# musket-ml/segmentation_training_pipeline

Hardware: AMD Instinct MI355X
Metric: images/sec U-Net/ResNet34 512x512 bs16 training step (higher is better)
Workload: dtype bf16; 1 GPU; U-Net/ResNet34 512x512x3 1-class, batch 16 per GPU, BCE+Dice, Adam, on-device augment S1 (BASELINE.json configs[1]); global_batch=16, parallelism=dp1, hipgraph=True

## Files before the change

segmentation_training_pipeline_amd/csrc/augment.hip:

```cpp
#include "common.h"
#include <cstdlib>

struct AugSample {
  float m[6];
  float add[3], mul[3];
  float flags, gray_q, noise_k, drop_t;
  float adde_lo, adde_hi, mule_lo, mule_hi;
  float seed, r0, r1, r2;
};

__device__ __forceinline__ uint32_t aug_hash(uint32_t seed, uint32_t pix, uint32_t ch, uint32_t op) {
  uint32_t h = seed ^ (pix * 0x9E3779B1u) ^ (ch * 0x85EBCA77u) ^ (op * 0xC2B2AE3Du);
  h ^= h >> 16; h *= 0x7feb352du; h ^= h >> 15; h *= 0x846ca68bu; h ^= h >> 16;
  return h;
}
__device__ __forceinline__ int clip255(int v) { return min(max(v, 0), 255); }

__device__ __forceinline__ int64_t fix10(double v) { return (int64_t)__double2ll_rn(v); }

__global__ __launch_bounds__(256) void augment_kernel(const uint8_t* __restrict__ img, const uint8_t* __restrict__ mask,
                                                      uint8_t* __restrict__ img_out, uint8_t* __restrict__ mask_out,
                                                      const AugSample* __restrict__ prm, int N, int Hin, int Win, int Hout,
                                                      int Wout, int C, const int32_t* __restrict__ field) {
  const int64_t total = (int64_t)N * Hout * Wout;
  for (int64_t i = (int64_t)blockIdx.x * 256 + threadIdx.x; i < total; i += (int64_t)gridDim.x * 256) {
    const int xo = (int)(i % Wout);
    const int yo = (int)((i / Wout) % Hout);
    const int n = (int)(i / ((int64_t)Wout * Hout));
    const AugSample s = prm[n];
    double xd = (double)xo, yd = (double)yo;
    if (field) {
      const int32_t f = field[i];
      xd = __dadd_rn(xd, __dmul_rn((double)(int16_t)(f & 0xffff), 0.015625));
      yd = __dadd_rn(yd, __dmul_rn((double)(int16_t)(f >> 16), 0.015625));
    }
    const int64_t X0 = fix10(__dmul_rn(__dmul_rn((double)s.m[0], xd), 1024.0)) +
                       fix10(__dmul_rn(__dadd_rn(__dmul_rn((double)s.m[1], yd), (double)s.m[2]), 1024.0));
    const int64_t Y0 = fix10(__dmul_rn(__dmul_rn((double)s.m[3], xd), 1024.0)) +
                       fix10(__dmul_rn(__dadd_rn(__dmul_rn((double)s.m[4], yd), (double)s.m[5]), 1024.0));
    const int64_t X = (X0 + 16) >> 5, Y = (Y0 + 16) >> 5;
    const int64_t ix = X >> 5, iy = Y >> 5;
    const int fx = (int)(X & 31), fy = (int)(Y & 31);
    const int w00 = (32 - fx) * (32 - fy), w01 = fx * (32 - fy), w10 = (32 - fx) * fy, w11 = fx * fy;
    const bool x0ok = ix >= 0 && ix < Win, x1ok = ix + 1 >= 0 && ix + 1 < Win;
    const bool y0ok = iy >= 0 && iy < Hin, y1ok = iy + 1 >= 0 && iy + 1 < Hin;
    const uint8_t* b = img + (int64_t)n * Hin * Win * C;
    const uint32_t flags = (uint32_t)s.flags, seed = (uint32_t)s.seed, pix = (uint32_t)(yo * Wout + xo);
    const int noise_k = (int)s.noise_k;
    const uint32_t drop_t = (uint32_t)s.drop_t;
    const int ae_lo = (int)s.adde_lo, ae_n = (int)s.adde_hi - ae_lo + 1;
    int px[4] = {0, 0, 0, 0};
    for (int c = 0; c < C; ++c) {
      const int v00 = (x0ok && y0ok) ? b[(iy * Win + ix) * C + c] : 0;
      const int v01 = (x1ok && y0ok) ? b[(iy * Win + ix + 1) * C + c] : 0;
      const int v10 = (x0ok && y1ok) ? b[((iy + 1) * Win + ix) * C + c] : 0;
      const int v11 = (x1ok && y1ok) ? b[((iy + 1) * Win + ix + 1) * C + c] : 0;
      int v = (w00 * v00 + w01 * v01 + w10 * v10 + w11 * v11 + 512) >> 10;
      const int cc = c < 3 ? c : 2;
      v = clip255(v + (int)s.add[cc]);
      if (s.mul[cc] != 1.f) v = clip255((int)rintf(__fmul_rn((float)v, s.mul[cc])));
      if (flags & 64u) {
        const float u = __fmul_rn((float)(aug_hash(seed, pix, (flags & 16u) ? c : 0, 1u) >> 8), 5.9604644775390625e-8f);
        const float m = __fadd_rn(s.mule_lo, __fmul_rn(__fsub_rn(s.mule_hi, s.mule_lo), u));
        v = clip255((int)rintf(__fmul_rn((float)v, m)));
      }
      if (flags & 32u) v = clip255(v + ae_lo + (int)(aug_hash(seed, pix, (flags & 8u) ? c : 0, 2u) % (uint32_t)ae_n));
      if (noise_k) {
        const uint32_t h = aug_hash(seed, pix, (flags & 2u) ? c : 0, 3u);
        const int sum = (int)(h & 255u) + (int)((h >> 8) & 255u) + (int)((h >> 16) & 255u) + (int)(h >> 24);
        v = clip255(v + (((sum - 510) * noise_k + 32768) >> 16));
      }
      if (drop_t && (aug_hash(seed, pix, (flags & 4u) ? c : 0, 4u) >> 8) < drop_t) v = 0;
      if (c < 4) px[c] = v;
      if (C != 3) img_out[i * C + c] = (uint8_t)((flags & 1u) ? 255 - v : v);
    }
    if (C == 3) {
      const int gq = (int)s.gray_q;
      if (gq) {
        const int gray = (px[0] * 4899 + px[1] * 9617 + px[2] * 1868 + 8192) >> 14;
#pragma unroll
        for (int c = 0; c < 3; ++c) px[c] = (gq * gray + (256 - gq) * px[c] + 128) >> 8;
      }
#pragma unroll
      for (int c = 0; c < 3; ++c) img_out[i * 3 + c] = (uint8_t)((flags & 1u) ? 255 - px[c] : px[c]);
    }
    if (mask) {
      const int64_t mx = (X0 + 512) >> 10, my = (Y0 + 512) >> 10;
      uint8_t mv = 0;
      if (mx >= 0 && mx < Win && my >= 0 && my < Hin) mv = mask[((int64_t)n * Hin + my) * Win + mx];
      mask_out[i] = mv;
    }
  }
}

static int launch_augment(const uint8_t* img, const uint8_t* mask, uint8_t* img_out, uint8_t* mask_out, const float* params,
                          const int32_t* field, int32_t N, int32_t Hin, int32_t Win, int32_t Hout, int32_t Wout, int32_t C, void* stream) {
  if (!img || !img_out || !params || N <= 0 || C <= 0 || (mask && !mask_out)) return STP_E_BADARG;
  int64_t g = ((int64_t)N * Hout * Wout + 255) / 256;
  if (g > 8192) g = 8192;
  hipLaunchKernelGGL(augment_kernel, dim3((int)g), dim3(256), 0, (hipStream_t)stream, img, mask, img_out, mask_out,
                     (const AugSample*)params, N, Hin, Win, Hout, Wout, C, field);
  STP_LAUNCH_CHECK();
  return STP_OK;
}

extern "C" int stp_augment_u8(const uint8_t* img, const uint8_t* mask, uint8_t* img_out, uint8_t* mask_out, const float* params,
                              int32_t N, int32_t Hin, int32_t Win, int32_t Hout, int32_t Wout, int32_t C, void* stream) {
  return launch_augment(img, mask, img_out, mask_out, params, nullptr, N, Hin, Win, Hout, Wout, C, stream);
}

extern "C" int stp_augment_field_u8(const uint8_t* img, const uint8_t* mask, uint8_t* img_out, uint8_t* mask_out, const float* params,
                                    const int32_t* field, int32_t N, int32_t Hin, int32_t Win, int32_t Hout, int32_t Wout, int32_t C,
                                    void* stream) {
  return launch_augment(img, mask, img_out, mask_out, params, field, N, Hin, Win, Hout, Wout, C, stream);
}

__device__ __forceinline__ int32_t pack_disp(int dx, int dy) {
  dx = min(max(dx, -32768), 32767);
  dy = min(max(dy, -32768), 32767);
  return (int32_t)(((uint32_t)dx & 0xffffu) | ((uint32_t)dy << 16));
}

__global__ __launch_bounds__(256) void field_piecewise_kernel(int32_t* __restrict__ field, const int32_t* __restrict__ grid, int N, int H, int W,
                                                              int R, int Cg) {
  const int64_t total = (int64_t)N * H * W;
  for (int64_t i = (int64_t)blockIdx.x * 256 + threadIdx.x; i < total; i += (int64_t)gridDim.x * 256) {
    const int x = (int)(i % W), y = (int)((i / W) % H), n = (int)(i / ((int64_t)W * H));
    const int64_t u = (int64_t)x * (Cg - 1) * 1024 / W, v = (int64_t)y * (R - 1) * 1024 / H;
    const int cx = min((int)(u >> 10), Cg - 2), cy = min((int)(v >> 10), R - 2);
    const int64_t fu = u - ((int64_t)cx << 10), fv = v - ((int64_t)cy << 10);
    const int32_t* g = grid + (((int64_t)n * R + cy) * Cg + cx) * 2;
    int d[2];
#pragma unroll
    for (int a = 0; a < 2; ++a) {
      const int64_t d00 = g[a], d10 = g[2 + a], d01 = g[2 * Cg + a], d11 = g[2 * Cg + 2 + a];
      const int64_t t = fu >= fv ? d00 * 1024 + fu * (d10 - d00) + fv * (d11 - d10) : d00 * 1024 + fv * (d01 - d00) + fu * (d11 - d01);
      d[a] = (int)((t + 512) >> 10);
    }
    field[i] = pack_disp(d[0], d[1]);
  }
}

extern "C" int stp_field_piecewise(int32_t* field, const int32_t* grid, int32_t N, int32_t H, int32_t W, int32_t rows, int32_t cols,
                                   void* stream) {
  if (!field || !grid || N <= 0 || H <= 0 || W <= 0 || rows < 2 || cols < 2) return STP_E_BADARG;
  int64_t g = ((int64_t)N * H * W + 255) / 256;
  if (g > 8192) g = 8192;
  hipLaunchKernelGGL(field_piecewise_kernel, dim3((int)g), dim3(256), 0, (hipStream_t)stream, field, grid, N, H, W, rows, cols);
  STP_LAUNCH_CHECK();
  return STP_OK;
}

#define STP_ELASTIC_RECORD 69
__global__ __launch_bounds__(256) void field_elastic_h_kernel(int32_t* __restrict__ tmp, const int32_t* __restrict__ prm, int N, int H, int W) {
  const int64_t total = (int64_t)N * H * W;
  for (int64_t i = (int64_t)blockIdx.x * 256 + threadIdx.x; i < total; i += (int64_t)gridDim.x * 256) {
    const int x = (int)(i % W), y = (int)((i / W) % H), n = (int)(i / ((int64_t)W * H));
    const int32_t* p = prm + (int64_t)n * STP_ELASTIC_RECORD;
    const uint32_t seed = (uint32_t)p[0];
    const int r = p[2];
    int t[2];
#pragma unroll
    for (int a = 0; a < 2; ++a) {
      int sum = 0;
      for (int k = -r; k <= r; ++k) {
        const int xx = x + k;
        if (xx < 0 || xx >= W) continue;
        const int nz = (int)(aug_hash(seed, (uint32_t)(y * W + xx), (uint32_t)a, 7u) >> 16) - 32768;
        sum += p[4 + (k < 0 ? -k : k)] * nz;
      }
      t[a] = (sum + 16384) >> 15;
    }
    tmp[i] = pack_disp(t[0], t[1]);
  }
}
__global__ __launch_bounds__(256) void field_elastic_v_kernel(int32_t* __restrict__ field, const int32_t* __restrict__ tmp,
                                                              const int32_t* __restrict__ prm, int N, int H, int W) {
  const int64_t total = (int64_t)N * H * W;
  for (int64_t i = (int64_t)blockIdx.x * 256 + threadIdx.x; i < total; i += (int64_t)gridDim.x * 256) {
    const int x = (int)(i % W), y = (int)((i / W) % H), n = (int)(i / ((int64_t)W * H));
    const int32_t* p = prm + (int64_t)n * STP_ELASTIC_RECORD;
    const int alpha = p[1], r = p[2];
    int s0 = 0, s1 = 0;
    for (int k = -r; k <= r; ++k) {
// ... 190 lines not shown
```

segmentation_training_pipeline_amd/csrc/bn_pool.hip:

```cpp
#include "common.h"
#include <algorithm>
#include <cstdlib>

#define BN_MAX_BLOCKS 1024
#ifndef POOL_ROWS
#define POOL_ROWS 4
#endif


template <typename T> __device__ __forceinline__ f32x4 ld4(const T* p);
template <> __device__ __forceinline__ f32x4 ld4<float>(const float* p) { return load4(p); }
template <> __device__ __forceinline__ f32x4 ld4<bf16_t>(const bf16_t* p) { return load4(p); }

template <typename T, int V> __device__ __forceinline__ void ldv(const T* p, float (&o)[V]) {
  if constexpr (V == 4) {
    const f32x4 v = ld4<T>(p);
    o[0] = v.x; o[1] = v.y; o[2] = v.z; o[3] = v.w;
  } else {
    const u32x4 r = *reinterpret_cast<const u32x4*>(p);
#pragma unroll
    for (int e = 0; e < 4; ++e) { o[2 * e] = h16lo_to_f32(r[e]); o[2 * e + 1] = h16hi_to_f32(r[e]); }
  }
}
template <typename T, int V> __device__ __forceinline__ void stv(T* p, const float (&o)[V]) {
// ... 1118 lines not shown
                       (bf16_t*)dx, rows, C, mean, rstd, gamma, (const float*)nullptr, sums, inv_rows, 0, accumulate_dx, (const long long*)nullptr, 0, (float*)nullptr, (float*)nullptr,
                       (const bf16_t*)dadd);
  else if (dtype == STP_F32)
    hipLaunchKernelGGL((bn_bwd_apply_kernel<float, 4>), dim3(gr), dim3(256), lds2, s, (const float*)x, (const float*)g, (float*)dx,
                       rows, C, mean, rstd, gamma, (const float*)nullptr, sums, inv_rows, 0, accumulate_dx, (const long long*)nullptr, 0, (float*)nullptr, (float*)nullptr,
                       (const float*)dadd);
  else
    return STP_E_BADARG;
  STP_LAUNCH_CHECK();
  return STP_OK;
}

extern "C" int stp_bn_backward_fused(const void* x, const void* g, void* dx, int32_t dtype, int64_t rows, int32_t C,
                                     const float* mean, const float* rstd, const float* gamma, const float* partial,
                                     int32_t tiles, float* dgamma, float* dbeta, int32_t accumulate_dx, void* workspace,
                                     size_t workspace_bytes, void* stream) {
  return stp_bn_backward_fused_add(x, g, dx, dx, dtype, rows, C, mean, rstd, gamma, partial, tiles, dgamma, dbeta, accumulate_dx, workspace,
                                   workspace_bytes, stream);
}

template <typename T, int V>
__global__ __launch_bounds__(256) void maxpool_fwd_kernel(const T* __restrict__ x, T* __restrict__ y, uint8_t* __restrict__ idx,
                                                          int N, int H, int W, int C, int Ho, int Wo) {
  const int cg = C / V;
  const int t = blockIdx.x * 256 + threadIdx.x;
  if (t >= Wo * cg) return;
  const int wo = t / cg, c = (t - wo * cg) * V;
  for (int rr = 0; rr < POOL_ROWS; ++rr) {
  const int orow = blockIdx.y * POOL_ROWS + rr;
  if (orow >= N * Ho) break;
  const int n = orow / Ho, ho = orow - n * Ho;
  float best[V];
  uint8_t bi[V];
  float v[9][V];
#pragma unroll
  for (int kh = 0; kh < 3; ++kh)
#pragma unroll
    for (int kw = 0; kw < 3; ++kw) {
      const int h = min(max(2 * ho - 1 + kh, 0), H - 1), w = min(max(2 * wo - 1 + kw, 0), W - 1);
      ldv<T, V>(x + (((size_t)n * H + h) * W + w) * C + c, v[kh * 3 + kw]);
    }
#pragma unroll
  for (int kh = 0; kh < 3; ++kh)
#pragma unroll
    for (int kw = 0; kw < 3; ++kw) {
      const int h = 2 * ho - 1 + kh, w = 2 * wo - 1 + kw;
      const bool in = (unsigned)h < (unsigned)H && (unsigned)w < (unsigned)W;
#pragma unroll
      for (int e = 0; e < V; ++e) {
        const float tv = in ? v[kh * 3 + kw][e] : 0.f;
        if ((kh | kw) == 0 || tv > best[e]) { best[e] = tv; bi[e] = (uint8_t)(kh * 3 + kw); }
      }
    }
  const size_t o = (((size_t)n * Ho + ho) * Wo + wo) * C + c;
  stv<T, V>(y + o, best);
  if (idx) {
    if constexpr (V == 8) *reinterpret_cast<uint2*>(idx + o) = *reinterpret_cast<const uint2*>(bi);
    else *reinterpret_cast<uint32_t*>(idx + o) = *reinterpret_cast<const uint32_t*>(bi);
  }
  }
}

__global__ __launch_bounds__(256) void bn_apply_maxpool_kernel(const bf16_t* __restrict__ x, bf16_t* __restrict__ yb, bf16_t* __restrict__ y,
                                                               uint8_t* __restrict__ idx, int N, int H, int W, int C, int Ho, int Wo,
                                                               const float* mean, const float* rstd, const float* gamma, const float* beta, int relu) {
  const int cg = C >> 3;
  const int t = blockIdx.x * 256 + threadIdx.x;
  if (t >= Wo * cg) return;
  const int wo = t / cg, c = (t - wo * cg) * 8;
  float sc[8], sh[8];
  {
    const f32x4 m0 = *reinterpret_cast<const f32x4*>(mean + c), m1 = *reinterpret_cast<const f32x4*>(mean + c + 4);
    const f32x4 r0 = *reinterpret_cast<const f32x4*>(rstd + c), r1 = *reinterpret_cast<const f32x4*>(rstd + c + 4);
    f32x4 g0 = {1.f, 1.f, 1.f, 1.f}, g1 = g0, b0 = {0.f, 0.f, 0.f, 0.f}, b1 = b0;
    if (gamma) { g0 = *reinterpret_cast<const f32x4*>(gamma + c); g1 = *reinterpret_cast<const f32x4*>(gamma + c + 4); }
    if (beta) { b0 = *reinterpret_cast<const f32x4*>(beta + c); b1 = *reinterpret_cast<const f32x4*>(beta + c + 4); }
#pragma unroll
    for (int e = 0; e < 8; ++e) {
      const float r = e < 4 ? r0[e & 3] : r1[e & 3], k = gamma ? r * (e < 4 ? g0[e & 3] : g1[e & 3]) : r;
      sc[e] = k;
      sh[e] = (e < 4 ? b0[e & 3] : b1[e & 3]) - (e < 4 ? m0[e & 3] : m1[e & 3]) * k;
    }
  }
  for (int rr = 0; rr < POOL_ROWS; ++rr) {
    const int orow = blockIdx.y * POOL_ROWS + rr;
    if (orow >= N * Ho) break;
    const int n = orow / Ho, ho = orow - n * Ho;
    u32x4 v[9];
#pragma unroll
    for (int kh = 0; kh < 3; ++kh)
#pragma unroll
      for (int kw = 0; kw < 3; ++kw) {
        const int h = min(max(2 * ho - 1 + kh, 0), H - 1), w = min(max(2 * wo - 1 + kw, 0), W - 1);
        v[kh * 3 + kw] = *reinterpret_cast<const u32x4*>(x + (((size_t)n * H + h) * W + w) * C + c);
      }
    float best[8];
    uint8_t bi[8];
#pragma unroll
    for (int kh = 0; kh < 3; ++kh)
#pragma unroll
      for (int kw = 0; kw < 3; ++kw) {
        const int h = 2 * ho - 1 + kh, w = 2 * wo - 1 + kw;
        const bool in = (unsigned)h < (unsigned)H && (unsigned)w < (unsigned)W;
        u32x4 o;
#pragma unroll
        for (int e = 0; e < 4; ++e) {
          const float lo = bn_act(bn_affine(h16lo_to_f32(v[kh * 3 + kw][e]), sc[2 * e], sh[2 * e]), relu);
          const float hi = bn_act(bn_affine(h16hi_to_f32(v[kh * 3 + kw][e]), sc[2 * e + 1], sh[2 * e + 1]), relu);
          o[e] = pack_bf16x2(lo, hi);
          const float tl = in ? h16lo_to_f32(o[e]) : 0.f, th = in ? h16hi_to_f32(o[e]) : 0.f;
          if ((kh | kw) == 0 || tl > best[2 * e]) { best[2 * e] = tl; bi[2 * e] = (uint8_t)(kh * 3 + kw); }
          if ((kh | kw) == 0 || th > best[2 * e + 1]) { best[2 * e + 1] = th; bi[2 * e + 1] = (uint8_t)(kh * 3 + kw); }
        }
        if (kh >= 1 && kw >= 1 && in) *reinterpret_cast<u32x4*>(yb + (((size_t)n * H + h) * W + w) * C + c) = o;
      }
    const size_t oo = (((size_t)n * Ho + ho) * Wo + wo) * C + c;
    *reinterpret_cast<u32x4*>(y + oo) = u32x4{pack_bf16x2(best[0], best[1]), pack_bf16x2(best[2], best[3]), pack_bf16x2(best[4], best[5]),
                                             pack_bf16x2(best[6], best[7])};
    if (idx) *reinterpret_cast<uint2*>(idx + oo) = *reinterpret_cast<const uint2*>(bi);
  }
}
extern "C" int stp_bn_apply_maxpool3x3s2(const void* x, void* yb, void* y, uint8_t* idx, int32_t N, int32_t H, int32_t W, int32_t C, int32_t dtype,
                                         const float* mean, const float* rstd, const float* gamma, const float* beta, int32_t relu, void* stream) {
  if (!stp_dtype_ok(dtype)) return STP_E_BADARG;
  if (dtype != STP_H16 || !x || !yb || !y || !mean || !rstd || N <= 0 || (C & 7) || (H & 1) || (W & 1)) return STP_E_BADARG;
  const int Ho = H / 2, Wo = W / 2;
  if ((int64_t)N * Ho > 65535 * POOL_ROWS) return STP_E_BADARG;
  const dim3 grid(ceil_div(Wo * (C / 8), 256), ceil_div(N * Ho, POOL_ROWS));
  hipLaunchKernelGGL(bn_apply_maxpool_kernel, grid, dim3(256), 0, (hipStream_t)stream, (const bf16_t*)x, (bf16_t*)yb, (bf16_t*)y, idx, N, H, W, C, Ho, Wo,
                     mean, rstd, gamma, beta, relu);
  STP_LAUNCH_CHECK();
  return STP_OK;
}

__device__ __forceinline__ f32x4 stored4(f32x4 v, const float*) { return v; }
__device__ __forceinline__ f32x4 stored4(f32x4 v, const bf16_t*) {
  const uint32_t a = pack_bf16x2(v.x, v.y), b = pack_bf16x2(v.z, v.w);
  return f32x4{h16lo_to_f32(a), h16hi_to_f32(a), h16lo_to_f32(b), h16hi_to_f32(b)};
}

#define BNB_ROWS 8


template <typename T, int V>
__device__ __forceinline__ void bnb_mask_store(float (&g)[V], size_t o, int c, const BnBack& bnb, T* __restrict__ dx, float (&sg)[V],
                                               float (&sq)[V]) {
  float xv[V];
  ldv<T, V>(reinterpret_cast<const T*>(bnb.x) + o, xv);
#pragma unroll
  for (int q = 0; q < V / 4; ++q) {
    const BnBackCh k = bnback_load(bnb, c + 4 * q);
    const f32x4 st = stored4(f32x4{g[4 * q], g[4 * q + 1], g[4 * q + 2], g[4 * q + 3]}, (const T*)nullptr);
    f32x4 s4 = {0.f, 0.f, 0.f, 0.f}, q4 = {0.f, 0.f, 0.f, 0.f};
    const f32x4 m = bnback_apply(k, bnb.relu, f32x4{xv[4 * q], xv[4 * q + 1], xv[4 * q + 2], xv[4 * q + 3]}, st, s4, q4);
#pragma unroll
    for (int e = 0; e < 4; ++e) { g[4 * q + e] = m[e]; sg[4 * q + e] += s4[e]; sq[4 * q + e] += q4[e]; }
  }
  stv<T, V>(dx + o, g);
}

template <int V>
__device__ __forceinline__ void bnb_reduce(const float (&sg)[V], const float (&sq)[V], int cg, int C, float* __restrict__ partial) {
  extern __shared__ float red[];
#pragma unroll
  for (int e = 0; e < V; ++e) { red[threadIdx.x * 2 * V + e] = sg[e]; red[threadIdx.x * 2 * V + V + e] = sq[e]; }
  __syncthreads();
  const int cl = cg < 256 ? cg : 256;
  for (int idx = threadIdx.x; idx < cl * V; idx += 256) {
    const int gq = idx / V, e = idx - gq * V;
    const int cg0 = (blockIdx.x * 256 + gq) % cg;
    float s = 0.f, q2 = 0.f;
    for (int l = gq; l < 256; l += cl) { s += red[l * 2 * V + e]; q2 += red[l * 2 * V + V + e]; }
    const size_t nblk = (size_t)gridDim.x * gridDim.y, blk = (size_t)blockIdx.y * gridDim.x + blockIdx.x;
    const int ch = cg0 * V + e;
    partial[(size_t)ch * nblk + blk] = s;
    partial[((size_t)C + ch) * nblk + blk] = q2;
  }
}

template <typename T, int V, bool BNB>
__global__ __launch_bounds__(256) void maxpool_bwd_kernel(const uint8_t* __restrict__ idx, const T* __restrict__ dy,
                                                          T* __restrict__ dx, int N, int H, int W, int C, int Ho, int Wo,
                                                          int accumulate, BnBack bnb, float* __restrict__ partial) {
  const int cg = C / V;
  const int t = blockIdx.x * 256 + threadIdx.x;
  const bool on = t < W * cg;
  if (!BNB && !on) return;
  const int w = on ? t / cg : 0, c = on ? (t - w * cg) * V : 0;
  constexpr int ROWS = BNB ? BNB_ROWS : POOL_ROWS;
  float sg[V], sq[V];
#pragma unroll
  for (int e = 0; e < V; ++e) { sg[e] = 0.f; sq[e] = 0.f; }
  for (int rr = 0; rr < ROWS; ++rr) {
    const int row = blockIdx.y * ROWS + rr;
    if (row >= N * H || !on) break;
    const int n = row / H, h = row - n * H;
    float g[V];
// ... 1568 lines not shown
}
extern "C" int stp_maxpool_k(const void* x, void* y, int32_t* idx, int32_t N, int32_t H, int32_t W, int32_t C, int32_t k, int32_t dtype,
                             void* stream) {
  if (!stp_dtype_ok(dtype)) return STP_E_BADARG;
  if (!x || !y || N <= 0 || H <= 0 || W <= 0 || C <= 0 || k < 1 || H % k || W % k) return STP_E_BADARG;
  const int g = grid_for((int64_t)N * (H / k) * (W / k) * C);
  if (dtype == STP_H16) hipLaunchKernelGGL(maxpool_k_kernel<bf16_t>, dim3(g), dim3(256), 0, (hipStream_t)stream, (const bf16_t*)x, (bf16_t*)y, idx, N, H, W, C, k);
  else if (dtype == STP_F32) hipLaunchKernelGGL(maxpool_k_kernel<float>, dim3(g), dim3(256), 0, (hipStream_t)stream, (const float*)x, (float*)y, idx, N, H, W, C, k);
  else return STP_E_BADARG;
  STP_LAUNCH_CHECK();
  return STP_OK;
}
extern "C" int stp_maxpool_k_bwd(const int32_t* idx, const void* dy, void* dx, int32_t N, int32_t H, int32_t W, int32_t C, int32_t k,
                                 int32_t dtype, int32_t accumulate, void* stream) {
  if (!stp_dtype_ok(dtype)) return STP_E_BADARG;
  if (!idx || !dy || !dx || N <= 0 || H <= 0 || W <= 0 || C <= 0 || k < 1 || H % k || W % k) return STP_E_BADARG;
  const int g = grid_for((int64_t)N * H * W * C);
  if (dtype == STP_H16) hipLaunchKernelGGL(maxpool_k_bwd_kernel<bf16_t>, dim3(g), dim3(256), 0, (hipStream_t)stream, idx, (const bf16_t*)dy, (bf16_t*)dx, N, H, W, C, k, accumulate);
  else if (dtype == STP_F32) hipLaunchKernelGGL(maxpool_k_bwd_kernel<float>, dim3(g), dim3(256), 0, (hipStream_t)stream, idx, (const float*)dy, (float*)dx, N, H, W, C, k, accumulate);
  else return STP_E_BADARG;
  STP_LAUNCH_CHECK();
  return STP_OK;
}

template <typename T>
__global__ __launch_bounds__(256) void resize_nearest_kernel(const T* __restrict__ x, T* __restrict__ y, int N, int H, int W, int C, int f,
                                                             int ldo, int coff) {
  const int Ho = H * f, Wo = W * f;
  const int64_t total = (int64_t)N * Ho * Wo * C;
  for (int64_t i = (int64_t)blockIdx.x * 256 + threadIdx.x; i < total; i += (int64_t)gridDim.x * 256) {
    const int c = (int)(i % C);
    const int64_t p = i / C;
    const int xo = (int)(p % Wo), yo = (int)((p / Wo) % Ho), n = (int)(p / ((int64_t)Wo * Ho));
    y[p * ldo + coff + c] = x[(((int64_t)n * H + yo / f) * W + xo / f) * C + c];
  }
}
template <typename T>
__global__ __launch_bounds__(256) void resize_nearest_bwd_kernel(const T* __restrict__ dy, T* __restrict__ dx, int N, int H, int W, int C,
                                                                 int f, int ldo, int coff, int accumulate) {
  const int Wo = W * f, Ho = H * f;
  const int64_t total = (int64_t)N * H * W * C;
  for (int64_t i = (int64_t)blockIdx.x * 256 + threadIdx.x; i < total; i += (int64_t)gridDim.x * 256) {
    const int c = (int)(i % C);
    const int64_t p = i / C;
    const int xi = (int)(p % W), yi = (int)((p / W) % H), n = (int)(p / ((int64_t)W * H));
    float s = 0.f;
    for (int a = 0; a < f; ++a)
      for (int b = 0; b < f; ++b) s += Elem<T>::load(dy + (((int64_t)n * Ho + yi * f + a) * Wo + xi * f + b) * ldo + coff + c);
    if (accumulate) s += Elem<T>::load(dx + i);
    Elem<T>::store(dx + i, s);
  }
}
extern "C" int stp_resize_nearest(const void* x, void* y, int32_t N, int32_t H, int32_t W, int32_t C, int32_t factor, int32_t ldo, int32_t coff,
                                  int32_t dtype, void* stream) {
  if (!stp_dtype_ok(dtype)) return STP_E_BADARG;
  if (!x || !y || N <= 0 || H <= 0 || W <= 0 || C <= 0 || factor < 1 || ldo < coff + C || coff < 0) return STP_E_BADARG;
  const int g = grid_for((int64_t)N * H * factor * W * factor * C);
  if (dtype == STP_H16) hipLaunchKernelGGL(resize_nearest_kernel<bf16_t>, dim3(g), dim3(256), 0, (hipStream_t)stream, (const bf16_t*)x, (bf16_t*)y, N, H, W, C, factor, ldo, coff);
  else if (dtype == STP_F32) hipLaunchKernelGGL(resize_nearest_kernel<float>, dim3(g), dim3(256), 0, (hipStream_t)stream, (const float*)x, (float*)y, N, H, W, C, factor, ldo, coff);
  else return STP_E_BADARG;
  STP_LAUNCH_CHECK();
  return STP_OK;
}
extern "C" int stp_resize_nearest_bwd(const void* dy, void* dx, int32_t N, int32_t H, int32_t W, int32_t C, int32_t factor, int32_t ldo,
                                      int32_t coff, int32_t dtype, int32_t accumulate, void* stream) {
  if (!stp_dtype_ok(dtype)) return STP_E_BADARG;
  if (!dy || !dx || N <= 0 || H <= 0 || W <= 0 || C <= 0 || factor < 1 || ldo < coff + C || coff < 0) return STP_E_BADARG;
  const int g = grid_for((int64_t)N * H * W * C);
  if (dtype == STP_H16) hipLaunchKernelGGL(resize_nearest_bwd_kernel<bf16_t>, dim3(g), dim3(256), 0, (hipStream_t)stream, (const bf16_t*)dy, (bf16_t*)dx, N, H, W, C, factor, ldo, coff, accumulate);
  else if (dtype == STP_F32) hipLaunchKernelGGL(resize_nearest_bwd_kernel<float>, dim3(g), dim3(256), 0, (hipStream_t)stream, (const float*)dy, (float*)dx, N, H, W, C, factor, ldo, coff, accumulate);
  else return STP_E_BADARG;
  STP_LAUNCH_CHECK();
  return STP_OK;
}

__global__ __launch_bounds__(256) void colsum_finalize_kernel(const float* partial, int blocks, int C, float* out,
                                                              int accumulate) {
  const int c = blockIdx.x * 4 + (threadIdx.x & 3);
  const Sum2 t = reduce_partials(partial, blocks, C, c, false);
  if ((threadIdx.x >> 2) != 0 || c >= C) return;
  out[c] = accumulate ? out[c] + (float)t.s : (float)t.s;
}

extern "C" int stp_channel_sum(const void* x, int32_t dtype, int64_t rows, int32_t C, float* out, int32_t accumulate,
                               void* workspace, size_t workspace_bytes, void* stream) {
  if (!stp_dtype_ok(dtype)) return STP_E_BADARG;
  if (!x || !out || !workspace || rows <= 0 || C <= 0 || (C & 3)) return STP_E_BADARG;
  if (workspace_bytes < stp_bn_workspace_bytes(C)) return STP_E_WORKSPACE;
  hipStream_t s = (hipStream_t)stream;
  const int blocks = bn_blocks(rows);
  float* partial = (float*)workspace;
  if (dtype == STP_H16 && (C & 7) == 0)
    hipLaunchKernelGGL((bn_partial_kernel<bf16_t, 8>), dim3(blocks), dim3(256), 256 * 16 * sizeof(float), s, (const bf16_t*)x, rows, C, partial);
  else if (dtype == STP_H16)
    hipLaunchKernelGGL((bn_partial_kernel<bf16_t, 4>), dim3(blocks), dim3(256), 256 * 8 * sizeof(float), s, (const bf16_t*)x, rows, C, partial);
  else if (dtype == STP_F32)
    hipLaunchKernelGGL((bn_partial_kernel<float, 4>), dim3(blocks), dim3(256), 256 * 8 * sizeof(float), s, (const float*)x, rows, C, partial);
  else
    return STP_E_BADARG;
  STP_LAUNCH_CHECK();
  hipLaunchKernelGGL(colsum_finalize_kernel, dim3(ceil_div(C, 4)), dim3(256), 0, s, partial, blocks, C, out, accumulate);
  STP_LAUNCH_CHECK();
  return STP_OK;
}

template <typename T>
__global__ __launch_bounds__(256) void add_inplace_kernel(T* __restrict__ dst, const T* __restrict__ src, int64_t n4) {
  for (int64_t i = (int64_t)blockIdx.x * 256 + threadIdx.x; i < n4; i += (int64_t)gridDim.x * 256)
    store4(dst + i * 4, ld4<T>(dst + i * 4) + ld4<T>(src + i * 4));
}

extern "C" int stp_add_inplace(void* dst, const void* src, int64_t count, int32_t dtype, void* stream) {
  if (!stp_dtype_ok(dtype)) return STP_E_BADARG;
  if (!dst || !src || count <= 0 || (count & 3)) return STP_E_BADARG;
  const int g = grid_for(count >> 2);
  hipStream_t s = (hipStream_t)stream;
  if (dtype == STP_H16)
    hipLaunchKernelGGL(add_inplace_kernel<bf16_t>, dim3(g), dim3(256), 0, s, (bf16_t*)dst, (const bf16_t*)src, count >> 2);
  else if (dtype == STP_F32)
    hipLaunchKernelGGL(add_inplace_kernel<float>, dim3(g), dim3(256), 0, s, (float*)dst, (const float*)src, count >> 2);
  else
    return STP_E_BADARG;
  STP_LAUNCH_CHECK();
  return STP_OK;
}
```

segmentation_training_pipeline_amd/csrc/conv_sc.h:

```cpp
#pragma once
#include "common.h"
#include <cstdlib>
#include <type_traits>
#include <utility>

struct ScArgs {
  const char* src;
  const char* weight;
  const float* bias;
  char* dst;
  int N, H, W, Hs, Ws, Cout, up, accumulate, relu;
  int tiles_x, tiles_y;
  FastDiv divTx, divTy;
  float* stats;
  int stat_slots;
  BnBack bnb;
  int sum2;
  uint32_t src_bytes;
  BnBack pbn;
};

template <typename T> struct ScStageBn;
template <> struct ScStageBn<float> {
  f32x4 sc, sh;
  __device__ __forceinline__ void load(const BnBack& b, int c) { const BnBackCh k = bnback_load(b, c); sc = k.sc; sh = k.sh; }
  __device__ __forceinline__ void load_tab(const float* tsc, const float* tsh, int c) {
    sc = *reinterpret_cast<const f32x4*>(tsc + c); sh = *reinterpret_cast<const f32x4*>(tsh + c);
  }
  __device__ __forceinline__ u32x4 apply(const u32x4& r, int relu) const {
    u32x4 o;
#pragma unroll
    for (int e = 0; e < 4; ++e) o[e] = __float_as_uint(bn_act(bn_affine(__uint_as_float(r[e]), sc[e], sh[e]), relu));
    return o;
  }
};
template <> struct ScStageBn<bf16_t> {
  f32x2 sc[4], sh[4];
  __device__ __forceinline__ void load(const BnBack& b, int c) {
    const BnBackCh k0 = bnback_load(b, c), k1 = bnback_load(b, c + 4);
    sc[0] = f32x2{k0.sc[0], k0.sc[1]}; sc[1] = f32x2{k0.sc[2], k0.sc[3]}; sc[2] = f32x2{k1.sc[0], k1.sc[1]}; sc[3] = f32x2{k1.sc[2], k1.sc[3]};
    sh[0] = f32x2{k0.sh[0], k0.sh[1]}; sh[1] = f32x2{k0.sh[2], k0.sh[3]}; sh[2] = f32x2{k1.sh[0], k1.sh[1]}; sh[3] = f32x2{k1.sh[2], k1.sh[3]};
  }
  __device__ __forceinline__ void load_tab(const float* tsc, const float* tsh, int c) {
#pragma unroll
    for (int e = 0; e < 4; ++e) { sc[e] = *reinterpret_cast<const f32x2*>(tsc + c + 2 * e); sh[e] = *reinterpret_cast<const f32x2*>(tsh + c + 2 * e); }
  }
  __device__ __forceinline__ u32x4 apply(const u32x4& r, int relu) const {
    u32x4 o;
#pragma unroll
    for (int e = 0; e < 4; ++e) {
      f32x2 v = {h16lo_to_f32(r[e]), h16hi_to_f32(r[e])};
      v = __builtin_elementwise_fma(v, sc[e], sh[e]);
      o[e] = pack_bf16x2(bn_act(v.x, relu), bn_act(v.y, relu));
    }
    return o;
  }
};


constexpr int SC_TH = 8, SC_TW = 32, SC_HW = SC_TW + 2, SC_HH = SC_TH + 2;

template <int... Ks, typename F>
__device__ __forceinline__ void sc_unroll_seq(std::integer_sequence<int, Ks...>, F&& f) { (f(std::integral_constant<int, Ks>{}), ...); }
template <int N, typename F>
__device__ __forceinline__ void sc_unroll(F&& f) { sc_unroll_seq(std::make_integer_sequence<int, N>{}, f); }
#ifndef SC_RING
#define SC_RING 8
#endif

#ifndef SC_WPE_SMALL
#define SC_WPE_SMALL 4
#endif

static inline bool sc_stream_on() {
  static const bool on = !(getenv("STP_SC_STREAM") && atoi(getenv("STP_SC_STREAM")) == 0);
  return on;
}
static inline int sc_cu_count() {
  static const int cus = [] {
    int d = 0, n = 0;
    if (hipGetDevice(&d) != hipSuccess || hipDeviceGetAttribute(&n, hipDeviceAttributeMultiprocessorCount, d) != hipSuccess || n <= 0) n = 256;
    return n;
  }();
  return cus;
}
static inline int sc_stream_blocks(int dtype, int cin, int cout, int ntiles) {
  const int per_cu = cout <= 16 ? (dtype == STP_H16 && cin <= 16 ? SC_WPE_SMALL : 3) : 2;
  const int64_t b = (int64_t)sc_cu_count() * per_cu;
  return (int)(b < ntiles ? b : ntiles);
}


struct ScWgArgs {
  const char* src;
  const char* dy;
  float* slabs;
  int N, H, W, Hs, Ws, Cout, up;
  int tiles_x, tiles_y, ntiles;
  int ctot, coff;
  uint32_t src_bytes, dy_bytes;
  BnBack pbn;
};

constexpr int ST_HH = (SC_TH - 1) * 2 + 7, ST_HW = 70, ST_WROW = 464, ST_HALO = ST_HH * ST_HW * 8, ST_WBYTES = 64 * ST_WROW;

struct StemArgs {
  const char* src;
  const char* weight;
  char* dst;
  int N, H, W, Ho, Wo, tiles_x, tiles_y;
  FastDiv divTx, divTy;
  float* stats;
  uint32_t src_bytes;
};

bool stem_lean_serves(int N, int H, int W);
int stem_lean_blocks(int ntiles);
int stem_lean_launch(const StemArgs& a, hipStream_t s);
bool stem_wg_lean_serves(int N, int H, int W, int Ho, int Wo);
int stem_wg_lean_blocks(int N, int Ho, int Wo);
int stem_wg_lean_launch(const void* src, const void* dy, float* slabs, int N, int H, int W, int Ho, int Wo, hipStream_t s);

int sc_lean_launch(const ScArgs& a, int cin, int dtype, hipStream_t s);
int sc_wg_lean_launch(const ScWgArgs& a, int cin, int cout, int dtype, int blocks, hipStream_t s);
```

segmentation_training_pipeline_amd/csrc/conv_sc.hip:

```cpp
#include "conv_sc.h"

__device__ __forceinline__ f32x4 sc_stored(f32x4 v, const float*) { return v; }
__device__ __forceinline__ f32x4 sc_stored(f32x4 v, const bf16_t*) {
  const uint32_t a = pack_bf16x2(v.x, v.y), b = pack_bf16x2(v.z, v.w);
  return f32x4{h16lo_to_f32(a), h16hi_to_f32(a), h16lo_to_f32(b), h16hi_to_f32(b)};
}

template <typename T> struct ScMma;
template <> struct ScMma<bf16_t> {
  __device__ static __forceinline__ void run(const u32x4& a, const u32x4& b, f32x4& c) {
    c = mfma16_16x16x32(a, b, c);
  }
};
template <> struct ScMma<float> {
  __device__ static __forceinline__ void run(const u32x4& a, const u32x4& b, f32x4& c) {
    c = __builtin_amdgcn_mfma_f32_16x16x4f32(__uint_as_float(a.x), __uint_as_float(b.x), c, 0, 0, 0);
    c = __builtin_amdgcn_mfma_f32_16x16x4f32(__uint_as_float(a.y), __uint_as_float(b.y), c, 0, 0, 0);
    c = __builtin_amdgcn_mfma_f32_16x16x4f32(__uint_as_float(a.z), __uint_as_float(b.z), c, 0, 0, 0);
    c = __builtin_amdgcn_mfma_f32_16x16x4f32(__uint_as_float(a.w), __uint_as_float(b.w), c, 0, 0, 0);
  }
};

template <typename T> struct ScRaw4;
template <> struct ScRaw4<float> {
// ... 455 lines not shown
        if (PART && c == NCH - 1 && !last_ok) v = u32x4{0u, 0u, 0u, 0u};
#pragma unroll
        for (int i = 0; i < TM; ++i) ScMma<T>::run(fa[i][c], v, acc[i][F]);
        if constexpr (k + D < R) issue(std::integral_constant<int, k + D>{});
      });
    } else
#endif
    {
#pragma unroll
    for (int f = 0; f < 4; ++f) {
#pragma unroll
      for (int c = 0; c < NCH; ++c) {
        u32x4 fb = {0u, 0u, 0u, 0u};
#if !defined(STP_EXP) || STP_EXP != 13
        if (bl[c] != 0xffffffffu) fb = *reinterpret_cast<const u32x4*>(smem + bl[c] + (CUR * BUF + ((f >> 1) * SC_HW + (f & 1) * 16) * PIXB));
#pragma unroll
        for (int i = 0; i < TM; ++i) ScMma<T>::run(fa[i][c], fb, acc[i][f]);
#else
        if (a.N < 0) acc[0][f][0] += __uint_as_float(fa[0][c][0] + bl[c]);
#endif
      }
    }
    }
    ep.finish(a, acc, red, n, y0, x0, tile, ntiles, tid, wave, lr, lg);
  };

  ep.reset_stats();
  for (int tile = t_first; tile < t_end; tile += 2 * t_step) {
    body(tile, std::integral_constant<int, 0>{});
    if (tile + t_step < t_end) body(tile + t_step, std::integral_constant<int, 1>{});
  }
  ep.flush_stats(a, red, (int)blockIdx.x, (int)gridDim.x, tid, wave, lr, lg);
}

template <typename T, int CIN, int TM>
static int launch_sc(const ScArgs& a, hipStream_t s) {
  const int ntiles = a.N * a.tiles_x * a.tiles_y;
  if (sc_stream_on()) {
    constexpr int NV = SC_HH * SC_HW * (CIN / Elem<T>::VEC), NPASS = (NV + 255) / 256;
    const size_t lds = (size_t)2 * NPASS * 4096 + (4 * TM * 16 * 2 + 128 + 64) * sizeof(float);
    const int blocks = sc_stream_blocks(Elem<T>::DTYPE, CIN, TM * 16, ntiles);
    static bool attr_set = false;
    if (lds > 64 * 1024 && !attr_set) {
      if (hipFuncSetAttribute(reinterpret_cast<const void*>(conv_sc_stream_kernel<T, CIN, TM>), hipFuncAttributeMaxDynamicSharedMemorySize, (int)lds) != hipSuccess)
        return STP_E_LAUNCH;
      attr_set = true;
    }
    hipLaunchKernelGGL((conv_sc_stream_kernel<T, CIN, TM>), dim3(blocks), dim3(256), lds, s, a);
    STP_LAUNCH_CHECK();
    return STP_OK;
  }
  const size_t lds = (size_t)SC_HH * SC_HW * CIN * sizeof(T) + 4 * TM * 16 * 2 * sizeof(float);
  hipLaunchKernelGGL((conv_sc_kernel<T, CIN, TM>), dim3(ntiles), dim3(256), lds, s, a);
  STP_LAUNCH_CHECK();
  return STP_OK;
}

extern "C" int stp_conv2d_sc_stats_tiles(const stp_conv_params* p) {
  const int ntiles = p->N * ceil_div(p->Hv, SC_TH) * ceil_div(p->Wv, SC_TW);
  if (!sc_stream_on() || p->stats_slots) return ntiles;
  return sc_stream_blocks(p->dtype, p->C0, p->Cout <= 16 ? 16 : 32, ntiles);
}

template <typename T>
static int dispatch_sc(const ScArgs& a, int cin, hipStream_t s) {
  const int tm = a.Cout <= 16 ? 1 : 2;
  switch (cin * 4 + tm) {
    case 4 * 4 + 1: if constexpr (sizeof(T) == 4) return launch_sc<T, 4, 1>(a, s); else return STP_E_BADARG;
    case 4 * 4 + 2: if constexpr (sizeof(T) == 4) return launch_sc<T, 4, 2>(a, s); else return STP_E_BADARG;
    case 8 * 4 + 1: return launch_sc<T, 8, 1>(a, s);
    case 8 * 4 + 2: return launch_sc<T, 8, 2>(a, s);
    case 16 * 4 + 1: return launch_sc<T, 16, 1>(a, s);
    case 16 * 4 + 2: return launch_sc<T, 16, 2>(a, s);
    case 32 * 4 + 1: return launch_sc<T, 32, 1>(a, s);
    case 32 * 4 + 2: return launch_sc<T, 32, 2>(a, s);
    default: return STP_E_BADARG;
  }
}

extern "C" int stp_conv2d_sc_eligible(const stp_conv_params* p) {
  if (!p || !stp_dtype_ok(p->dtype)) return 0;
  const int vec = p->dtype == STP_H16 ? 8 : 4;
  const int cin = p->C0;
  const bool cin_ok = p->dtype == STP_F32 ? (cin == 4 || cin == 8 || cin == 16) : (cin == 8 || cin == 16 || cin == 32);
  return p->KH == 3 && p->KW == 3 && p->stride == 1 && p->pad == 1 && p->C1 == 0 && cin_ok && (cin % vec) == 0 && p->Cout <= 32 &&
         p->Cd0 == p->Cout && !p->residual && p->Ho == p->Hv && p->Wo == p->Wv &&
         (p->src0_mode == STP_SRC_DIRECT || (p->src0_mode == STP_SRC_NEAREST2X && p->Hv == 2 * p->Hs0 && p->Wv == 2 * p->Ws0));
}

extern "C" int stp_conv2d_sc(const stp_conv_params* p, void* stream) {
  if (!stp_conv2d_sc_eligible(p) || !p->src0 || !p->weight || !p->dst0) return STP_E_BADARG;
  ScArgs a;
  a.src = (const char*)p->src0; a.weight = (const char*)p->weight; a.bias = p->bias; a.dst = (char*)p->dst0;
  a.N = p->N; a.H = p->Hv; a.W = p->Wv; a.Hs = p->Hs0; a.Ws = p->Ws0; a.Cout = p->Cout;
  a.up = p->src0_mode == STP_SRC_NEAREST2X; a.accumulate = p->accumulate0; a.relu = p->relu;
  {
    const uint64_t sb = (uint64_t)p->N * p->Hs0 * p->Ws0 * p->C0 * (p->dtype == STP_H16 ? 2 : 4);
    if (sb >= 0x80000000ull) return STP_E_BADARG;
    a.src_bytes = (uint32_t)sb;
  }
  a.tiles_x = ceil_div(a.W, SC_TW); a.tiles_y = ceil_div(a.H, SC_TH);
  a.divTx = make_fastdiv((uint32_t)a.tiles_x); a.divTy = make_fastdiv((uint32_t)a.tiles_y);
  a.stats = p->stats_partial;
  a.stat_slots = p->stats_slots;
  if (a.stats && (p->Cout & 3)) return STP_E_BADARG;
  if (a.stat_slots && (!a.stats || (a.stat_slots & (a.stat_slots - 1)) || a.stat_slots > 64)) return STP_E_BADARG;
  a.bnb.x = (const char*)p->bnb_x; a.bnb.mean = p->bnb_mean; a.bnb.rstd = p->bnb_rstd; a.bnb.gamma = p->bnb_gamma;
  a.bnb.beta = p->bnb_beta; a.bnb.relu = p->bnb_relu;
  a.sum2 = p->dst_sum2x2;
  a.pbn.x = nullptr; a.pbn.mean = p->src_bn_mean; a.pbn.rstd = p->src_bn_rstd; a.pbn.gamma = p->src_bn_gamma; a.pbn.beta = p->src_bn_beta;
  a.pbn.relu = p->src_bn_relu;
  if (a.pbn.mean && !a.pbn.rstd) return STP_E_BADARG;
  if (a.bnb.x && (!a.stats || !a.bnb.mean || !a.bnb.rstd || p->relu)) return STP_E_BADARG;
  if (a.sum2 && ((p->Cout & 3) || (a.H & 1) || (a.W & 1) || p->bias || p->relu || (a.stats && !a.bnb.x))) return STP_E_BADARG;
  const_cast<stp_conv_params*>(p)->stats_tiles = stp_conv2d_sc_stats_tiles(p);
  hipStream_t s = (hipStream_t)stream;
  {
    const int r = sc_lean_launch(a, p->C0, p->dtype, s);
    if (r != 1) return r;
  }
  return p->dtype == STP_H16 ? dispatch_sc<bf16_t>(a, p->C0, s) : dispatch_sc<float>(a, p->C0, s);
}

struct ScwArgs {
  const char* src;
  const char* weight;
  char* dst_up;
  char* dst_sk;
  int N, H, W, C0, C1, acc_up, acc_sk;
  int tiles_x, tiles_y;
  FastDiv divTx, divTy;
  float* stats;
  BnBack bnb;
  uint32_t src_bytes, x_bytes;
  uint32_t up_bytes, sk_bytes;
};

template <typename T>
__global__ __launch_bounds__(256, 2) void conv_scw_stream_kernel(const ScwArgs a) {
  constexpr int CIN = 32, SZ = (int)sizeof(T), K = 9 * CIN, NCH = 9, VPP = 4, PIXB = CIN * SZ;
  constexpr int NV = SC_HH * SC_HW * VPP, NPASS = (NV + 255) / 256, BUF = NPASS * 4096;
  static_assert(SZ == 2, "16-bit storage");
  extern __shared__ __attribute__((aligned(16))) char smem[];
  float* ktab = reinterpret_cast<float*>(smem + 2 * BUF);
  constexpr int XBUF = 3 * 4096;
  char* const xlds = smem + 2 * BUF + 2048;
  const int tid = threadIdx.x, lane = tid & 63;
  const int wave = __builtin_amdgcn_readfirstlane(tid >> 6);
  const int lr = lane & 15, lg = lane >> 4;
  const int cbi[2] = {a.C0 == 64 ? wave * 16 : wave * 32, a.C0 == 64 ? 64 + wave * 16 : wave * 32 + 16};
  const bool upi[2] = {cbi[0] < a.C0, cbi[1] < a.C0};

  const int ntiles = a.N * a.tiles_x * a.tiles_y;
  int t_first, t_step, t_end;
  if ((gridDim.x & 7) == 0) {
    const int q = ntiles >> 3, r = ntiles & 7, x = blockIdx.x & 7;
    const int start = x < r ? x * (q + 1) : r * (q + 1) + (x - r) * q;
    t_first = start + (int)(blockIdx.x >> 3); t_step = (int)(gridDim.x >> 3); t_end = start + q + (x < r ? 1 : 0);
  } else {
    t_first = (int)blockIdx.x; t_step = (int)gridDim.x; t_end = ntiles;
  }
  if (t_first >= t_end) {
    if (a.stats && tid < a.C0) {
      a.stats[(size_t)tid * gridDim.x + blockIdx.x] = 0.f;
      a.stats[((size_t)a.C0 + tid) * gridDim.x + blockIdx.x] = 0.f;
    }
    return;
  }

  const __amdgpu_buffer_rsrc_t rs = __builtin_amdgcn_make_buffer_rsrc((void*)a.src, 0, a.src_bytes, 0x00020000);
  const int H2 = a.H >> 1, W2 = a.W >> 1;
  const bool bnb = a.bnb.x != nullptr;
  const bool xrs_on = bnb;
  const __amdgpu_buffer_rsrc_t xrs = __builtin_amdgcn_make_buffer_rsrc((void*)(bnb ? a.bnb.x : a.src), 0, bnb ? a.x_bytes : 0u, 0x00020000);
  int hyx[NPASS];
  const int cvb = (tid % VPP) * 16;
#pragma unroll
  for (int p = 0; p < NPASS; ++p) {
    const int v = p * 256 + tid, pix = v / VPP;
    const int hy = pix / SC_HW, hx = pix - hy * SC_HW;
    hyx[p] = v < NV ? (hy << 16 | hx) : -1;
  }
  int xq[3];
  {
    const int vpp = a.C0 >> 3;
#pragma unroll
    for (int p = 0; p < 3; ++p) {
      const int v = p * 256 + tid, px = v / vpp;
      xq[p] = (xrs_on && px < 64) ? ((px >> 4) << 16 | (px & 15) << 8 | (v - px * vpp)) : -1;
    }
  }
  auto decode = [&](int tile, int& n, int& y0, int& x0) {
    const int bq = (int)fdiv((uint32_t)tile, a.divTx);
    const int tx = tile - bq * a.tiles_x;
    n = (int)fdiv((uint32_t)bq, a.divTy);
    const int ty = bq - n * a.tiles_y;
    y0 = ty * SC_TH; x0 = tx * SC_TW;
  };
  uint32_t hrel[NPASS];
#pragma unroll
  for (int p = 0; p < NPASS; ++p) hrel[p] = hyx[p] >= 0 ? (uint32_t)(((hyx[p] >> 16) * a.W + (hyx[p] & 0xffff)) * PIXB + cvb) : 0x80000000u;
  auto issue_tile = [&](int tile, int b) {
    int n, y0, x0;
// ... 1153 lines not shown
        u32x4 fa[TMo];
#pragma unroll
        for (int i = 0; i < TMo; ++i) {
          const char* p = dyt + ((row * SC_TW + xl) * COUT + i * 16) * SZ + qb;
          const s16x4_t lo = __builtin_amdgcn_ds_read_tr16_b64_v4i16((__attribute__((address_space(3))) s16x4_t*)p);
          const s16x4_t hi = __builtin_amdgcn_ds_read_tr16_b64_v4i16((__attribute__((address_space(3))) s16x4_t*)(p + 16 * DYB));
          const u32x2 l2 = __builtin_bit_cast(u32x2, lo), h2 = __builtin_bit_cast(u32x2, hi);
          fa[i] = u32x4{l2.x, l2.y, h2.x, h2.y};
        }
#pragma unroll
        for (int t = 0; t < 3; ++t) {
          const int tap = wave + 4 * t;
          if (tap < 9) {
            const int kh = tap / 3, kw = tap - kh * 3;
#pragma unroll
            for (int j = 0; j < TNi; ++j) {
              const char* p = halo + (((row + kh) * SC_HW + xl + kw) * CIN + j * 16) * SZ + qb;
              const s16x4_t lo = __builtin_amdgcn_ds_read_tr16_b64_v4i16((__attribute__((address_space(3))) s16x4_t*)p);
              const s16x4_t hi = __builtin_amdgcn_ds_read_tr16_b64_v4i16((__attribute__((address_space(3))) s16x4_t*)(p + 16 * PIXB));
              const u32x2 l2 = __builtin_bit_cast(u32x2, lo), h2 = __builtin_bit_cast(u32x2, hi);
              const u32x4 fb = u32x4{l2.x, l2.y, h2.x, h2.y};
#pragma unroll
              for (int i = 0; i < TMo; ++i)
                acc[t][i][j] = mfma16_16x16x32(fa[i], fb, acc[t][i][j]);
            }
          }
        }
      } else {
#pragma unroll
        for (int s = 0; s < 8; ++s) {
          const int x = s * 4 + lg;
          float fa[TMo];
#pragma unroll
          for (int i = 0; i < TMo; ++i) fa[i] = *reinterpret_cast<const float*>(dyt + ((row * SC_TW + x) * COUT + i * 16 + lr) * SZ);
#pragma unroll
          for (int t = 0; t < 3; ++t) {
            const int tap = wave + 4 * t;
            if (tap < 9) {
              const int kh = tap / 3, kw = tap - kh * 3;
#pragma unroll
              for (int j = 0; j < TNi; ++j) {
                const float fb = *reinterpret_cast<const float*>(halo + (((row + kh) * SC_HW + x + kw) * CIN + j * 16 + lr) * SZ);
#pragma unroll
                for (int i = 0; i < TMo; ++i) acc[t][i][j] = __builtin_amdgcn_mfma_f32_16x16x4f32(fa[i], fb, acc[t][i][j], 0, 0, 0);
              }
            }
          }
        }
      }
    }
  }

  float* out = a.slabs + (size_t)blockIdx.x * a.Cout * (9 * a.ctot);
#pragma unroll
  for (int t = 0; t < 3; ++t) {
    const int tap = wave + 4 * t;
    if (tap >= 9) continue;
#pragma unroll
    for (int i = 0; i < TMo; ++i)
#pragma unroll
      for (int j = 0; j < TNi; ++j)
#pragma unroll
        for (int r = 0; r < 4; ++r) {
          const int co = i * 16 + lg * 4 + r;
          if (co < a.Cout) out[(size_t)co * (9 * a.ctot) + tap * a.ctot + a.coff + j * 16 + lr] = acc[t][i][j][r];
        }
  }
}

#define SC_WG_MAX_BLOCKS 1024

static bool wgrad_stem_shape(const stp_wgrad_params* p) {
  return p->dtype == STP_H16 && p->C0 == 4 && p->C1 == 0 && p->KH == 7 && p->KW == 8 && p->stride == 2 && p->pad == 3 && p->Cout == 64 &&
         p->src0_mode == STP_SRC_DIRECT && p->Hs0 == p->Hv && p->Ws0 == p->Wv && p->Ho == (p->Hv - 1) / 2 + 1 && p->Wo == (p->Wv - 1) / 2 + 1 &&
         !p->src_bn_mean && stem_wg_lean_serves(p->N, p->Hv, p->Wv, p->Ho, p->Wo);
}

extern "C" int stp_wgrad_sc_eligible(const stp_wgrad_params* p) {
  if (!p || !stp_dtype_ok(p->dtype)) return 0;
  if (wgrad_stem_shape(p)) return 1;
  const int vec = p->dtype == STP_H16 ? 8 : 4;
  const bool c0ok = p->C0 == 16 || p->C0 == 32 || (p->C0 == 64 && vec == 8);
  const bool c1ok = p->C1 == 0 || p->C1 == 16 || p->C1 == 32 || (p->C1 == 64 && vec == 8);
  return p->KH == 3 && p->KW == 3 && p->stride == 1 && p->pad == 1 && c0ok && c1ok &&
         (p->Cout == 8 || p->Cout == 16 || p->Cout == 32 || (p->Cout == 4 && vec == 4)) && (p->Cout % vec) == 0 &&
         p->Ho == p->Hv && p->Wo == p->Wv &&
         (p->src0_mode == STP_SRC_DIRECT || (p->src0_mode == STP_SRC_NEAREST2X && p->Hv == 2 * p->Hs0 && p->Wv == 2 * p->Ws0));
}

extern "C" int stp_wgrad_sc_slabs(const stp_wgrad_params* p) {
  if (wgrad_stem_shape(p)) return stem_wg_lean_blocks(p->N, p->Ho, p->Wo);
  const int64_t tiles = (int64_t)p->N * ceil_div(p->Hv, SC_TH) * ceil_div(p->Wv, SC_TW);
  static const int max_blocks = getenv("STP_SC_WG_BLOCKS") ? atoi(getenv("STP_SC_WG_BLOCKS")) : SC_WG_MAX_BLOCKS;
  const int vec = p->dtype == STP_H16 ? 8 : 4, cin = p->C0 > p->C1 ? p->C0 : p->C1;
  const int64_t npx = ((int64_t)SC_HH * SC_HW * (cin / vec) + 255) / 256, npd = ((int64_t)SC_TH * SC_TW * ((p->Cout + vec - 1) / vec) + 255) / 256;
  const int64_t lds = 2 * (npx + npd) * 4096;
  int per_cu = (int)((160 * 1024) / (lds > 0 ? lds : 1));
  per_cu = per_cu < 1 ? 1 : per_cu > 4 ? 4 : per_cu;
  int64_t blocks = (int64_t)sc_cu_count() * per_cu;
  if (blocks > max_blocks) blocks = max_blocks;
  return (int)(tiles < blocks ? tiles : blocks);
}

template <typename T, int CIN, int COUT>
static int launch_sc_wg(const ScWgArgs& a, int blocks, hipStream_t s) {
  if (sc_stream_on() && a.src_bytes && a.dy_bytes) {
    constexpr int VEC = Elem<T>::VEC;
    constexpr int NPX = (SC_HH * SC_HW * (CIN / VEC) + 255) / 256, NPD = (SC_TH * SC_TW * (COUT / VEC) + 255) / 256;
    const size_t lds = (size_t)2 * (NPX + NPD) * 4096;
    static bool attr_set = false;
    if (lds > 64 * 1024 && !attr_set) {
      if (hipFuncSetAttribute(reinterpret_cast<const void*>(conv_sc_wgrad_stream_kernel<T, CIN, COUT>), hipFuncAttributeMaxDynamicSharedMemorySize, (int)lds) != hipSuccess)
        return STP_E_LAUNCH;
      attr_set = true;
    }
    hipLaunchKernelGGL((conv_sc_wgrad_stream_kernel<T, CIN, COUT>), dim3(blocks), dim3(256), lds, s, a);
    STP_LAUNCH_CHECK();
    return STP_OK;
  }
  const size_t lds = (size_t)SC_HH * SC_HW * CIN * sizeof(T) + (size_t)SC_TH * SC_TW * COUT * sizeof(T) + 64;
  hipLaunchKernelGGL((conv_sc_wgrad_kernel<T, CIN, COUT>), dim3(blocks), dim3(256), lds, s, a);
  STP_LAUNCH_CHECK();
  return STP_OK;
}

template <typename T>
static int sc_wg_dispatch(const ScWgArgs& a, int cin, int cout, int blocks, hipStream_t s) {
  {
    const int r = sc_wg_lean_launch(a, cin, cout, Elem<T>::DTYPE, blocks, s);
    if (r != 1) return r;
  }
  const int key = cin * 64 + cout;
  if constexpr (sizeof(T) == 2) {
    switch (key) {
      case 16 * 64 + 8: return launch_sc_wg<T, 16, 8>(a, blocks, s);
      case 16 * 64 + 16: return launch_sc_wg<T, 16, 16>(a, blocks, s);
      case 16 * 64 + 32: return launch_sc_wg<T, 16, 32>(a, blocks, s);
      case 32 * 64 + 8: return launch_sc_wg<T, 32, 8>(a, blocks, s);
      case 32 * 64 + 16: return launch_sc_wg<T, 32, 16>(a, blocks, s);
      case 32 * 64 + 32: return launch_sc_wg<T, 32, 32>(a, blocks, s);
      case 64 * 64 + 8: return launch_sc_wg<T, 64, 8>(a, blocks, s);
      case 64 * 64 + 16: return launch_sc_wg<T, 64, 16>(a, blocks, s);
      case 64 * 64 + 32: return launch_sc_wg<T, 64, 32>(a, blocks, s);
      default: return STP_E_BADARG;
    }
  } else {
    switch (key) {
      case 16 * 64 + 4: return launch_sc_wg<T, 16, 4>(a, blocks, s);
      case 16 * 64 + 8: return launch_sc_wg<T, 16, 8>(a, blocks, s);
      case 16 * 64 + 16: return launch_sc_wg<T, 16, 16>(a, blocks, s);
      case 16 * 64 + 32: return launch_sc_wg<T, 16, 32>(a, blocks, s);
      case 32 * 64 + 4: return launch_sc_wg<T, 32, 4>(a, blocks, s);
      case 32 * 64 + 8: return launch_sc_wg<T, 32, 8>(a, blocks, s);
      case 32 * 64 + 16: return launch_sc_wg<T, 32, 16>(a, blocks, s);
      case 32 * 64 + 32: return launch_sc_wg<T, 32, 32>(a, blocks, s);
      default: return STP_E_BADARG;
    }
  }
}

extern "C" int stp_wgrad_sc_partial(const stp_wgrad_params* p, void* workspace, void* stream) {
  if (!stp_wgrad_sc_eligible(p) || !p->src0 || !p->dy || !workspace || (p->C1 > 0 && !p->src1)) return STP_E_BADARG;
  if (wgrad_stem_shape(p)) return stem_wg_lean_launch(p->src0, p->dy, (float*)workspace, p->N, p->Hv, p->Wv, p->Ho, p->Wo, (hipStream_t)stream);
  ScWgArgs a;
  a.dy = (const char*)p->dy; a.slabs = (float*)workspace;
  a.N = p->N; a.H = p->Hv; a.W = p->Wv; a.Cout = p->Cout;
  a.tiles_x = ceil_div(a.W, SC_TW); a.tiles_y = ceil_div(a.H, SC_TH); a.ntiles = a.N * a.tiles_x * a.tiles_y;
  a.ctot = p->C0 + p->C1;
  a.pbn.x = nullptr; a.pbn.mean = p->src_bn_mean; a.pbn.rstd = p->src_bn_rstd; a.pbn.gamma = p->src_bn_gamma; a.pbn.beta = p->src_bn_beta;
  a.pbn.relu = p->src_bn_relu;
  if (a.pbn.mean && (!a.pbn.rstd || p->C1 > 0)) return STP_E_BADARG;
  const int blocks = stp_wgrad_sc_slabs(p);
  hipStream_t s = (hipStream_t)stream;
  const uint64_t szb = p->dtype == STP_H16 ? 2 : 4, lim = 0x80000000ull;
  const uint64_t dyb = (uint64_t)p->N * p->Hv * p->Wv * p->Cout * szb, b0 = (uint64_t)p->N * p->Hs0 * p->Ws0 * p->C0 * szb;
  const uint64_t b1 = (uint64_t)p->N * p->Hv * p->Wv * p->C1 * szb;
  a.dy_bytes = dyb < lim ? (uint32_t)dyb : 0u;
  a.src_bytes = b0 < lim ? (uint32_t)b0 : 0u;
  a.src = (const char*)p->src0; a.Hs = p->Hs0; a.Ws = p->Ws0; a.up = p->src0_mode == STP_SRC_NEAREST2X; a.coff = 0;
  int rc = p->dtype == STP_H16 ? sc_wg_dispatch<bf16_t>(a, p->C0, p->Cout, blocks, s) : sc_wg_dispatch<float>(a, p->C0, p->Cout, blocks, s);
  if (rc != STP_OK || p->C1 == 0) return rc;
  a.pbn.mean = nullptr;
  a.src = (const char*)p->src1; a.Hs = p->Hv; a.Ws = p->Wv; a.up = 0; a.coff = p->C0;
  a.src_bytes = b1 < lim ? (uint32_t)b1 : 0u;
  return p->dtype == STP_H16 ? sc_wg_dispatch<bf16_t>(a, p->C1, p->Cout, blocks, s) : sc_wg_dispatch<float>(a, p->C1, p->Cout, blocks, s);
}
```

segmentation_training_pipeline_amd/csrc/conv_sc_lean.hip:

```cpp
#include "conv_sc.h"

enum { SCL_STATS = 0, SCL_BNB = 1, SCL_BNB_SUM2 = 2, SCL_HEAD = 3 };

struct TileC { int n, y0, x0; bool interior; };

__device__ __forceinline__ f32x2 scl_unpack(uint32_t w) { return f32x2{h16lo_to_f32(w), h16hi_to_f32(w)}; }

template <int TM>
__device__ __forceinline__ void scl_store(char* p, const u32x2 (&o)[TM]) {
  if constexpr (TM == 2) *reinterpret_cast<u32x4*>(p) = u32x4{o[0].x, o[0].y, o[1].x, o[1].y};
  else *reinterpret_cast<u32x2*>(p) = o[0];
}

template <int CIN, int TM, int EPI, bool PBN, bool UP>
__global__ __launch_bounds__(256, (TM == 1 ? (CIN <= 16 ? SC_WPE_SMALL : 3) : 2)) void conv_sc_lean_kernel(const ScArgs a) {
  typedef bf16_t T;
  constexpr int SZ = 2, VEC = 8, KC = 32, K = 9 * CIN, NCH = (K + KC - 1) / KC, VPP = CIN / VEC, PIXB = CIN * SZ;
  constexpr int HH = UP ? SC_TH / 2 + 2 : SC_HH, HW = UP ? SC_TW / 2 + 2 : SC_HW;
  constexpr int NV = HH * HW * VPP, NPASS = (NV + 255) / 256, BUF = NPASS * 4096;
  constexpr bool PART = (K % KC) != 0;
  constexpr int COUT = EPI == SCL_HEAD ? 1 : TM * 16;
  constexpr int CB = COUT * SZ;
  static_assert(EPI != SCL_HEAD || TM == 1, "head: one output channel");
  static_assert(!PBN || EPI == SCL_STATS || EPI == SCL_HEAD, "producer BatchNormalization: forward only");

  extern __shared__ __attribute__((aligned(16))) char smem[];
  float* red = reinterpret_cast<float*>(smem + 2 * BUF);
  float* ptab = red + 4 * TM * 16 * 2;
  const int tid = threadIdx.x, lane = tid & 63;
  const int wave = __builtin_amdgcn_readfirstlane(tid >> 6);
  const int lr = lane & 15, lg = lane >> 4;
  constexpr int sh = UP ? 1 : 0;

  const int ntiles = a.N * a.tiles_x * a.tiles_y;
  int t_first, t_step, t_end;
  if ((gridDim.x & 7) == 0) {
    const int q = ntiles >> 3, r = ntiles & 7, x = blockIdx.x & 7;
    const int start = x < r ? x * (q + 1) : r * (q + 1) + (x - r) * q;
    t_first = start + (int)(blockIdx.x >> 3); t_step = (int)(gridDim.x >> 3); t_end = start + q + (x < r ? 1 : 0);
  } else {
    t_first = (int)blockIdx.x; t_step = (int)gridDim.x; t_end = ntiles;
  }
  if (t_first >= t_end) return;

  const __amdgpu_buffer_rsrc_t rs = __builtin_amdgcn_make_buffer_rsrc((void*)a.src, 0, a.src_bytes, 0x00020000);
  int hyx[NPASS];
  uint32_t lo[NPASS];
  const int cvb = (tid % VPP) * 16;
#pragma unroll
  for (int p = 0; p < NPASS; ++p) {
    const int v = p * 256 + tid, pix = v / VPP;
    const int hy = pix / HW, hx = pix - hy * HW;
    hyx[p] = v < NV ? (hy << 16 | hx) : -1;
    lo[p] = v < NV ? (uint32_t)(((hy - 1) * a.Ws + (hx - 1)) * PIXB + cvb) : 0x80000000u;
  }

  auto decode = [&](int tile) -> TileC {
    const int bq = (int)fdiv((uint32_t)tile, a.divTx);
    const int tx = tile - bq * a.tiles_x;
    const int n = (int)fdiv((uint32_t)bq, a.divTy);
    const int ty = bq - n * a.tiles_y;
    TileC t;
    t.n = n; t.y0 = ty * SC_TH; t.x0 = tx * SC_TW;
    t.interior = ty > 0 && tx > 0 && t.y0 + SC_TH < a.H && t.x0 + SC_TW < a.W;
    return t;
  };
  auto issue_tile = [&](const TileC& t, int b, bool live) -> uint32_t {
    uint32_t inside = 0;
    if (live && t.interior) {
      const uint32_t tb = (uint32_t)((t.n * a.Hs + (t.y0 >> sh)) * a.Ws + (t.x0 >> sh)) * (uint32_t)PIXB;
#pragma unroll
      for (int p = 0; p < NPASS; ++p)
        __builtin_amdgcn_raw_ptr_buffer_load_lds(rs, (__attribute__((address_space(3))) void*)(smem + b * BUF + p * 4096 + wave * 1024), 16, (int)(tb + lo[p]), 0, 0, 0);
      inside = (1u << NPASS) - 1u;
    } else {
#pragma unroll
      for (int p = 0; p < NPASS; ++p) {
        const int gy = (t.y0 >> sh) - 1 + (hyx[p] >> 16), gx = (t.x0 >> sh) - 1 + (hyx[p] & 0xffff);
        const bool ok = live && hyx[p] >= 0 && (unsigned)gy < (unsigned)a.Hs && (unsigned)gx < (unsigned)a.Ws;
        const uint32_t off = ok ? (uint32_t)((t.n * a.Hs + gy) * a.Ws + gx) * (uint32_t)PIXB + (uint32_t)cvb : 0x80000000u;
        inside |= ok ? (1u << p) : 0u;
        __builtin_amdgcn_raw_ptr_buffer_load_lds(rs, (__attribute__((address_space(3))) void*)(smem + b * BUF + p * 4096 + wave * 1024), 16, (int)off, 0, 0, 0);
      }
    }
    return inside;
  };

  TileC tc = decode(t_first);
  uint32_t inside_cur = issue_tile(tc, 0, true);

  u32x4 fa[TM][NCH];
  constexpr int NA = UP ? 2 : 1;
  uint32_t bla[NA][NCH];
#pragma unroll
  for (int c = 0; c < NCH; ++c) {
    const int k0 = c * KC + lg * VEC;
    const int tap = k0 / CIN, ch = k0 - tap * CIN;
    const int kh = tap / 3, kw = tap - kh * 3;
#pragma unroll
    for (int ar = 0; ar < NA; ++ar) {
      const int prow = UP ? wave + ((ar + kh + 1) >> 1) : wave * 2 + kh, pcol = UP ? ((lr + kw + 1) >> 1) : kw + lr;
      bla[ar][c] = (uint32_t)(uintptr_t)smem + ((k0 < K) ? (uint32_t)(((prow * HW + pcol) * CIN + ch) * SZ) : 0u);
    }
#pragma unroll
    for (int i = 0; i < TM; ++i) {
      u32x4 w = {0u, 0u, 0u, 0u};
      const int wrow = TM == 2 ? (lr >> 2) * 8 + i * 4 + (lr & 3) : i * 16 + lr;
      if (k0 < K) w = *reinterpret_cast<const u32x4*>(a.weight + ((size_t)wrow * K + k0) * SZ);
      fa[i][c] = w;
    }
  }
  const bool last_ok = (NCH - 1) * KC + lg * VEC < K;
  if (PBN && tid < CIN) {
    const float r = a.pbn.rstd[tid], sc = a.pbn.gamma ? r * a.pbn.gamma[tid] : r;
    ptab[tid] = sc;
    ptab[32 + tid] = (a.pbn.beta ? a.pbn.beta[tid] : 0.f) - a.pbn.mean[tid] * sc;
  }
  f32x2 ksc[TM][2], ksh[TM][2];
  float alo = 0.f, ahi = 0.f;
  if constexpr (EPI == SCL_BNB || EPI == SCL_BNB_SUM2) {
#pragma unroll
    for (int i = 0; i < TM; ++i) {
      const BnBackCh k = bnback_load(a.bnb, TM == 2 ? lg * 8 + i * 4 : i * 16 + lg * 4);
      ksc[i][0] = f32x2{k.sc[0], k.sc[1]}; ksc[i][1] = f32x2{k.sc[2], k.sc[3]};
      ksh[i][0] = f32x2{k.sh[0], k.sh[1]}; ksh[i][1] = f32x2{k.sh[2], k.sh[3]};
    }
    alo = a.bnb.relu ? __uint_as_float(1u) : -__builtin_inff();
    ahi = a.bnb.relu == 2 ? __uint_as_float(0x40bfffffu) : __builtin_inff();
  }
  float bias0 = 0.f;
  if constexpr (EPI == SCL_HEAD) bias0 = a.bias ? a.bias[0] : 0.f;
  constexpr int LB = TM == 2 ? 16 : 8;
  const uint32_t so = EPI == SCL_BNB_SUM2 ? (uint32_t)((wave * (a.W >> 1) + (lr >> 1)) * CB + lg * LB)
                      : EPI == SCL_HEAD   ? (uint32_t)(((wave * 2) * a.W + lr) * CB)
                                          : (uint32_t)(((wave * 2) * a.W + lr) * CB + lg * LB);
  f32x4 ss[TM], qq[TM];
#pragma unroll
  for (int i = 0; i < TM; ++i) { ss[i] = f32x4{0.f, 0.f, 0.f, 0.f}; qq[i] = f32x4{0.f, 0.f, 0.f, 0.f}; }
  lds_barrier();

  const bool own = !(lr & 1);
  auto prefetch = [&](const TileC& pt, const bool EDGE, u32x2 (&xo)[TM][4]) __attribute__((always_inline)) {
    if constexpr (EPI == SCL_BNB) {
      const char* xb = a.bnb.x + (((size_t)pt.n * a.H + pt.y0) * a.W + pt.x0) * CB;
#pragma unroll
      for (int f = 0; f < 4; ++f) {
        const char* xf = xb + (size_t)(((f >> 1) * a.W + (f & 1) * 16) * CB);
        const bool ok = !EDGE || (pt.y0 + wave * 2 + (f >> 1) < a.H && pt.x0 + (f & 1) * 16 + lr < a.W);
        if constexpr (TM == 2) {
          const u32x4 w4 = *reinterpret_cast<const u32x4*>(ok ? xf + so : a.bnb.x);
          xo[0][f] = u32x2{w4.x, w4.y}; xo[TM - 1][f] = u32x2{w4.z, w4.w};
        } else {
          xo[0][f] = *reinterpret_cast<const u32x2*>(ok ? xf + so : a.bnb.x);
        }
      }
    }
    if constexpr (EPI == SCL_BNB_SUM2) {
      const char* xb = a.bnb.x + (((size_t)pt.n * (a.H >> 1) + (pt.y0 >> 1)) * (a.W >> 1) + (pt.x0 >> 1)) * CB;
#pragma unroll
      for (int h2 = 0; h2 < 2; ++h2) {
        const char* xf = xb + (size_t)(h2 * 8 * CB);
        const bool ok = own && (!EDGE || (pt.y0 + wave * 2 < a.H && pt.x0 + h2 * 16 + lr < a.W));
        if constexpr (TM == 2) {
          const u32x4 w4 = *reinterpret_cast<const u32x4*>(ok ? xf + so : a.bnb.x);
          xo[0][h2] = u32x2{w4.x, w4.y}; xo[TM - 1][h2] = u32x2{w4.z, w4.w};
        } else {
          xo[0][h2] = *reinterpret_cast<const u32x2*>(ok ? xf + so : a.bnb.x);
        }
      }
    }
  };
  u32x2 xp[TM][4];
  constexpr bool AHEAD = (EPI == SCL_BNB || EPI == SCL_BNB_SUM2) && !(CIN == 32 && TM == 2 && EPI == SCL_BNB);
  if constexpr (AHEAD) {
    if (tc.interior) prefetch(tc, false, xp); else prefetch(tc, true, xp);
  }

  int cur = 0;
  for (int tile = t_first; tile < t_end; tile += t_step, cur ^= 1) {
    const TileC t = tc;
    ScStageBn<T> sbn;
    if (PBN) sbn.load_tab(ptab, ptab + 32, (tid % VPP) * VEC);
    __builtin_amdgcn_s_waitcnt(0x0f70);
    asm volatile("" ::: "memory");
    if (PBN) {
#pragma unroll
      for (int p0 = 0; p0 < NPASS; p0 += 3) {
        u32x4 v[3];
#pragma unroll
        for (int q = 0; q < 3; ++q)
          if (p0 + q < NPASS) v[q] = *reinterpret_cast<const u32x4*>(smem + cur * BUF + ((p0 + q) * 256 + tid) * 16);
#pragma unroll
        for (int q = 0; q < 3; ++q)
          if (p0 + q < NPASS && (inside_cur & (1u << (p0 + q))))
            *reinterpret_cast<u32x4*>(smem + cur * BUF + ((p0 + q) * 256 + tid) * 16) = sbn.apply(v[q], a.pbn.relu);
      }
    }
    lds_barrier();

    const bool edge = !t.interior;
    if constexpr (!AHEAD) {
      if (edge) prefetch(t, true, xp); else prefetch(t, false, xp);
    }
    const int next = tile + t_step;
    const bool live = next < t_end;
    if (live) tc = decode(next);
    inside_cur = issue_tile(tc, cur ^ 1, live);
    u32x2 xn[TM][4];
    if (AHEAD && live) {
      if (tc.interior) prefetch(tc, false, xn); else prefetch(tc, true, xn);
    }

    f32x4 acc[TM][4];
#pragma unroll
    for (int i = 0; i < TM; ++i)
#pragma unroll
      for (int f = 0; f < 4; ++f) acc[i][f] = f32x4{0.f, 0.f, 0.f, 0.f};
    {
      constexpr int R = 4 * NCH;
      constexpr int RING = (CIN == 32 && TM == 2 && EPI == SCL_BNB_SUM2) ? 4 : SC_RING;
      constexpr int D = RING < R ? RING : R;
      u32x4 ring[D];
      auto issue = [&ring, &bla](auto kc) {
        constexpr int k = decltype(kc)::value, F = k / NCH, c = k % NCH;
        constexpr int OFF = UP ? (F & 1) * 8 * PIXB : ((F >> 1) * SC_HW + (F & 1) * 16) * PIXB;
        asm volatile("ds_read_b128 %0, %1 offset:%2" : "=v"(ring[k % D]) : "v"(bla[UP ? (F >> 1) : 0][c]), "n"(OFF));
      };
      sc_unroll<D>(issue);
      sc_unroll<R>([&ring, &fa, &acc, &issue, last_ok](auto kc) {
        constexpr int k = decltype(kc)::value, F = k / NCH, c = k % NCH;
        constexpr int young = (R - 1 - k) < (D - 1) ? (R - 1 - k) : (D - 1);
        asm volatile("s_waitcnt lgkmcnt(%1)" : "+v"(ring[k % D]) : "n"(young));
        u32x4 v = ring[k % D];
        if (PART && c == NCH - 1 && !last_ok) v = u32x4{0u, 0u, 0u, 0u};
#pragma unroll
        for (int i = 0; i < TM; ++i) acc[i][F] = mfma16_16x16x32(fa[i][c], v, acc[i][F]);
        if constexpr (k + D < R) issue(std::integral_constant<int, k + D>{});
      });
    }

    auto epilogue = [&](const bool EDGE) __attribute__((always_inline)) {
      bool okf[4];
#pragma unroll
      for (int f = 0; f < 4; ++f) okf[f] = !EDGE || (t.y0 + wave * 2 + (f >> 1) < a.H && t.x0 + (f & 1) * 16 + lr < a.W);
      if constexpr (EPI == SCL_STATS) {
        char* ob = a.dst + (((size_t)t.n * a.H + t.y0) * a.W + t.x0) * CB;
        const bool st = a.stats != nullptr;
#pragma unroll
        for (int f = 0; f < 4; ++f) {
          char* of = ob + (size_t)(((f >> 1) * a.W + (f & 1) * 16) * CB);
          u32x2 o[TM];
#pragma unroll
          for (int i = 0; i < TM; ++i) {
            const f32x4 v = acc[i][f];
            o[i] = u32x2{pack_bf16x2(v.x, v.y), pack_bf16x2(v.z, v.w)};
            if (st && okf[f]) {
              const f32x2 s0 = scl_unpack(o[i].x), s1 = scl_unpack(o[i].y);
              const f32x4 sv = {s0.x, s0.y, s1.x, s1.y};
              ss[i] += sv;
              qq[i] += sv * sv;
            }
          }
          if (okf[f]) scl_store<TM>(of + so, o);
        }
      }
      if constexpr (EPI == SCL_HEAD) {
        char* ob = a.dst + (((size_t)t.n * a.H + t.y0) * a.W + t.x0) * CB;
// ... 27 lines not shown
            }
          }
          if (okf[f]) scl_store<TM>(of + so, oo);
        }
      }
      if constexpr (EPI == SCL_BNB_SUM2) {
        char* ob = a.dst + (((size_t)t.n * (a.H >> 1) + (t.y0 >> 1)) * (a.W >> 1) + (t.x0 >> 1)) * CB;
#pragma unroll
        for (int h2 = 0; h2 < 2; ++h2) {
          char* of = ob + (size_t)(h2 * 8 * CB);
          const bool mine = own && okf[h2];
          u32x2 oo[TM];
#pragma unroll
          for (int i = 0; i < TM; ++i) {
            f32x4 v = acc[i][h2] + acc[i][h2 + 2];
#pragma unroll
            for (int e = 0; e < 4; ++e)
              v[e] += __int_as_float(__builtin_amdgcn_update_dpp(0, __float_as_int(v[e]), 0xB1, 0xf, 0xf, true));
            u32x2& o = oo[i];
#pragma unroll
            for (int e = 0; e < 2; ++e) {
              const uint32_t stw = pack_bf16x2(v[2 * e], v[2 * e + 1]);
              const f32x2 dy = scl_unpack(stw), xv = scl_unpack(xp[i][h2][e]);
              const f32x2 tt = __builtin_elementwise_fma(xv, ksc[i][e], ksh[i][e]);
              const f32x2 g = {mine && __builtin_amdgcn_fmed3f(tt.x, alo, ahi) == tt.x ? dy.x : 0.f,
                               mine && __builtin_amdgcn_fmed3f(tt.y, alo, ahi) == tt.y ? dy.y : 0.f};
              ss[i][2 * e] += g.x; ss[i][2 * e + 1] += g.y;
              qq[i][2 * e] = fmaf(g.x, xv.x, qq[i][2 * e]); qq[i][2 * e + 1] = fmaf(g.y, xv.y, qq[i][2 * e + 1]);
              o[e] = pack_bf16x2(g.x, g.y);
            }
          }
          if (mine) scl_store<TM>(of + so, oo);
        }
      }
    };
    if (edge) epilogue(true); else epilogue(false);
    {
      const uint32_t flip = cur ? (uint32_t)(-BUF) : (uint32_t)BUF;
#pragma unroll
      for (int ar = 0; ar < NA; ++ar)
#pragma unroll
        for (int c = 0; c < NCH; ++c) bla[ar][c] += flip;
    }
    if constexpr (AHEAD) {
#pragma unroll
      for (int i = 0; i < TM; ++i)
#pragma unroll
        for (int f = 0; f < 4; ++f) xp[i][f] = xn[i][f];
    }
  }

  if (EPI != SCL_HEAD && a.stats) {
    if constexpr (EPI == SCL_BNB || EPI == SCL_BNB_SUM2) {
#pragma unroll
      for (int i = 0; i < TM; ++i) {
        const int cb = TM == 2 ? lg * 8 + i * 4 : i * 16 + lg * 4;
        const f32x4 mu = *reinterpret_cast<const f32x4*>(a.bnb.mean + cb), rsd = *reinterpret_cast<const f32x4*>(a.bnb.rstd + cb);
#pragma unroll
        for (int e = 0; e < 4; ++e) qq[i][e] = rsd[e] * (qq[i][e] - mu[e] * ss[i][e]);
      }
    }
#pragma unroll
    for (int i = 0; i < TM; ++i)
#pragma unroll
      for (int e = 0; e < 4; ++e) {
        const float sv = row_sum16_to_lane15(ss[i][e]), qv = row_sum16_to_lane15(qq[i][e]);
        if (lr == 15) {
          const int cl = (TM == 2 ? lg * 8 + i * 4 : i * 16 + lg * 4) + e;
          red[(wave * TM * 16 + cl) * 2] = sv;
          red[(wave * TM * 16 + cl) * 2 + 1] = qv;
        }
      }
    lds_barrier();
    if (tid < TM * 16) {
      float sv = 0.f, qv = 0.f;
#pragma unroll
      for (int w = 0; w < 4; ++w) { sv += red[(w * TM * 16 + tid) * 2]; qv += red[(w * TM * 16 + tid) * 2 + 1]; }
      a.stats[(size_t)tid * gridDim.x + blockIdx.x] = sv;
      a.stats[((size_t)COUT + tid) * gridDim.x + blockIdx.x] = qv;
    }
  }
}

template <int CIN, int TM, int EPI, bool PBN, bool UP>
static int launch_scl(const ScArgs& a, hipStream_t s) {
  const int ntiles = a.N * a.tiles_x * a.tiles_y;
  constexpr int NV = (UP ? (SC_TH / 2 + 2) * (SC_TW / 2 + 2) : SC_HH * SC_HW) * (CIN / 8), NPASS = (NV + 255) / 256;
  const size_t lds = (size_t)2 * NPASS * 4096 + (4 * TM * 16 * 2 + 64) * sizeof(float);
  const int blocks = sc_stream_blocks(STP_H16, CIN, TM * 16, ntiles);
  static bool attr_set = false;
  if (lds > 64 * 1024 && !attr_set) {
    if (hipFuncSetAttribute(reinterpret_cast<const void*>(conv_sc_lean_kernel<CIN, TM, EPI, PBN, UP>), hipFuncAttributeMaxDynamicSharedMemorySize, (int)lds) != hipSuccess)
      return STP_E_LAUNCH;
    attr_set = true;
  }
  hipLaunchKernelGGL((conv_sc_lean_kernel<CIN, TM, EPI, PBN, UP>), dim3(blocks), dim3(256), lds, s, a);
  STP_LAUNCH_CHECK();
  return STP_OK;
}

template <int EPI, bool PBN, bool UP>
static int dispatch_scl2(const ScArgs& a, int cin, int tm, hipStream_t s) {
  switch (cin * 4 + tm) {
    case 8 * 4 + 1: return launch_scl<8, 1, EPI, PBN, UP>(a, s);
    case 16 * 4 + 1: return launch_scl<16, 1, EPI, PBN, UP>(a, s);
    case 32 * 4 + 1: return launch_scl<32, 1, EPI, PBN, UP>(a, s);
    case 8 * 4 + 2: if constexpr (EPI != SCL_HEAD) return launch_scl<8, 2, EPI, PBN, UP>(a, s); else return 1;
    case 16 * 4 + 2: if constexpr (EPI != SCL_HEAD) return launch_scl<16, 2, EPI, PBN, UP>(a, s); else return 1;
    case 32 * 4 + 2: if constexpr (EPI != SCL_HEAD) return launch_scl<32, 2, EPI, PBN, UP>(a, s); else return 1;
    default: return 1;
  }
}
template <int EPI, bool PBN>
static int dispatch_scl(const ScArgs& a, int cin, int tm, hipStream_t s) {
  if (a.up) {
    if constexpr (EPI == SCL_STATS) return dispatch_scl2<EPI, PBN, true>(a, cin, tm, s); else return 1;
  }
  return dispatch_scl2<EPI, PBN, false>(a, cin, tm, s);
}

static bool sc_lean_on() {
  static const bool on = !(getenv("STP_SC_LEAN") && atoi(getenv("STP_SC_LEAN")) == 0);
  return on;
}

int sc_lean_launch(const ScArgs& a, int cin, int dtype, hipStream_t s) {
  if (!sc_lean_on() || !sc_stream_on() || dtype != STP_H16 || a.stat_slots || a.accumulate || a.relu) return 1;
  const bool pbn = a.pbn.mean != nullptr;
  const int tm = a.Cout <= 16 ? 1 : 2;
  if (a.bnb.x) {
    if (pbn || a.bias || !a.stats || a.Cout != tm * 16) return 1;
    return a.sum2 ? dispatch_scl<SCL_BNB_SUM2, false>(a, cin, tm, s) : dispatch_scl<SCL_BNB, false>(a, cin, tm, s);
  }
  if (a.sum2) return 1;
  if (a.Cout == 1) {
    if (a.stats) return 1;
    return pbn ? dispatch_scl<SCL_HEAD, true>(a, cin, 1, s) : dispatch_scl<SCL_HEAD, false>(a, cin, 1, s);
  }
  if (a.bias || a.Cout != tm * 16) return 1;
  return pbn ? dispatch_scl<SCL_STATS, true>(a, cin, tm, s) : dispatch_scl<SCL_STATS, false>(a, cin, tm, s);
}

template <int CIN, int COUT, bool PBN, bool UP>
__global__ __launch_bounds__(256) void conv_sc_wgrad_lean_kernel(const ScWgArgs a) {
  typedef bf16_t T;
  constexpr int SZ = 2, VEC = 8, TMo = (COUT + 15) / 16, TNi = CIN / 16, PIXB = CIN * SZ, DYB = COUT * SZ;
  constexpr int VPPX = CIN / VEC, VPPD = COUT / VEC;
  constexpr int HH = UP ? SC_TH / 2 + 2 : SC_HH, HW = UP ? SC_TW / 2 + 2 : SC_HW;
  constexpr int NVX = HH * HW * VPPX, NPX = (NVX + 255) / 256;
  constexpr int NVD = SC_TH * SC_TW * VPPD, NPD = (NVD + 255) / 256;
  constexpr int XBUF = NPX * 4096, DBUF = NPD * 4096, BUF = XBUF + DBUF;
  constexpr int F3 = 3 * TMo * TNi;
  static_assert(4 * F3 * 1024 <= 2 * BUF, "the final reduction of a filter row fits the (dead) staging buffers");

  extern __shared__ __attribute__((aligned(16))) char smem[];
  const int tid = threadIdx.x, lane = tid & 63;
  const int wave = __builtin_amdgcn_readfirstlane(tid >> 6);
  const int lr = lane & 15, lg = lane >> 4;
  constexpr int sh = UP ? 1 : 0;

  int t_first, t_step, t_end;
  if ((gridDim.x & 7) == 0) {
    const int q = a.ntiles >> 3, r = a.ntiles & 7, x = blockIdx.x & 7;
    const int start = x < r ? x * (q + 1) : r * (q + 1) + (x - r) * q;
    t_first = start + (int)(blockIdx.x >> 3); t_step = (int)(gridDim.x >> 3); t_end = start + q + (x < r ? 1 : 0);
  } else {
    t_first = (int)blockIdx.x; t_step = (int)gridDim.x; t_end = a.ntiles;
  }

  f32x4 acc[9][TMo][TNi];
#pragma unroll
  for (int t = 0; t < 9; ++t)
#pragma unroll
    for (int i = 0; i < TMo; ++i)
#pragma unroll
      for (int j = 0; j < TNi; ++j) acc[t][i][j] = f32x4{0.f, 0.f, 0.f, 0.f};

  if (t_first < t_end) {
    const __amdgpu_buffer_rsrc_t rsx = __builtin_amdgcn_make_buffer_rsrc((void*)a.src, 0, a.src_bytes, 0x00020000);
    const __amdgpu_buffer_rsrc_t rsd = __builtin_amdgcn_make_buffer_rsrc((void*)a.dy, 0, a.dy_bytes, 0x00020000);
    int hyx[NPX], pyx[NPD];
    uint32_t lox[NPX], lod[NPD];
    const uint32_t cvx = (uint32_t)(tid % VPPX) * 16u, cvd = (uint32_t)(tid % VPPD) * 16u;
#pragma unroll
    for (int p = 0; p < NPX; ++p) {
      const int v = p * 256 + tid, pix = v / VPPX;
      const int hy = pix / HW, hx = pix - hy * HW;
      hyx[p] = v < NVX ? (hy << 16 | hx) : -1;
      lox[p] = v < NVX ? (uint32_t)(((hy - 1) * a.Ws + (hx - 1)) * PIXB) + cvx : 0x80000000u;
    }
#pragma unroll
    for (int p = 0; p < NPD; ++p) {
      const int v = p * 256 + tid, pix = v / VPPD;
      const int py = pix / SC_TW, px = pix % SC_TW;
      pyx[p] = v < NVD ? (py << 16 | px) : -1;
      lod[p] = v < NVD ? (uint32_t)((py * a.W + px) * DYB) + cvd : 0x80000000u;
    }
    auto decode = [&](int tile) -> TileC {
      int b = tile;
      const int tx = b % a.tiles_x; b /= a.tiles_x;
      const int ty = b % a.tiles_y;
      TileC t;
      t.n = b / a.tiles_y; t.y0 = ty * SC_TH; t.x0 = tx * SC_TW;
      t.interior = ty > 0 && tx > 0 && t.y0 + SC_TH < a.H && t.x0 + SC_TW < a.W;
      return t;
    };
    auto issue_tile = [&](const TileC& t, int bsel, bool live) -> uint32_t {
      uint32_t inside = 0;
      char* xb = smem + bsel * BUF;
      if (live && t.interior) {
        const uint32_t tbx = (uint32_t)((t.n * a.Hs + (t.y0 >> sh)) * a.Ws + (t.x0 >> sh)) * (uint32_t)PIXB;
        const uint32_t tbd = (uint32_t)((t.n * a.H + t.y0) * a.W + t.x0) * (uint32_t)DYB;
#pragma unroll
        for (int p = 0; p < NPX; ++p)
          __builtin_amdgcn_raw_ptr_buffer_load_lds(rsx, (__attribute__((address_space(3))) void*)(xb + p * 4096 + wave * 1024), 16, (int)(tbx + lox[p]), 0, 0, 0);
#pragma unroll
        for (int p = 0; p < NPD; ++p)
          __builtin_amdgcn_raw_ptr_buffer_load_lds(rsd, (__attribute__((address_space(3))) void*)(xb + XBUF + p * 4096 + wave * 1024), 16, (int)(tbd + lod[p]), 0, 0, 0);
        inside = (1u << NPX) - 1u;
      } else {
#pragma unroll
        for (int p = 0; p < NPX; ++p) {
          const int gy = (t.y0 >> sh) - 1 + (hyx[p] >> 16), gx = (t.x0 >> sh) - 1 + (hyx[p] & 0xffff);
          const bool ok = live && hyx[p] >= 0 && (unsigned)gy < (unsigned)a.Hs && (unsigned)gx < (unsigned)a.Ws;
          const uint32_t off = ok ? (uint32_t)((t.n * a.Hs + gy) * a.Ws + gx) * (uint32_t)PIXB + cvx : 0x80000000u;
          inside |= ok ? (1u << p) : 0u;
          __builtin_amdgcn_raw_ptr_buffer_load_lds(rsx, (__attribute__((address_space(3))) void*)(xb + p * 4096 + wave * 1024), 16, (int)off, 0, 0, 0);
        }
#pragma unroll
        for (int p = 0; p < NPD; ++p) {
          const int gy = t.y0 + (pyx[p] >> 16), gx = t.x0 + (pyx[p] & 0xffff);
          const bool ok = live && pyx[p] >= 0 && gy < a.H && gx < a.W;
          const uint32_t off = ok ? (uint32_t)((t.n * a.H + gy) * a.W + gx) * (uint32_t)DYB + cvd : 0x80000000u;
          __builtin_amdgcn_raw_ptr_buffer_load_lds(rsd, (__attribute__((address_space(3))) void*)(xb + XBUF + p * 4096 + wave * 1024), 16, (int)off, 0, 0, 0);
        }
      }
      return inside;
    };

    TileC tc = decode(t_first);
    uint32_t inside_cur = issue_tile(tc, 0, true);
    ScStageBn<T> sbn;
    if (PBN) sbn.load(a.pbn, (tid % VPPX) * VEC);
    const int xl = lg * 4 + (lr >> 2), qb = (lr & 3) * 8;
    const uint32_t aA0 = (uint32_t)(uintptr_t)smem + (uint32_t)(XBUF + ((2 * wave * SC_TW + xl) * COUT) * SZ + qb);
    uint32_t aB0[3];
#pragma unroll
    for (int kw = 0; kw < 3; ++kw)
      aB0[kw] = (uint32_t)(uintptr_t)smem + (uint32_t)((UP ? (wave * HW + ((xl + kw + 1) >> 1)) : ((2 * wave) * HW + xl + kw)) * CIN * SZ + qb);

    int cur = 0;
    for (int tile = t_first; tile < t_end; tile += t_step, cur ^= 1) {
      __builtin_amdgcn_s_waitcnt(0x0f70);
      asm volatile("" ::: "memory");
      if (PBN) {
#pragma unroll
        for (int p0 = 0; p0 < NPX; p0 += 3) {
          u32x4 v[3];
#pragma unroll
          for (int q = 0; q < 3; ++q)
            if (p0 + q < NPX) v[q] = *reinterpret_cast<const u32x4*>(smem + cur * BUF + ((p0 + q) * 256 + tid) * 16);
#pragma unroll
          for (int q = 0; q < 3; ++q)
            if (p0 + q < NPX && (inside_cur & (1u << (p0 + q))))
              *reinterpret_cast<u32x4*>(smem + cur * BUF + ((p0 + q) * 256 + tid) * 16) = sbn.apply(v[q], a.pbn.relu);
        }
      }
      lds_barrier();
      const int next = tile + t_step;
      const bool live = next < t_end;
      if (live) tc = decode(next);
      inside_cur = issue_tile(tc, cur ^ 1, live);

      const uint32_t aA = aA0 + (uint32_t)(cur * BUF);
      uint32_t aB[3];
#pragma unroll
      for (int kw = 0; kw < 3; ++kw) aB[kw] = aB0[kw] + (uint32_t)(cur * BUF);
      u32x2 fa[2][TMo][2];
      u32x2 fb[2][3][TNi][2];
      sc_unroll<2 * TMo * 2>([&fa, aA](auto kc) {
        constexpr int k = decltype(kc)::value, r = k / (TMo * 2), i = (k / 2) % TMo, hl = k & 1;
        asm volatile("ds_read_b64_tr_b16 %0, %1 offset:%2" : "=v"(fa[r][i][hl]) : "v"(aA), "n"((r * SC_TW * COUT + i * 16 + hl * 16 * COUT) * SZ));
      });
      auto issue_b = [&fb, &aB](auto hc) {
        constexpr int h = decltype(hc)::value;
        sc_unroll<3 * TNi * 2>([&fb, &aB](auto kc) {
          constexpr int k = decltype(kc)::value, kw = k / (TNi * 2), j = (k / 2) % TNi, hl = k & 1;
          constexpr int OFF = UP ? ((((h + 1) >> 1) * HW + hl * 8) * CIN + j * 16) * SZ : ((h * HW + hl * 16) * CIN + j * 16) * SZ;
          asm volatile("ds_read_b64_tr_b16 %0, %1 offset:%2" : "=v"(fb[h & 1][kw][j][hl]) : "v"(aB[kw]), "n"(OFF));
        });
      };
      issue_b(std::integral_constant<int, 0>{});
      sc_unroll<4>([&](auto hc) {
        constexpr int h = decltype(hc)::value;
        if constexpr (h < 3) issue_b(std::integral_constant<int, h + 1>{});
        asm volatile("s_waitcnt lgkmcnt(%0)" ::"n"(h < 3 ? 3 * TNi * 2 : 0) : "memory");
        if constexpr (h == 0) {
#pragma unroll
          for (int r = 0; r < 2; ++r)
#pragma unroll
            for (int i = 0; i < TMo; ++i) { asm volatile("" : "+v"(fa[r][i][0])); asm volatile("" : "+v"(fa[r][i][1])); }
        }
#pragma unroll
        for (int kw = 0; kw < 3; ++kw)
#pragma unroll
          for (int j = 0; j < TNi; ++j) { asm volatile("" : "+v"(fb[h & 1][kw][j][0])); asm volatile("" : "+v"(fb[h & 1][kw][j][1])); }
#pragma unroll
        for (int r = 0; r < 2; ++r) {
          const int kh = h - r;
          if (kh < 0 || kh > 2) continue;
#pragma unroll
          for (int kw = 0; kw < 3; ++kw)
#pragma unroll
            for (int j = 0; j < TNi; ++j) {
              const u32x4 vb = {fb[h & 1][kw][j][0].x, fb[h & 1][kw][j][0].y, fb[h & 1][kw][j][1].x, fb[h & 1][kw][j][1].y};
#pragma unroll
              for (int i = 0; i < TMo; ++i) {
                const u32x4 va = {fa[r][i][0].x, fa[r][i][0].y, fa[r][i][1].x, fa[r][i][1].y};
                acc[kh * 3 + kw][i][j] = mfma16_16x16x32(va, vb, acc[kh * 3 + kw][i][j]);
              }
            }
        }
      });
    }
  }

  float* out = a.slabs + (size_t)blockIdx.x * a.Cout * (9 * a.ctot);
  f32x4* rbuf = reinterpret_cast<f32x4*>(smem);
  __builtin_amdgcn_s_waitcnt(0x0f70);
#pragma unroll
  for (int kh = 0; kh < 3; ++kh) {
    lds_barrier();
#pragma unroll
    for (int kw = 0; kw < 3; ++kw)
#pragma unroll
      for (int i = 0; i < TMo; ++i)
#pragma unroll
        for (int j = 0; j < TNi; ++j) rbuf[(wave * F3 + (kw * TMo + i) * TNi + j) * 64 + lane] = acc[kh * 3 + kw][i][j];
    lds_barrier();
    for (int f = wave; f < F3; f += 4) {
      const f32x4 s01 = rbuf[(0 * F3 + f) * 64 + lane] + rbuf[(1 * F3 + f) * 64 + lane];
      const f32x4 s23 = rbuf[(2 * F3 + f) * 64 + lane] + rbuf[(3 * F3 + f) * 64 + lane];
      const f32x4 v = s01 + s23;
      const int kw = f / (TMo * TNi), i = (f / TNi) % TMo, j = f % TNi;
#pragma unroll
      for (int r = 0; r < 4; ++r) {
        const int co = i * 16 + lg * 4 + r;
        if (co < a.Cout) out[(size_t)co * (9 * a.ctot) + (kh * 3 + kw) * a.ctot + a.coff + j * 16 + lr] = v[r];
      }
    }
  }
}

template <int CIN, int COUT, bool PBN, bool UP>
static int launch_scwl(const ScWgArgs& a, int blocks, hipStream_t s) {
  constexpr int NPX = ((UP ? (SC_TH / 2 + 2) * (SC_TW / 2 + 2) : SC_HH * SC_HW) * (CIN / 8) + 255) / 256, NPD = (SC_TH * SC_TW * (COUT / 8) + 255) / 256;
  const size_t lds = (size_t)2 * (NPX + NPD) * 4096;
  static bool attr_set = false;
  if (lds > 64 * 1024 && !attr_set) {
    if (hipFuncSetAttribute(reinterpret_cast<const void*>(conv_sc_wgrad_lean_kernel<CIN, COUT, PBN, UP>), hipFuncAttributeMaxDynamicSharedMemorySize, (int)lds) != hipSuccess)
      return STP_E_LAUNCH;
    attr_set = true;
  }
  hipLaunchKernelGGL((conv_sc_wgrad_lean_kernel<CIN, COUT, PBN, UP>), dim3(blocks), dim3(256), lds, s, a);
  STP_LAUNCH_CHECK();
  return STP_OK;
}

static bool sc_wg_lean_3232() {
  static const bool on = getenv("STP_SC_WG_LEAN_3232") && atoi(getenv("STP_SC_WG_LEAN_3232")) != 0;
  return on;
}

template <bool PBN, bool UP>
static int dispatch_scwl(const ScWgArgs& a, int cin, int cout, int blocks, hipStream_t s) {
  switch (cin * 64 + cout) {
    case 16 * 64 + 8: return launch_scwl<16, 8, PBN, UP>(a, blocks, s);
    case 16 * 64 + 16: return launch_scwl<16, 16, PBN, UP>(a, blocks, s);
    case 16 * 64 + 32: return launch_scwl<16, 32, PBN, UP>(a, blocks, s);
    case 32 * 64 + 8: return launch_scwl<32, 8, PBN, UP>(a, blocks, s);
    case 32 * 64 + 16: return launch_scwl<32, 16, PBN, UP>(a, blocks, s);
    case 32 * 64 + 32: if (UP || sc_wg_lean_3232()) return launch_scwl<32, 32, PBN, UP>(a, blocks, s); else return 1;
    default: return 1;
  }
}

int sc_wg_lean_launch(const ScWgArgs& a, int cin, int cout, int dtype, int blocks, hipStream_t s) {
  if (!sc_lean_on() || !sc_stream_on() || dtype != STP_H16 || !a.src_bytes || !a.dy_bytes) return 1;
  if (a.up) return a.pbn.mean ? dispatch_scwl<true, true>(a, cin, cout, blocks, s) : dispatch_scwl<false, true>(a, cin, cout, blocks, s);
  return a.pbn.mean ? dispatch_scwl<true, false>(a, cin, cout, blocks, s) : dispatch_scwl<false, false>(a, cin, cout, blocks, s);
}

constexpr int STL_VPR = 35, STL_NV = ST_HH * STL_VPR, STL_NPASS = (STL_NV + 255) / 256, STL_BUF = STL_NPASS * 4096, STL_ROW = STL_VPR * 16;
constexpr int STL_LDS = ST_WBYTES + 2 * STL_BUF + 4 * 64 * 2 * 4;

__global__ __launch_bounds__(256, 2) void conv_stem_lean_kernel(const StemArgs a) {
  constexpr int TM = 4, NCH = 7, K = 224, COUT = 64;
  extern __shared__ __attribute__((aligned(16))) char smem[];
  char* const wl = smem;
  char* const hb = smem + ST_WBYTES;
  float* const red = reinterpret_cast<float*>(smem + ST_WBYTES + 2 * STL_BUF);
  const int tid = threadIdx.x, lane = tid & 63;
  const int wave = __builtin_amdgcn_readfirstlane(tid >> 6);
  const int lr = lane & 15, lg = lane >> 4;

  const int ntiles = a.N * a.tiles_x * a.tiles_y;
  int t_first, t_step, t_end;
  if ((gridDim.x & 7) == 0) {
    const int q = ntiles >> 3, r = ntiles & 7, x = blockIdx.x & 7;
    const int start = x < r ? x * (q + 1) : r * (q + 1) + (x - r) * q;
    t_first = start + (int)(blockIdx.x >> 3); t_step = (int)(gridDim.x >> 3); t_end = start + q + (x < r ? 1 : 0);
  } else {
    t_first = (int)blockIdx.x; t_step = (int)gridDim.x; t_end = ntiles;
  }
  f32x4 ss[TM], qq[TM];
#pragma unroll
  for (int i = 0; i < TM; ++i) { ss[i] = f32x4{0.f, 0.f, 0.f, 0.f}; qq[i] = f32x4{0.f, 0.f, 0.f, 0.f}; }

  if (t_first < t_end) {
    const __amdgpu_buffer_rsrc_t rs = __builtin_amdgcn_make_buffer_rsrc((void*)a.src, 0, a.src_bytes, 0x00020000);
    int hyx[STL_NPASS];
    uint32_t lo[STL_NPASS];
#pragma unroll
    for (int p = 0; p < STL_NPASS; ++p) {
      const int v = p * 256 + tid, hy = v / STL_VPR, vx = v - hy * STL_VPR;
      hyx[p] = v < STL_NV ? (hy << 16 | vx) : -1;
      lo[p] = v < STL_NV ? (uint32_t)((hy * a.W + 2 * vx) * 8) : 0x80000000u;
    }
    auto decode = [&](int tile) -> TileC {
      const int bq = (int)fdiv((uint32_t)tile, a.divTx);
      const int tx = tile - bq * a.tiles_x;
      const int n = (int)fdiv((uint32_t)bq, a.divTy);
      const int ty = bq - n * a.tiles_y;
      TileC t;
      t.n = n; t.y0 = ty * SC_TH; t.x0 = tx * SC_TW;
      t.interior = 2 * t.y0 >= 3 && 2 * t.x0 >= 4 && 2 * t.y0 + 17 < a.H && 2 * t.x0 + 65 < a.W && t.y0 + SC_TH <= a.Ho && t.x0 + SC_TW <= a.Wo;
      return t;
    };
    auto issue_tile = [&](const TileC& t, int b, bool live) {
      if (live && t.interior) {
        const uint32_t tb = (uint32_t)(((t.n * a.H + 2 * t.y0 - 3) * a.W + 2 * t.x0 - 4) * 8);
#pragma unroll
        for (int p = 0; p < STL_NPASS; ++p)
          __builtin_amdgcn_raw_ptr_buffer_load_lds(rs, (__attribute__((address_space(3))) void*)(hb + b * STL_BUF + p * 4096 + wave * 1024), 16, (int)(tb + lo[p]), 0, 0, 0);
      } else {
#pragma unroll
        for (int p = 0; p < STL_NPASS; ++p) {
          const int gy = 2 * t.y0 - 3 + (hyx[p] >> 16), gx = 2 * t.x0 - 4 + 2 * (hyx[p] & 0xffff);
          const bool ok = live && hyx[p] >= 0 && (unsigned)gy < (unsigned)a.H && (unsigned)gx < (unsigned)a.W;
          const uint32_t off = ok ? (uint32_t)(((t.n * a.H + gy) * a.W + gx) * 8) : 0x80000000u;
          __builtin_amdgcn_raw_ptr_buffer_load_lds(rs, (__attribute__((address_space(3))) void*)(hb + b * STL_BUF + p * 4096 + wave * 1024), 16, (int)off, 0, 0, 0);
        }
      }
    };
    TileC tc = decode(t_first);
    issue_tile(tc, 0, true);
    for (int v = tid; v < COUT * (K / 8); v += 256) {
      const int co = v / (K / 8), q = v - co * (K / 8);
      const int slot = ((co >> 5) * 2 + ((co >> 2) & 1)) * 16 + ((co >> 3) & 3) * 4 + (co & 3);
      *reinterpret_cast<u32x4*>(wl + (q * COUT + slot) * 16) = *reinterpret_cast<const u32x4*>(a.weight + ((size_t)co * K + q * 8) * 2);
    }
    const uint32_t wa = (uint32_t)(uintptr_t)wl + (uint32_t)((lg * COUT + lr) * 16);
    uint32_t ba = (uint32_t)(uintptr_t)hb + (uint32_t)((4 * wave) * STL_ROW + (2 * lr + 2 * lg + 1) * 8);
    const uint32_t so = (uint32_t)(((wave * 2) * a.Wo + lr) * (COUT * 2) + lg * 16);
#if defined(STP_STEM_WAIT_LATE)
    __builtin_amdgcn_s_waitcnt(0x0f70);
    asm volatile("" ::: "memory");
#endif

    int cur = 0;
    bool prev_full = false;
// ... 300 lines not shown
```

segmentation_training_pipeline_amd/graph.py:

```python
import os
import ctypes as C
from collections import OrderedDict

import numpy as np
import torch

from . import _lib, ops

_TD = {"bf16": torch.bfloat16, "fp16": torch.float16, "fp32": torch.float32}


class StpShapeError(ValueError):
    pass


def _rup(a, b):
    return (a + b - 1) // b * b


class DT(object):
    __slots__ = ("name", "N", "H", "W", "C", "buf", "grad", "_grad_ready", "grad_writes", "needs_grad", "gradC", "meta")

    def __init__(self, name, N, H, W, Cn, buf=None, needs_grad=False):
        self.name, self.N, self.H, self.W, self.C = name, N, H, W, Cn
# ... 257 lines not shown
    @staticmethod
    def _set_src_bn(p, bn):
        p.src_bn_mean, p.src_bn_rstd, p.src_bn_gamma, p.src_bn_beta, p.src_bn_relu = bn[1:]

    @staticmethod
    def _set_bnb(q, bn):
        q.bnb_x, q.bnb_mean, q.bnb_rstd, q.bnb_gamma, q.bnb_beta, q.bnb_relu = bn or (None, None, None, None, None, 0)

    def _fuse_bn_into_consumers(self):
        drop, kept = set(), set()
        for t in self.tensors.values():
            rec, sc, halo = t.meta.get("apply_rec"), t.meta.get("sc_consumers") or [], t.meta.get("halo_consumers") or []
            if rec is None or not (sc or halo) or len(sc) + len(halo) != t.meta.get("uses", 0):
                continue
            bn = t.meta["bn"]
            halo_full = bool(halo) and all(ok for _, _, ok in halo)
            for cp, wp in sc + [h[:2] for h in halo]:
                cp.src0 = bn[0]
                self._set_src_bn(cp, bn)
                if not halo or halo_full:
                    self._set_src_bn(wp, bn)
            if halo and not halo_full:
                kept.add(id(rec))
            else:
                t.meta["deferred"] = rec
                t.meta["src_override"] = bn[0]
                drop.add(id(rec))
        self.fwd = [r for r in self.fwd if id(r) not in drop]
        return kept

    def _fuse_bn_finalize(self, keep=()):
        if os.environ.get("STP_BN_FUSE_FINALIZE", "1") == "0":
            return
        out, i, fwd = [], 0, self.fwd
        while i < len(fwd):
            r = fwd[i]
            nxt = fwd[i + 1] if i + 1 < len(fwd) else None
            if (r[2] == "stp_bn_finalize" and nxt is not None and nxt[2] == "stp_bn_apply" and id(nxt) not in keep
                    and nxt[1][7] == r[1][6] and nxt[1][8] == r[1][7] and nxt[1][1] == nxt[1][3] == self.cdt and nxt[1][5] == nxt[1][6] == r[1][3]
                    and nxt[1][12] == 0.0):
                part, tiles, rows, Cn, eps, mom, mean, rstd, mm, mv = r[1]
                x, _, y, _, rows2, _, _, _, _, gp, beta, relu, _ = nxt[1]
                if rows2 == rows and int(self.lib.stp_bn_finalize_apply_ok(self.cdt, rows, Cn, tiles)):
                    out.append((self.lib.stp_bn_finalize_apply, (part, tiles, x, y, self.cdt, rows, Cn, eps, mom, mean, rstd, mm, mv, gp, beta, relu),
                                "stp_bn_finalize_apply", None))
                    i += 2
                    continue
            out.append(r)
            i += 1
        self.fwd = out

    def tensor(self, name):
        t = self.tensors[name]
        rec = t.meta.get("deferred")
        if rec is not None:
            fn, args = rec[0], rec[1]
            rc = fn(*args, torch.cuda.current_stream().cuda_stream)
            if rc != 0:
                raise _lib.StpError("%s failed with %d" % (rec[2], rc))
        return t

    def _scratch(self, nbytes):
        nbytes = int(nbytes)
        if nbytes <= 0:
            return None, 0
        buf = self._alloc((nbytes // 4,), torch.float32)
        return buf.data_ptr(), nbytes

    def _group_stats(self, p, st, Cs):
        cols = int(self.lib.stp_conv2d_stats_floats(C.byref(p))) // (2 * Cs)
        G = int(self.lib.stp_conv2d_stats_group_for(C.byref(p)))
        if G < 2:
            return st, cols
        ng = -(-cols // G)
        out = self._alloc((2 * Cs * ng,), torch.float32)
        cnt = torch.zeros((max(1, int(self.lib.stp_conv2d_stats_group_counters(C.byref(p), G))),), dtype=torch.int32, device=self.device)
        self._keep.append(cnt)
        p.stats_group_out, p.stats_group_counters, p.stats_group = out.data_ptr(), cnt.data_ptr(), G
        return out, ng

    def _emit_conv(self, lst, p, meta=None):
        self._keep.append(p)
        if meta is not None and meta.get("tile") == 512:
            meta = dict(meta, sc=(int(p.C0), 1 if p.Cout <= 16 else 2))
        if meta is not None and meta.get("tile") == 800:
            meta = dict(meta, pw=(int(p.C0), int(p.Cout)))
        lst.append((self.lib.stp_conv2d, (C.byref(p),), "stp_conv2d", meta))

    def _emit_wgrad(self, p, name, flops, defer_hi=0):
        lst = self.bwd
        self._keep.append(p)
        meta = {"layer": name, "pass": "wgrad", "flops": flops, "cout": p.Cout, "sc": bool(self.lib.stp_wgrad_sc_eligible(C.byref(p))),
                "kernel_id": int(self.lib.stp_conv2d_wgrad_kernel_id(C.byref(p)))}
        if defer_hi > 0 and self.reduce_batch > 0:
            db = int(self.lib.stp_wgrad_reduce_desc_bytes())
            wsb = int(self.lib.stp_conv2d_wgrad_workspace_bytes(C.byref(p)))
            ws = self._alloc((max(wsb // 4, 4) + 4,), torch.float32)
            desc = (C.c_char * db)()
            count = int(self.lib.stp_wgrad_reduce_desc_fill(C.addressof(desc), 0, C.byref(p), ws.data_ptr()))
            if count > 0:
                lst.append((self.lib.stp_conv2d_wgrad_partial, (C.byref(p), ws.data_ptr(), ws.numel() * 4, 0), "stp_conv2d_wgrad", meta))
                self._pending_reduces.append((bytes(desc), count))
                self._pending_reduce_hi = max(self._pending_reduce_hi, int(defer_hi))
                if len(self._pending_reduces) >= self.reduce_batch:
                    self._flush_reduces()
                return
            self._keep = [t for t in self._keep if t is not ws]
        lst.append((self.lib.stp_conv2d_wgrad_partial, (C.byref(p), self.ws_wgrad.data_ptr(), self.ws_wgrad.numel() * 4, 0),
                    "stp_conv2d_wgrad", meta))
        lst.append((self.lib.stp_conv2d_wgrad_reduce, (C.byref(p), self.ws_wgrad.data_ptr(), 0), "stp_conv2d_wgrad_reduce", None))

    def _flush_reduces(self):
        if not self._pending_reduces:
            return
        table = b"".join(d for d, _ in self._pending_reduces)
        dev = self._table(table)
        n, maxc = len(self._pending_reduces), max(c for _, c in self._pending_reduces)
        self.bwd.append((self.lib.stp_wgrad_reduce_batched, (dev.data_ptr(), n, maxc), "stp_wgrad_reduce_batched", {"layers": n}))
        self._pending_reduces, self._pending_reduce_hi = [], 0

    def _flush_wgroup(self):
        if not self._wgroup:
            return
        layers, cls = self._wgroup, self._wgroup_cls
        self._wgroup, self._wgroup_cls, self._wgroup_flops, self._wgroup_hi, self._wgroup_reads = [], 0, 0.0, 0, set()
        n = len(layers)
        lone_group = cls == 128 and 0 < self.wgrad_lone_group_gflop * 1e9 <= layers[0][2]
        if n == 1 and cls != 32 and not lone_group:
            self._emit_wgrad(*layers[0])
            return
        arr = (C.POINTER(_lib.WgradParams) * n)(*[C.pointer(wp) for wp, _, _ in layers])
        tb = int(self.lib.stp_wgrad_group_table_bytes(arr, n))
        wsb = int(self.lib.stp_wgrad_group_workspace_bytes(arr, n))
        if tb <= 0 or wsb <= 0:
            raise StpShapeError("grouped weight gradient: the layers %s do not form a group" % [nm for _, nm, _ in layers])
        host = (C.c_char * tb)()
        _lib.check(self.lib.stp_wgrad_group_build(arr, n, C.addressof(host), tb), "stp_wgrad_group_build")
        dev = self._table(bytes(host))
        ws = self._alloc((wsb // 4,), torch.float32)
        self._keep += [arr, host] + [wp for wp, _, _ in layers]
        names = [nm for _, nm, _ in layers]
        self.wgroups.append((names, cls))
        hdr = (C.c_int32 * 16).from_buffer_copy(bytes(host)[:64])
        meta = {"layer": "group[%d]:%s..%s" % (n, names[0], names[-1]), "pass": "wgrad", "flops": sum(f for _, _, f in layers), "cout": cls,
                "bm": cls, "layers": names, "taps9": int(hdr[15]), "pbn": int(hdr[14])}
        self.bwd.append((self.lib.stp_wgrad_group_partial, (C.addressof(host), dev.data_ptr(), ws.data_ptr(), wsb), "stp_wgrad_group_partial", meta))
        self.bwd.append((self.lib.stp_wgrad_group_reduce, (C.addressof(host), dev.data_ptr(), ws.data_ptr()), "stp_wgrad_group_reduce", None))

    def input_u8(self, name, H, W, Cn):
        t = DT(name, self.N, H, W, Cn, None if self.dry else self._alloc((self.N, H, W, Cn), torch.uint8))
        self.inputs[name] = t
        return t

    def input_bn(self, name, x, eps):
        if x.C > 7:
            raise StpShapeError("input_bn handles up to 7 image channels")
        Cp = 4 if x.C <= 3 else 8
        beta = self.param(name + "/beta", (x.C,), "beta")
        mm = self.state(name + "/moving_mean", x.C, 0.0)
        mv = self.state(name + "/moving_variance", x.C, 1.0)
        out = self._new(name, x.H, x.W, Cp, False)
        out.meta["real_c"] = x.C
        out.meta["input_bn_beta"] = beta
        if self.dry:
            return out
        if self.training:
            mean, rstd = self._alloc((x.C,), torch.float32), self._alloc((x.C,), torch.float32)
# ... 621 lines not shown
            self._emit(self.bwd, "stp_maxpool2x2_bwd", idx.data_ptr(), out.grad.data_ptr(), self._gradbuf(x).data_ptr(), self.N,
                       x.H, x.W, x.C, self.cdt, int(x.grad_ready))
            x.grad_ready = True

        if self.training:
            self._tape.append(back)
        return out

    def maxpool(self, name, x):
        Ho, Wo = (x.H + 2 - 3) // 2 + 1, (x.W + 2 - 3) // 2 + 1
        out = self._new(name, Ho, Wo, x.C, x.needs_grad)
        self._use(x)
        if self.dry:
            return out
        idx = self._alloc((self.N, Ho, Wo, x.C), torch.uint8) if self.training else None
        last = self.fwd[-1] if self.fwd else None
        if (self.training and self.dtype != "fp32" and last is not None and last[2] == "stp_bn_apply" and last[1][2] == x.buf.data_ptr()
                and last[1][1] == last[1][3] == self.cdt and last[1][5] == last[1][6] == x.C and last[1][12] == 0.0 and x.C % 8 == 0
                and x.H % 2 == 0 and x.W % 2 == 0 and x.meta.get("apply_rec") in (None, last) and not x.meta.get("sc_consumers")
                and not x.meta.get("halo_consumers") and os.environ.get("STP_FUSE_BN_POOL_FWD", "1") != "0"):
            xa = last[1]
            self.fwd.pop()
            x.meta.pop("apply_rec", None)
            self._emit(self.fwd, "stp_bn_apply_maxpool3x3s2", xa[0], x.buf.data_ptr(), out.buf.data_ptr(), idx.data_ptr() if idx is not None else None,
                       self.N, x.H, x.W, x.C, self.cdt, xa[7], xa[8], xa[9], xa[10], xa[11])
        else:
            self._emit(self.fwd, "stp_maxpool3x3s2", x.buf.data_ptr(), out.buf.data_ptr(), idx.data_ptr() if idx is not None else None,
                       self.N, x.H, x.W, x.C, self.cdt)

        def back():
            if not (x.needs_grad and out.grad_ready):
                return
            acc = int(x.grad_ready)
            self._emit_grad_pass("stp_maxpool3x3s2_bwd", x, acc, (self.N, x.H, x.W, x.C, self.cdt),
                                 (idx.data_ptr(), out.grad.data_ptr(), self._gradbuf(x).data_ptr(), self.N, x.H, x.W, x.C, self.cdt, acc),
                                 os.environ.get("STP_FUSE_POOL_BN", "0") == "1")
            x.grad_ready = True

        if self.training:
            self._tape.append(back)
        return out

    def _emit_loss(self, name, logits, target, dims, weights, tail=()):
        dl = self._gradbuf(logits) if self.training else None
        if len(weights) == 5:
            self._loss_weights = (C.c_float * 5)(*weights)
            weights = (C.addressof(self._loss_weights),)
        else:
            weights = tuple(float(w) for w in weights)
        self._emit(self.fwd, name, logits.buf.data_ptr(), target.buf.data_ptr(), *dims, self.cdt, *weights, self.loss_scalars.data_ptr(),
                   dl.data_ptr() if dl is not None else None, logits.gradC, float(self.loss_scale), self.ws_loss.data_ptr(),
                   self.ws_loss.numel() * 4, *tail)
        if self.training and self.dls is not None:
            self._emit(self.fwd, "stp_scale_by_device", dl.data_ptr(), logits.rows * logits.gradC, self.cdt, self.dls.data_ptr(), self.dls.data_ptr() + 16)
        return dl

    def _emit_confusion(self, rows, target, factor=0, ignore_label=None):
        if not self.class_metrics:
            return
        classes = rows.C
        nb = int(self.lib.stp_class_confusion_workspace_bytes(classes))
        if nb <= 0:
            raise StpShapeError("class metrics need a head of 2..32 classes")
        self.class_counts = self._alloc((classes * classes,), torch.int32)
        ws = self._alloc((nb // 4,), torch.int32)
        if factor:
            self._emit(self.fwd, "stp_class_confusion_up", rows.buf.data_ptr(), target.buf.data_ptr(), self.N, rows.H, rows.W, factor, classes,
                       rows.C, self.cdt, self.class_counts.data_ptr(), ws.data_ptr(), nb)
        elif ignore_label is not None:
            self._emit(self.fwd, "stp_class_confusion_ignore", rows.buf.data_ptr(), target.buf.data_ptr(), rows.rows, classes, rows.C, self.cdt,
                       self.class_counts.data_ptr(), ws.data_ptr(), nb, int(ignore_label))
        else:
            self._emit(self.fwd, "stp_class_confusion", rows.buf.data_ptr(), target.buf.data_ptr(), rows.rows, classes, rows.C, self.cdt,
                       self.class_counts.data_ptr(), ws.data_ptr(), nb)

    def sigmoid_loss(self, logits, target, w_bce, w_dice, w_iou=0.0, w_jaccard=0.0, w_focal=0.0, w_lovasz=0.0):
        if logits.C != 1:
            raise StpShapeError("binary loss expects one class")
        if self.dry:
            return
        self.loss_scalars = self._alloc((16,), torch.float32)
        self.loss_scalars.zero_()
        count = logits.rows
        if w_iou or w_jaccard or w_focal:
            dl = self._emit_loss("stp_sigmoid_loss_ex", logits, target, (count,), (w_bce, w_dice, w_iou, w_jaccard, w_focal))
        else:
            dl = self._emit_loss("stp_sigmoid_bce_dice", logits, target, (count,), (w_bce, w_dice))
        logits.meta["loss_bias_grad"] = bool(self.training and not w_lovasz and self.dls is None)
        if w_lovasz:
            if self.training and self.loss_scale != 1.0:
                raise StpShapeError("lovasz_loss has no loss-scaling form: use loss_scale=1 (or bf16) with it")
            nbytes = int(self.lib.stp_lovasz_workspace_bytes(count, self.N))
            if nbytes <= 0:
                raise StpShapeError("lovasz_loss: the sort workspace cannot be sized (no device)")
            self.ws_lovasz = torch.empty(nbytes, dtype=torch.uint8, device=self.device)
            self._emit(self.fwd, "stp_lovasz_hinge", logits.buf.data_ptr(), target.buf.data_ptr(), self.N, count // self.N, self.cdt,
                       float(w_lovasz), self.loss_scalars.data_ptr(), dl.data_ptr() if dl is not None else None, logits.gradC,
                       self.ws_lovasz.data_ptr(), nbytes)
        logits.grad_ready = self.training

    def sigmoid_multilabel_loss(self, logits, target, w_bce, w_dice, w_iou=0.0, w_jaccard=0.0, w_focal=0.0):
        if not 2 <= logits.C <= 8:
            raise StpShapeError("multi-label loss expects 2..8 classes")
        if self.dry:
            return
        self.loss_scalars = self._alloc((16,), torch.float32)
        self.loss_scalars.zero_()
        self._emit_loss("stp_sigmoid_multilabel_loss", logits, target, (logits.rows, logits.C, logits.C), (w_bce, w_dice, w_iou, w_jaccard, w_focal))
        logits.meta["loss_bias_grad"] = "multilabel" if (self.training and self.dls is None) else False
        logits.grad_ready = self.training

    def softmax_loss(self, logits, target, w_cce, w_dice, w_iou=0.0, w_jaccard=0.0, w_focal=0.0):
        if logits.C < 2:
            raise StpShapeError("categorical loss expects at least two classes")
        if self.dry:
            return
        opts = self.masked_loss or {}
        ignore_label, class_weights = opts.get("ignore_label"), opts.get("class_weights")
        masked = ignore_label is not None or class_weights is not None
        if masked or w_iou or w_jaccard or w_focal:
            name, tail, ign = "stp_softmax_loss_ex", (), None
            if masked:
                if logits.C > 32:
                    raise StpShapeError("ignore_label / class_weights need a head of 2..32 classes")
                ign = -1 if ignore_label is None else int(ignore_label)
                cw = None
                if class_weights is not None:
                    if len(class_weights) != logits.C:
                        raise StpShapeError("class_weights: %d weights for %d classes" % (len(class_weights), logits.C))
                    cw = self._alloc((logits.C,), torch.float32)
                    cw.copy_(torch.tensor([float(w) for w in class_weights], dtype=torch.float32))
                self.class_weights = cw
                name, tail = "stp_softmax_loss_masked", (ign, cw.data_ptr() if cw is not None else None)
            self.loss_scalars = self._alloc((16,), torch.float32)
            self.loss_scalars.zero_()
            self._emit_loss(name, logits, target, (logits.rows, logits.C, logits.C), (w_cce, w_dice, w_iou, w_jaccard, w_focal), tail=tail)
            self._emit_confusion(logits, target, ignore_label=ign)
            logits.grad_ready = self.training
            return
        self.loss_scalars = self._alloc((12,), torch.float32)
        rec = logits.meta.get("resize_rec")
        if (self.training and rec is not None and self.fwd[rec[0]][2] == "stp_resize_bilinear" and rec[1].needs_grad
                and not rec[1].grad_ready and target.buf.data_ptr() % 4 == 0
                and self.lib.stp_softmax_cce_dice_up_ok(rec[2], logits.C, self.cdt)
                and (not self.class_metrics or self.lib.stp_class_confusion_up_ok(rec[2], logits.C, self.cdt))):
            idx, lo, f = rec
            logits.meta["deferred"] = (self.fwd[idx][0], self.fwd[idx][1], self.fwd[idx][2])
            self.fwd[idx] = (None, (), "fused:resize->loss", None)
            nb = int(self.lib.stp_softmax_cce_dice_up_corner_bytes(self.N, lo.H, lo.W, logits.C))
            corners = self._alloc((nb // 4,), torch.float32)
            dlow = self._gradbuf(lo)
            dls = self.dls.data_ptr() if self.dls is not None else None
            self._emit(self.fwd, "stp_softmax_cce_dice_up", lo.buf.data_ptr(), target.buf.data_ptr(), self.N, lo.H, lo.W, f, logits.C, lo.C,
                       self.cdt, float(w_cce), float(w_dice), self.loss_scalars.data_ptr(), dlow.data_ptr(), lo.gradC, float(self.loss_scale),
                       dls, (dls + 16) if dls is not None else None, self.ws_loss.data_ptr(), self.ws_loss.numel() * 4, corners.data_ptr(), nb)
            self._emit_confusion(lo, target, f)
            lo.grad_ready = True
            logits.grad_ready = False
            logits.meta["fused_into_loss"] = True
            return
        self._emit_loss("stp_softmax_cce_dice", logits, target, (logits.rows, logits.C, logits.C), (w_cce, w_dice))
        self._emit_confusion(logits, target)
        logits.grad_ready = self.training

    def softmax_out(self, logits):
        if self.dry:
# ... 40 lines not shown
            elif name == "stp_lovasz_hinge" and done:
                a = list(args)
                a[2] = n_valid
                _lib.check(fn(*a, st), name)
        if not done:
            raise _lib.StpError("the plan has no loss launch")
        self.rerun_confusion(n_valid)

    def rerun_confusion(self, n_valid):
        n_valid = int(n_valid)
        if not 0 < n_valid <= self.N:
            raise ValueError("n_valid out of range")
        st = torch.cuda.current_stream().cuda_stream
        for fn, args, name, _meta in self.fwd:
            if name in ("stp_class_confusion", "stp_class_confusion_up", "stp_class_confusion_ignore"):
                a = list(args)
                a[2] = n_valid if name.endswith("_up") else args[2] // self.N * n_valid
                _lib.check(fn(*a, st), name)

    def init_states(self):
        for name, (off, numel, init) in self.states.items():
            self.S[off:off + numel] = init

    def set_trainable_mask(self):
        self.mask.fill_(1)
        for info in self.params.values():
            if not info.trainable:
                self.mask[info.offset:info.offset + info.numel] = 0


class Dgrad(object):

    def __init__(self, q, layer, s2d=False, fold1=False, folded_up=False, two_dest=False, collapsed=False):
        self.q, self.s2d, self.fold1, self.folded_up, self.two_dest = q, s2d, fold1, folded_up, two_dest
        self.C1 = 0 if collapsed else layer.C1
        self.flops = layer.flops * (layer.C0 - 0.0) / (layer.C0 + layer.C1) if collapsed else layer.flops


class ConvLayer(object):

    def __init__(self, plan, name, x, Cout, k, stride, pad, src1, upsample, residual, transpose, relu, same_tf, fold_shortcut, param_cols):
        if transpose:
            if stride != 1 or upsample or src1 is not None or residual is not None or k % 2:
                raise StpShapeError("transpose=True is the plain stride-2 'same' Conv2DTranspose with an even kernel")
            pad = k - 1 - (k // 2 - 1)
        real_c0 = x.meta.get("real_c", x.C)
        stem = real_c0 != x.C
        if stem and (src1 is not None or upsample):
            raise StpShapeError("padded-channel input supports a plain conv only")
        C0, C1 = x.C, (src1.C if src1 is not None else 0)
        if not stem and (C0 % plan.vec or C1 % plan.vec):
            raise StpShapeError("%s: input channels (%d,%d) must be multiples of %d for dtype %s" % (name, C0, C1, plan.vec, plan.dtype))
        Hv, Wv = (2 * x.H, 2 * x.W) if upsample else ((2 * x.H - 1, 2 * x.W - 1) if transpose else (x.H, x.W))
        if src1 is not None and (src1.H, src1.W) != (Hv, Wv):
            raise StpShapeError("%s: skip tensor is %dx%d, expected %dx%d" % (name, src1.H, src1.W, Hv, Wv))
        Ho, Wo = (Hv + 2 * pad - k) // stride + 1, (Wv + 2 * pad - k) // stride + 1
        if same_tf:
            Ho, Wo = -(-Hv // stride), -(-Wv // stride)
            pad = max((Ho - 1) * stride + k - Hv, 0) // 2
            if max((Wo - 1) * stride + k - Wv, 0) // 2 != pad:
                raise StpShapeError("%s: 'same' padding differs between height and width" % name)
        self.KWp = k + (k & 1) if (stem and x.C == 4) else k
        self.plan, self.name, self.x, self.src1, self.residual, self.fs, self.param_cols = plan, name, x, src1, residual, fold_shortcut, param_cols
        self.Cout, self.k, self.stride, self.pad, self.upsample, self.transpose, self.relu = Cout, k, stride, pad, upsample, transpose, relu
        self.real_c0, self.stem, self.C0, self.C1, self.Hv, self.Wv, self.Ho, self.Wo = real_c0, stem, C0, C1, Hv, Wv, Ho, Wo
        self.Cin_master, self.Cinp = real_c0 + C1, C0 + C1
        self.src_mode = ops.SRC_NEAREST2X if upsample else (ops.SRC_ZEROINS2X if transpose else ops.SRC_DIRECT)

    def declare(self, param_name, param_shape, cout_pad, bias):
        pl, name, x, src1, residual, Cout, k, Cin_master, param_cols = self.plan, self.name, self.x, self.src1, self.residual, self.Cout, self.k, self.Cin_master, self.param_cols
        if param_cols is not None:
            if k != 1 or self.stem or self.transpose or self.C1 or Cout % pl.vec or Cin_master % 4 or param_cols[0] % 4 or param_cols[1] % 4 \
                    or param_cols[0] + Cin_master > param_cols[1]:
                raise StpShapeError("%s: a column range of a shared kernel serves a plain 1x1 convolution with aligned channel counts" % name)
            param_shape = None
        w = pl.param((param_name or name) + "/kernel", (Cout, 1, 1, param_cols[1]) if param_cols is not None else (param_shape or (Cout, k, k, Cin_master)),
                     "tkernel" if self.transpose else "kernel")
        if param_shape is not None and int(np.prod(param_shape)) != Cout * k * k * Cin_master:
            raise StpShapeError("%s: parameter view of %s does not match %d x %d x %d x %d" % (name, param_shape, Cout, k, k, Cin_master))
        self.w, self.b = w, (pl.param(name + "/bias", (Cout,), "bias") if bias else None)
        CoutB = self.CoutB = _rup(Cout, cout_pad or pl.vec)
        self.x_ng, self.s_ng = x.needs_grad, (src1.needs_grad if src1 is not None else False)
        self.out = pl._new(name, self.Ho, self.Wo, Cout, self.x_ng or self.s_ng or w.trainable or (residual is not None and residual.needs_grad))
        self.out.gradC = CoutB
        if bias:
            pl._bn_ws_c = max(pl._bn_ws_c, CoutB)
        pl._use(x, src1, residual)
        wp = self.wp = _lib.WgradParams()
        wp.N, wp.Hs0, wp.Ws0, wp.Hv, wp.Wv, wp.C0, wp.C1, wp.src0_mode = pl.N, x.H, x.W, self.Hv, self.Wv, self.C0, self.C1, self.src_mode
        wp.KH, wp.KW, wp.stride, wp.pad, wp.Ho, wp.Wo, wp.Cout = k, self.KWp, self.stride, self.pad, self.Ho, self.Wo, CoutB
        wp.accumulate, wp.dtype, wp.splits = 0, pl.cdt, 0
        if pl.training and w.trainable:
            pl._wg_ws_bytes = max(pl._wg_ws_bytes, int(pl.lib.stp_conv2d_wgrad_workspace_bytes(C.byref(wp))))

    def forward(self, bn_stats, flops_as):
        pl, x, src1, residual, out, k, Cout = self.plan, self.x, self.src1, self.residual, self.out, self.k, self.Cout
        self._weight_copies()
        p = self.p = ops.conv_params(x.buf, self.wf, out.buf, N=pl.N, Hs0=x.H, Ws0=x.W, Hv=self.Hv, Wv=self.Wv, C0=self.C0, C1=self.C1,
                                     src1=src1.buf if src1 is not None else None,
                                     mode=self.src_mode, KH=k, KW=self.KWp, stride=self.stride, pad=self.pad,
                                     Ho=self.Ho, Wo=self.Wo, Cout=Cout, dtype=pl.cdt, residual=residual.buf if residual is not None else None)
        self._collapsed_copies()
        self._register_bn_consumer()
        if self.b is not None:
            p.bias = pl._pptr(self.b)
        if self.relu:
            if self.CoutB != Cout:
                raise StpShapeError("%s: a fused ReLU needs Cout to be a multiple of %d" % (self.name, pl.vec))
            p.relu = 1
        if bn_stats and pl.training and pl.slot_arena is not None and pl.N * self.Ho * self.Wo <= pl.bn_slots_max_rows:
            p.stats_partial, p.stats_slots = out.meta["stats_slots"] = pl._slots(Cout)
        elif bn_stats and pl.training:
            nfl = int(pl.lib.stp_conv2d_stats_floats(C.byref(p)))
            st = pl._alloc((max(nfl, 4),), torch.float32)
            p.stats_partial = st.data_ptr()
            out.meta["stats_table"] = pl._group_stats(p, st, Cout)
        self.flops = 2.0 * pl.N * self.Ho * self.Wo * Cout * k * k * self.Cin_master / (4.0 if self.transpose else 1.0)
        if flops_as is not None:
            self.flops = float(flops_as)
        pl._emit_conv(pl.fwd, p, {"layer": self.name, "pass": "fwd", "flops": self.flops, "tile": int(pl.lib.stp_conv2d_tile_for(C.byref(p))),
                                  "src2": bool(self.C1 or self.upsample)})

    def _weight_copies(self):
        pl, w, Cout, k, KWp, Cinp, Cin_master, param_cols = self.plan, self.w, self.Cout, self.k, self.KWp, self.Cinp, self.Cin_master, self.param_cols
        wf = self.wf = pl._alloc((_rup(Cout, 16) * k * KWp * Cinp,))
        self.need_dgrad = pl.training and (self.x_ng or self.s_ng) and not self.stem
        wb = self.wb = pl._alloc((_rup(Cinp, 16) * k * k * self.CoutB,)) if self.need_dgrad else None
        self.out.meta["wb"] = wb
        wsrc = pl._pptr(w)
        if param_cols is not None:
            w.pending_slices += 1
            wm = pl._alloc((Cout * Cin_master,), torch.float32)
            pl._emit(pl.prep, "stp_copy_cols_f32", wm.data_ptr(), Cin_master, wsrc + 4 * int(param_cols[0]), int(param_cols[1]), Cout, Cin_master, 0)
            wsrc = wm.data_ptr()
        self.out.meta["w_master"] = (wsrc, Cout, Cin_master, k)
        pl._prep_layers.append((wsrc, wf.data_ptr(), wb.data_ptr() if wb is not None else None, Cout, k, k, Cin_master, KWp, Cinp, self.CoutB))

    def _collapsed_copies(self):
        pl, p, C0, C1, rows_f = self.plan, self.p, self.C0, self.C1, _rup(self.Cout, 16)
        self.w4 = None
        if not (self.upsample and self.src1 is not None and self.k == 3 and self.KWp == 3 and self.stride == 1 and self.pad == 1
                and self.Cinp == self.Cin_master == C0 + C1
                and os.environ.get("STP_UPCOLLAPSE", "1") != "0" and not pl.lib.stp_conv2d_scn_eligible(C.byref(p))
                and int(pl.lib.stp_conv2d_halo_variant(C.byref(p))) < 0):
            return
        wup = pl._alloc((rows_f * 16 * C0,))
        pl._upc_layers.append((pl._pptr(self.w), wup.data_ptr(), self.Cout, rows_f, C0, C0 + C1))
        p.weight_up = wup.data_ptr()
        if self.need_dgrad and self.x_ng and C0 % 16 == 0 and os.environ.get("STP_UPCOLLAPSE_BWD", "0") == "1":
            self.w4 = pl._alloc((C0 * 16 * self.CoutB,))
            pl._upc4_layers.append((pl._pptr(self.w), self.w4.data_ptr(), self.Cout, self.CoutB, C0, C0 + C1))

    def _register_bn_consumer(self):
        pl, x, p, wp, w = self.plan, self.x, self.p, self.wp, self.w
        if not pl.training or x.meta.get("apply_rec") is None or self.src1 is not None or self.transpose or self.stem:
            return
        if self.residual is None and pl.lib.stp_conv2d_sc_eligible(C.byref(p)) and (not w.trainable or pl.lib.stp_wgrad_sc_eligible(C.byref(wp))):
            x.meta["sc_consumers"].append((p, wp))
        elif pl.fuse_bn_halo and not self.upsample and pl.lib.stp_conv2d_halo_variant(C.byref(p)) >= 0:
            x.meta["halo_consumers"].append((p, wp, (not w.trainable) or int(pl.lib.stp_conv2d_wgrad_kernel_id(C.byref(wp))) in (2, 3)))

    def backward(self):
        pl, out, residual, b = self.plan, self.out, self.residual, self.b
        if not out.needs_grad or not out.grad_ready:
            return
        dy = self.dy = out.grad
        if self.relu:
            pl._guard_write(dy)
            pl._emit(pl.bwd, "stp_relu_bwd", out.buf.data_ptr(), dy.data_ptr(), out.rows * out.gradC, pl.cdt)
        if residual is not None and residual.needs_grad:
            if not residual.grad_ready and residual.gradC == out.gradC:
                residual.grad = dy
                residual.grad_ready = True
            else:
                pl._emit(pl.bwd, "stp_add_inplace", pl._gradbuf(residual).data_ptr(), dy.data_ptr(), out.rows * out.gradC, pl.cdt)
        if self.w.trainable:
            self._weight_grad()
        if b is not None and b.trainable and out.meta.get("loss_bias_grad") and self.Cout == 1:
            pl._emit(pl.bwd, "stp_sigmoid_loss_bias_grad", pl.ws_loss.data_ptr(), out.rows, pl._gptr(b), 0)
        elif b is not None and b.trainable and out.meta.get("loss_bias_grad") == "multilabel":
            pl._emit(pl.bwd, "stp_sigmoid_multilabel_bias_grad", pl.ws_loss.data_ptr(), out.rows, self.Cout, pl._gptr(b), 0)
        elif b is not None and b.trainable:
            pl._emit_bias_grad(dy, out.rows, self.CoutB, self.Cout, b)
        if self.need_dgrad and not out.meta.get("dgrad_folded"):
            self._data_grad()

    def _weight_grad(self):
        pl, x, src1, w, wp, k, Cout, Cin_master, param_cols = self.plan, self.x, self.src1, self.w, self.wp, self.k, self.Cout, self.Cin_master, self.param_cols
        padded, gcols = self.stem or self.CoutB != Cout, None
        if padded:
            dwp = pl._alloc((self.CoutB * k * self.KWp * self.Cinp,), torch.float32)
            wp.dw = dwp.data_ptr()
        elif param_cols is not None:
            gcols = pl._alloc((Cout * Cin_master,), torch.float32)
            wp.dw = gcols.data_ptr()
        else:
            wp.dw = pl._gptr(w)
        wp.src0, wp.src1, wp.dy = x.meta.get("src_override") or x.buf.data_ptr(), (src1.buf.data_ptr() if src1 is not None else None), self.dy.data_ptr()
        cls = int(pl.lib.stp_wgrad_group_class(C.byref(wp))) if (pl.wgrad_group_gflop > 0 and not padded and gcols is None) else 0
        if cls:
            self._wgrad_join_group(cls)
        else:
            pl._flush_wgroup()
            pl._emit_wgrad(wp, self.name, self.flops, defer_hi=0 if (padded or gcols is not None) else w.end)
        if gcols is not None:
            w.pending_slices -= 1
            gbase = pl._gptr(w) if w.pending_slices == 0 else pl.G.data_ptr() + 4 * w.offset
            pl._emit(pl.bwd, "stp_copy_cols_f32", gbase + 4 * int(param_cols[0]), int(param_cols[1]), gcols.data_ptr(), Cin_master, Cout, Cin_master, 0)
        if padded:
            pl._emit(pl.bwd, "stp_weight_grad_unpad", dwp.data_ptr(), pl._gptr(w), Cout, k, k, Cin_master, self.KWp, self.Cinp, 0)
        beta = x.meta.get("input_bn_beta")
        if self.stem and beta is not None and beta.trainable:
            pl._emit(pl.bwd, "stp_stem_beta_grad", dwp.data_ptr(), pl._pptr(w), pl._gptr(beta), Cout, k, k, self.real_c0, self.KWp, self.Cinp, self.real_c0)

    def _wgrad_join_group(self, cls):
        pl = self.plan
        if pl._wgroup and pl._wgroup_cls != cls:
            pl._flush_wgroup()
        pl._wgroup.append((self.wp, self.name, self.flops))
        pl._wgroup_cls = cls
        pl._wgroup_flops += self.flops
        pl._wgroup_hi = max(pl._wgroup_hi, self.w.end)
        pl._wgroup_reads.add(self.dy.data_ptr())
        if pl._wgroup_flops >= pl.wgrad_group_gflop * 1e9:
            pl._flush_wgroup()

    def _data_grad(self):
        pl, x = self.plan, self.x
        self._dgrad_dests()
        q = self._dgrad_plain()
        if self.stride not in (1, 2):
            raise StpShapeError("data gradient supports stride 1 and 2")
        if self._form_scatter():
            return
        form = (self._form_s2d() or self._form_parity_fold(q) or self._form_fold1(q) or self._form_collapsed()
                or self._form_sum2x2_stream(q) or self._form_sum2x2_halo(q) or Dgrad(q, self))
        if form.folded_up and self.d0_hires is not None:
            pl._keep = [t for t in pl._keep if t is not self.d0_hires]
            self.d0 = self.d0_hires = None
        self._attach_bn_sums(form)
        pl._emit_conv(pl.bwd, form.q, {"layer": self.name, "pass": "dgrad", "flops": form.flops,
                                       "tile": int(pl.lib.stp_conv2d_tile_for(C.byref(form.q))), "s2d": form.s2d, "fold1": form.fold1})
        if self.upsample and self.x_ng and not form.folded_up:
            acc = int(x.grad_ready)
            pl._emit_grad_pass("stp_upsample2x_bwd", x, acc, (pl.N, x.H, x.W, self.C0, self.C0, pl.cdt),
                               (self.d0.data_ptr(), pl._gradbuf(x).data_ptr(), pl.N, x.H, x.W, self.C0, self.C0, pl.cdt, acc),
                               os.environ.get("STP_FUSE_UP_BN", "1") != "0")
        if self.x_ng:
            x.grad_ready = True
        if self.s_ng:
            self.src1.grad_ready = True

    def _dgrad_dests(self):
        pl, x, src1, shape = self.plan, self.x, self.src1, (self.plan.N, self.Hv, self.Wv)
        self.d0_hires = None
        if self.upsample:
            d0 = self.d0_hires = pl._alloc(shape + (self.C0,)) if self.x_ng else None
            self.acc0 = 0
        else:
            d0 = pl._gradbuf(x) if self.x_ng else None
            self.acc0 = int(x.grad_ready)
        d1 = pl._gradbuf(src1) if self.s_ng else None
        self.acc1 = int(src1.grad_ready) if self.s_ng else 0
        if d0 is None:
            d0 = pl._alloc(shape + (self.C0,))
        if self.C1 and d1 is None:
            d1 = pl._alloc(shape + (self.C1,))
        self.d0, self.d1 = d0, d1

    def _dgrad_plain(self):
        pl, x, k, stride, Ho, Wo, C0 = self.plan, self.x, self.k, self.stride, self.Ho, self.Wo, self.C0
        if self.transpose:
            return ops.conv_params(self.dy, self.wb, self.d0, N=pl.N, Hs0=Ho, Ws0=Wo, Hv=Ho, Wv=Wo, C0=self.CoutB, mode=ops.SRC_DIRECT, KH=k, KW=k,
                                   stride=2, pad=k - 1 - self.pad, Ho=x.H, Wo=x.W, Cout=C0, dtype=pl.cdt, accumulate0=self.acc0)
        return ops.conv_params(self.dy, self.wb, self.d0, N=pl.N, Hs0=Ho, Ws0=Wo,
                               Hv=(2 * Ho - 1 if stride == 2 else Ho), Wv=(2 * Wo - 1 if stride == 2 else Wo),
                               C0=self.CoutB, mode=(ops.SRC_ZEROINS2X if stride == 2 else ops.SRC_DIRECT), KH=k, KW=k, stride=1,
                               pad=k - 1 - self.pad, Ho=self.Hv, Wo=self.Wv, Cout=C0 + self.C1, dtype=pl.cdt, dst1=self.d1, Cd0=C0,
                               accumulate0=self.acc0, accumulate1=self.acc1)

    def _form_scatter(self):
        pl, x, N, Ho, Wo, C0 = self.plan, self.x, self.plan.N, self.Ho, self.Wo, self.C0
        if not (self.stride == 2 and self.k == 1 and self.pad == 0 and not self.transpose and not self.upsample and self.src1 is None and self.x_ng
                and self.fs is None and C0 % 4 == 0 and os.environ.get("STP_SCATTER_1X1S2", "1") != "0"):
            return False
        t_low = pl._alloc((N, Ho, Wo, C0))
        qg = ops.conv_params(self.dy, self.wb, t_low, N=N, Hs0=Ho, Ws0=Wo, Hv=Ho, Wv=Wo, C0=self.CoutB, mode=ops.SRC_DIRECT, KH=1, KW=1,
                             stride=1, pad=0, Ho=Ho, Wo=Wo, Cout=C0, dtype=pl.cdt)
        pl._emit_conv(pl.bwd, qg, {"layer": self.name, "pass": "dgrad", "flops": 2.0 * N * Ho * Wo * self.Cout * self.Cin_master,
                                   "tile": int(pl.lib.stp_conv2d_tile_for(C.byref(qg)))})
        pl._emit_grad_pass("stp_scatter2x_bwd", x, self.acc0, (N, x.H, x.W, C0, pl.cdt),
                           (t_low.data_ptr(), self.d0.data_ptr(), N, x.H, x.W, C0, pl.cdt, self.acc0))
        x.grad_ready = True
        return True

    def _sibling_ready(self):
        fs = self.fs
        return (fs is not None and self.src1 is None and self.x_ng and not self.transpose and fs.needs_grad and fs.grad_ready
                and fs.meta.get("wb") is not None and (fs.H, fs.W) == (self.Ho, self.Wo))

    def _fold_sibling(self):
        self.fs.meta["dgrad_folded"] = True
        self.x.grad_writes += 1

    def _form_s2d(self):
        pl, fs, dy, Ho, Wo, C0, CoutB = self.plan, self.fs, self.dy, self.Ho, self.Wo, self.C0, self.CoutB
        if not (self.stride == 2 and self.k == 3 and self.pad == 1 and not self.transpose and self.src1 is None and self.x_ng and pl.dtype != "fp32"
                and not self.stem and self.Cout == CoutB and C0 == self.Cin_master and (self.Hv, self.Wv) == (2 * Ho, 2 * Wo)
                and os.environ.get("STP_S2D", "1") != "0"
                and os.environ.get("STP_HALO", "1") != "0"):
            return None
        fold = self._sibling_ready() and fs.gradC == CoutB and fs.meta.get("w_master", (0, 0, 0, 0))[1:] == (self.Cout, C0, 1)
        qs = ops.conv_params(dy, dy, self.d0, N=pl.N, Hs0=Ho, Ws0=Wo, Hv=Ho, Wv=Wo, C0=CoutB, C1=(CoutB if fold else 0),
                             src1=(fs.grad if fold else None), mode=ops.SRC_DIRECT, KH=2, KW=2, stride=1, pad=0, Ho=Ho, Wo=Wo,
                             Cout=4 * C0, dtype=pl.cdt, accumulate0=self.acc0)
        qs.s2d_dgrad = 1
        qs.weight = self.wb.data_ptr()
        if fold:
            qs.fold_weight = fs.meta["wb"].data_ptr()
        if int(pl.lib.stp_conv2d_halo_variant(C.byref(qs))) < 0:
            return None
        if fold:
            self._fold_sibling()
        return Dgrad(qs, self, s2d=True)

    def _form_parity_fold(self, q):
        fs = self.fs
        if not (self.stride == 2 and self.k == 3 and self._sibling_ready() and fs.gradC == self.CoutB and int(self.plan.lib.stp_conv2d_fold_ok(C.byref(q)))):
            return None
        q.fold_src, q.fold_weight, q.fold_C = fs.grad.data_ptr(), fs.meta["wb"].data_ptr(), self.CoutB
        self._fold_sibling()
        return Dgrad(q, self)

    def _form_fold1(self, q):
        pl, fs = self.plan, self.fs
        if not (self.stride == 1 and self.k == 3 and self.pad == 1 and not self.upsample and self._sibling_ready()
                and fs.meta.get("w_master", (0, 0, 0, 0))[2:] == (self.C0, 1) and pl.dtype != "fp32" and os.environ.get("STP_HALO", "1") != "0"):
            return None
        c = _lib.ConvParams.from_buffer_copy(q)
        c.fold_src, c.fold_weight, c.fold_C = fs.grad.data_ptr(), fs.meta["wb"].data_ptr(), fs.gradC
        if int(pl.lib.stp_conv2d_halo_variant(C.byref(c))) < 0:
            return None
        self._fold_sibling()
        return Dgrad(c, self, fold1=True)

    def _form_collapsed(self):
        pl, x, dy, wb, k, Ho, Wo, C0, C1, CoutB = self.plan, self.x, self.dy, self.wb, self.k, self.Ho, self.Wo, self.C0, self.C1, self.CoutB
        if self.w4 is None:
            return None
        if self.s_ng:
            q1 = ops.conv_params(dy, wb, self.d1, N=pl.N, Hs0=Ho, Ws0=Wo, Hv=Ho, Wv=Wo, C0=CoutB, mode=ops.SRC_DIRECT, KH=k, KW=k,
                                 stride=1, pad=k - 1 - self.pad, Ho=self.Hv, Wo=self.Wv, Cout=C1, dtype=pl.cdt, accumulate0=self.acc1)
            q1.weight = wb.data_ptr() + C0 * k * k * CoutB * wb.element_size()
            pl._emit_conv(pl.bwd, q1, {"layer": self.name, "pass": "dgrad", "flops": self.flops * C1 / float(C0 + C1),
                                       "tile": int(pl.lib.stp_conv2d_tile_for(C.byref(q1)))})
        q = ops.conv_params(dy, self.w4, pl._gradbuf(x), N=pl.N, Hs0=Ho, Ws0=Wo, Hv=Ho, Wv=Wo, C0=CoutB, mode=ops.SRC_DIRECT,
                            KH=4, KW=4, stride=2, pad=1, Ho=x.H, Wo=x.W, Cout=C0, dtype=pl.cdt, accumulate0=int(x.grad_ready))
        return Dgrad(q, self, folded_up=True, collapsed=True)

    def _form_sum2x2_stream(self, q):
# ... 40 lines not shown
```

Baseline: 2527 images/sec.

## Tile augment kernel with vectorized fast path, reuse pool rows, compact head gradient

Reworks the augment kernel into 2D tiles. A fast path handles the plain RGB case with 4-pixel quads, aligned word loads and packed stores, while other cases fall back to the general per-pixel path. The fused BN+maxpool kernel now carries the last row's activated values into the next output row instead of reloading and recomputing them. The 1-channel head conv's gradient is stored compactly (1 channel instead of padded CoutB), with a compact-dy variant of the wgrad kernel and matching dgrad and bias-grad plumbing. This adds several code paths with eligibility checks that could diverge bitwise or mis-handle edge cases.

Result: no change. 2546 images/sec (median of 6 runs) (+0.8%).

```diff
diff --git a/segmentation_training_pipeline_amd/csrc/augment.hip b/segmentation_training_pipeline_amd/csrc/augment.hip
--- a/segmentation_training_pipeline_amd/csrc/augment.hip
+++ b/segmentation_training_pipeline_amd/csrc/augment.hip
@@ -18,77 +18,174 @@
 
 __device__ __forceinline__ int64_t fix10(double v) { return (int64_t)__double2ll_rn(v); }
 
+__device__ __forceinline__ void aug_pixel_general(const uint8_t* __restrict__ img, const uint8_t* __restrict__ mask, uint8_t* __restrict__ img_out,
+                                                  uint8_t* __restrict__ mask_out, const AugSample& s, int n, int yo, int xo, int64_t i, int Hin,
+                                                  int Win, int Wout, int C, const int32_t* __restrict__ field) {
+  double xd = (double)xo, yd = (double)yo;
+  if (field) {
+    const int32_t f = field[i];
+    xd = __dadd_rn(xd, __dmul_rn((double)(int16_t)(f & 0xffff), 0.015625));
+    yd = __dadd_rn(yd, __dmul_rn((double)(int16_t)(f >> 16), 0.015625));
+  }
+  const int64_t X0 = fix10(__dmul_rn(__dmul_rn((double)s.m[0], xd), 1024.0)) +
+                     fix10(__dmul_rn(__dadd_rn(__dmul_rn((double)s.m[1], yd), (double)s.m[2]), 1024.0));
+  const int64_t Y0 = fix10(__dmul_rn(__dmul_rn((double)s.m[3], xd), 1024.0)) +
+                     fix10(__dmul_rn(__dadd_rn(__dmul_rn((double)s.m[4], yd), (double)s.m[5]), 1024.0));
+  const int64_t X = (X0 + 16) >> 5, Y = (Y0 + 16) >> 5;
+  const int64_t ix = X >> 5, iy = Y >> 5;
+  const int fx = (int)(X & 31), fy = (int)(Y & 31);
+  const int w00 = (32 - fx) * (32 - fy), w01 = fx * (32 - fy), w10 = (32 - fx) * fy, w11 = fx * fy;
+  const bool x0ok = ix >= 0 && ix < Win, x1ok = ix + 1 >= 0 && ix + 1 < Win;
+  const bool y0ok = iy >= 0 && iy < Hin, y1ok = iy + 1 >= 0 && iy + 1 < Hin;
+  const uint8_t* b = img + (int64_t)n * Hin * Win * C;
+  const uint32_t flags = (uint32_t)s.flags, seed = (uint32_t)s.seed, pix = (uint32_t)(yo * Wout + xo);
+  const int noise_k = (int)s.noise_k;
+  const uint32_t drop_t = (uint32_t)s.drop_t;
+  const int ae_lo = (int)s.adde_lo, ae_n = (int)s.adde_hi - ae_lo + 1;
+  int px[4] = {0, 0, 0, 0};
+  for (int c = 0; c < C; ++c) {
+    const int v00 = (x0ok && y0ok) ? b[(iy * Win + ix) * C + c] : 0;
+    const int v01 = (x1ok && y0ok) ? b[(iy * Win + ix + 1) * C + c] : 0;
+    const int v10 = (x0ok && y1ok) ? b[((iy + 1) * Win + ix) * C + c] : 0;
+    const int v11 = (x1ok && y1ok) ? b[((iy + 1) * Win + ix + 1) * C + c] : 0;
+    int v = (w00 * v00 + w01 * v01 + w10 * v10 + w11 * v11 + 512) >> 10;
+    const int cc = c < 3 ? c : 2;
+    v = clip255(v + (int)s.add[cc]);
+    if (s.mul[cc] != 1.f) v = clip255((int)rintf(__fmul_rn((float)v, s.mul[cc])));
+    if (flags & 64u) {
+      const float u = __fmul_rn((float)(aug_hash(seed, pix, (flags & 16u) ? c : 0, 1u) >> 8), 5.9604644775390625e-8f);
+      const float m = __fadd_rn(s.mule_lo, __fmul_rn(__fsub_rn(s.mule_hi, s.mule_lo), u));
+      v = clip255((int)rintf(__fmul_rn((float)v, m)));
+    }
+    if (flags & 32u) v = clip255(v + ae_lo + (int)(aug_hash(seed, pix, (flags & 8u) ? c : 0, 2u) % (uint32_t)ae_n));
+    if (noise_k) {
+      const uint32_t h = aug_hash(seed, pix, (flags & 2u) ? c : 0, 3u);
+      const int sum = (int)(h & 255u) + (int)((h >> 8) & 255u) + (int)((h >> 16) & 255u) + (int)(h >> 24);
+      v = clip255(v + (((sum - 510) * noise_k + 32768) >> 16));
+    }
+    if (drop_t && (aug_hash(seed, pix, (flags & 4u) ? c : 0, 4u) >> 8) < drop_t) v = 0;
+    if (c < 4) px[c] = v;
+    if (C != 3) img_out[i * C + c] = (uint8_t)((flags & 1u) ? 255 - v : v);
+  }
+  if (C == 3) {
+    const int gq = (int)s.gray_q;
+    if (gq) {
+      const int gray = (px[0] * 4899 + px[1] * 9617 + px[2] * 1868 + 8192) >> 14;
+#pragma unroll
+      for (int c = 0; c < 3; ++c) px[c] = (gq * gray + (256 - gq) * px[c] + 128) >> 8;
+    }
+#pragma unroll
+    for (int c = 0; c < 3; ++c) img_out[i * 3 + c] = (uint8_t)((flags & 1u) ? 255 - px[c] : px[c]);
+  }
+  if (mask) {
+    const int64_t mx = (X0 + 512) >> 10, my = (Y0 + 512) >> 10;
+    uint8_t mv = 0;
+    if (mx >= 0 && mx < Win && my >= 0 && my < Hin) mv = mask[((int64_t)n * Hin + my) * Win + mx];
+    mask_out[i] = mv;
+  }
+}
+
+__device__ __forceinline__ void aug_load_2px(const uint8_t* p, int* t) {
+  const uint32_t sh = (uint32_t)((uintptr_t)p & 3);
+  const uint32_t* q = reinterpret_cast<const uint32_t*>(p - sh);
+  const uint32_t d0 = q[0], d1 = q[1], d2 = q[2];
+  const uint32_t lo = __builtin_amdgcn_alignbyte(d1, d0, sh), hi = __builtin_amdgcn_alignbyte(d2, d1, sh);
+  t[0] = (int)(lo & 255u); t[1] = (int)((lo >> 8) & 255u); t[2] = (int)((lo >> 16) & 255u);
+  t[3] = (int)(lo >> 24); t[4] = (int)(hi & 255u); t[5] = (int)((hi >> 8) & 255u);
+}
+
+__device__ __forceinline__ void aug_quad_fast(const uint8_t* __restrict__ img, const uint8_t* __restrict__ mask, uint8_t* __restrict__ img_out,
+                                              uint8_t* __restrict__ mask_out, const AugSample& s, int n, int yo, int xo, int64_t i0, int Hin,
+                                              int Win, int Wout, bool wide) {
+  const double yd = (double)yo;
+  const int64_t RX = fix10(__dmul_rn(__dadd_rn(__dmul_rn((double)s.m[1], yd), (double)s.m[2]), 1024.0));
+  const int64_t RY = fix10(__dmul_rn(__dadd_rn(__dmul_rn((double)s.m[4], yd), (double)s.m[5]), 1024.0));
+  const int add[3] = {(int)s.add[0], (int)s.add[1], (int)s.add[2]};
+  const uint8_t* b = img + (int64_t)n * Hin * Win * 3;
+  const uint8_t* mb = mask ? mask + (int64_t)n * Hin * Win : nullptr;
+  int64_t X0[4], Y0[4];
+  bool inside = wide;
+#pragma unroll
+  for (int p = 0; p < 4; ++p) {
+    const double xd = (double)(xo + p);
+    X0[p] = fix10(__dmul_rn(__dmul_rn((double)s.m[0], xd), 1024.0)) + RX;
+    Y0[p] = fix10(__dmul_rn(__dmul_rn((double)s.m[3], xd), 1024.0)) + RY;
+    const int64_t ix = (X0[p] + 16) >> 10, iy = (Y0[p] + 16) >> 10;
+    inside = inside && ix >= 0 && ix + 1 < Win && iy >= 0 && iy + 2 < Hin;
+  }
+  uint32_t ob[3] = {0u, 0u, 0u}, om = 0u;
+#pragma unroll
+  for (int p = 0; p < 4; ++p) {
+    const int64_t X = (X0[p] + 16) >> 5, Y = (Y0[p] + 16) >> 5;
+    const int64_t ix = X >> 5, iy = Y >> 5;
+    const int fx = (int)(X & 31), fy = (int)(Y & 31);
+    const int w00 = (32 - fx) * (32 - fy), w01 = fx * (32 - fy), w10 = (32 - fx) * fy, w11 = fx * fy;
+    int t0[6], t1[6];
+    if (inside) {
+      const uint8_t* r = b + ((int64_t)iy * Win + ix) * 3;
+      aug_load_2px(r, t0);
+      aug_load_2px(r + (int64_t)Win * 3, t1);
+    } else {
+      const bool x0ok = ix >= 0 && ix < Win, x1ok = ix + 1 >= 0 && ix + 1 < Win;
+      const bool y0ok = iy >= 0 && iy < Hin, y1ok = iy + 1 >= 0 && iy + 1 < Hin;
+#pragma unroll
+      for (int c = 0; c < 3; ++c) {
+        t0[c] = (x0ok && y0ok) ? b[(iy * Win + ix) * 3 + c] : 0;
+        t0[3 + c] = (x1ok && y0ok) ? b[(iy * Win + ix + 1) * 3 + c] : 0;
+        t1[c] = (x0ok && y1ok) ? b[((iy + 1) * Win + ix) * 3 + c] : 0;
+        t1[3 + c] = (x1ok && y1ok) ? b[((iy + 1) * Win + ix + 1) * 3 + c] : 0;
+      }
+    }
+    int mv = 0;
+    if (mb) {
+      const int64_t mx = (X0[p] + 512) >> 10, my = (Y0[p] + 512) >> 10;
+      if (mx >= 0 && mx < Win && my >= 0 && my < Hin) mv = mb[my * Win + mx];
+    }
+    int v[3];
+#pragma unroll
+    for (int c = 0; c < 3; ++c) {
+      v[c] = (w00 * t0[c] + w01 * t0[3 + c] + w10 * t1[c] + w11 * t1[3 + c] + 512) >> 10;
+      v[c] = clip255(v[c] + add[c]);
+      v[c] = clip255((int)rintf(__fmul_rn((float)v[c], s.mul[c])));
+    }
+    if (wide) {
+#pragma unroll
+      for (int c = 0; c < 3; ++c) ob[(p * 3 + c) >> 2] |= (uint32_t)v[c] << (8 * ((p * 3 + c) & 3));
+      om |= (uint32_t)mv << (8 * p);
+    } else if (xo + p < Wout) {
+#pragma unroll
+      for (int c = 0; c < 3; ++c) img_out[(i0 + p) * 3 + c] = (uint8_t)v[c];
+      if (mb) mask_out[i0 + p] = (uint8_t)mv;
+    }
+  }
+  if (wide) {
+    uint32_t* o = reinterpret_cast<uint32_t*>(img_out + i0 * 3);
+    o[0] = ob[0]; o[1] = ob[1]; o[2] = ob[2];
+    if (mb) *reinterpret_cast<uint32_t*>(mask_out + i0) = om;
+  }
+}
+
+#define AUG_TW 64
+#define AUG_TH 16
 __global__ __launch_bounds__(256) void augment_kernel(const uint8_t* __restrict__ img, const uint8_t* __restrict__ mask,
                                                       uint8_t* __restrict__ img_out, uint8_t* __restrict__ mask_out,
                                                       const AugSample* __restrict__ prm, int N, int Hin, int Win, int Hout,
-                                                      int Wout, int C, const int32_t* __restrict__ field) {
-  const int64_t total = (int64_t)N * Hout * Wout;
-  for (int64_t i = (int64_t)blockIdx.x * 256 + threadIdx.x; i < total; i += (int64_t)gridDim.x * 256) {
-    const int xo = (int)(i % Wout);
-    const int yo = (int)((i / Wout) % Hout);
-    const int n = (int)(i / ((int64_t)Wout * Hout));
-    const AugSample s = prm[n];
-    double xd = (double)xo, yd = (double)yo;
-    if (field) {
-      const int32_t f = field[i];
-      xd = __dadd_rn(xd, __dmul_rn((double)(int16_t)(f & 0xffff), 0.015625));
-      yd = __dadd_rn(yd, __dmul_rn((double)(int16_t)(f >> 16), 0.015625));
-    }
-    const int64_t X0 = fix10(__dmul_rn(__dmul_rn((double)s.m[0], xd), 1024.0)) +
-                       fix10(__dmul_rn(__dadd_rn(__dmul_rn((double)s.m[1], yd), (double)s.m[2]), 1024.0));
-    const int64_t Y0 = fix10(__dmul_rn(__dmul_rn((double)s.m[3], xd), 1024.0)) +
-                       fix10(__dmul_rn(__dadd_rn(__dmul_rn((double)s.m[4], yd), (double)s.m[5]), 1024.0));
-    const int64_t X = (X0 + 16) >> 5, Y = (Y0 + 16) >> 5;
-    const int64_t ix = X >> 5, iy = Y >> 5;
-    const int fx = (int)(X & 31), fy = (int)(Y & 31);
-    const int w00 = (32 - fx) * (32 - fy), w01 = fx * (32 - fy), w10 = (32 - fx) * fy, w11 = fx * fy;
-    const bool x0ok = ix >= 0 && ix < Win, x1ok = ix + 1 >= 0 && ix + 1 < Win;
-    const bool y0ok = iy >= 0 && iy < Hin, y1ok = iy + 1 >= 0 && iy + 1 < Hin;
-    const uint8_t* b = img + (int64_t)n * Hin * Win * C;
-    const uint32_t flags = (uint32_t)s.flags, seed = (uint32_t)s.seed, pix = (uint32_t)(yo * Wout + xo);
-    const int noise_k = (int)s.noise_k;
-    const uint32_t drop_t = (uint32_t)s.drop_t;
-    const int ae_lo = (int)s.adde_lo, ae_n = (int)s.adde_hi - ae_lo + 1;
-    int px[4] = {0, 0, 0, 0};
-    for (int c = 0; c < C; ++c) {
-      const int v00 = (x0ok && y0ok) ? b[(iy * Win + ix) * C + c] : 0;
-      const int v01 = (x1ok && y0ok) ? b[(iy * Win + ix + 1) * C + c] : 0;
-      const int v10 = (x0ok && y1ok) ? b[((iy + 1) * Win + ix) * C + c] : 0;
-      const int v11 = (x1ok && y1ok) ? b[((iy + 1) * Win + ix + 1) * C + c] : 0;
-      int v = (w00 * v00 + w01 * v01 + w10 * v10 + w11 * v11 + 512) >> 10;
-      const int cc = c < 3 ? c : 2;
-      v = clip255(v + (int)s.add[cc]);
-      if (s.mul[cc] != 1.f) v = clip255((int)rintf(__fmul_rn((float)v, s.mul[cc])));
-      if (flags & 64u) {
-        const float u = __fmul_rn((float)(aug_hash(seed, pix, (flags & 16u) ? c : 0, 1u) >> 8), 5.9604644775390625e-8f);
-        const float m = __fadd_rn(s.mule_lo, __fmul_rn(__fsub_rn(s.mule_hi, s.mule_lo), u));
-        v = clip255((int)rintf(__fmul_rn((float)v, m)));
+                                                      int Wout, int C, const int32_t* __restrict__ field, int tiles_x, int wide) {
+  const int ty = (int)blockIdx.x / tiles_x, tx = (int)blockIdx.x - ty * tiles_x;
+  for (int n = blockIdx.y; n < N; n += gridDim.y) {
+    const AugSample& s = prm[n];
+    const bool fast = !field && C == 3 && s.flags == 0.f && s.gray_q == 0.f && s.noise_k == 0.f && s.drop_t == 0.f;
+    if (fast) {
+      const int yo = ty * AUG_TH + (int)(threadIdx.x >> 4), xo = tx * AUG_TW + (int)(threadIdx.x & 15) * 4;
+      if (yo < Hout && xo < Wout)
+        aug_quad_fast(img, mask, img_out, mask_out, s, n, yo, xo, ((int64_t)n * Hout + yo) * Wout + xo, Hin, Win, Wout, wide != 0);
+    } else {
+      const int xo = tx * AUG_TW + (int)(threadIdx.x & 63), y0 = ty * AUG_TH + (int)(threadIdx.x >> 6) * 4;
+      for (int r = 0; r < 4; ++r) {
+        const int yo = y0 + r;
+        if (yo < Hout && xo < Wout)
+          aug_pixel_general(img, mask, img_out, mask_out, s, n, yo, xo, ((int64_t)n * Hout + yo) * Wout + xo, Hin, Win, Wout, C, field);
       }
-      if (flags & 32u) v = clip255(v + ae_lo + (int)(aug_hash(seed, pix, (flags & 8u) ? c : 0, 2u) % (uint32_t)ae_n));
-      if (noise_k) {
-        const uint32_t h = aug_hash(seed, pix, (flags & 2u) ? c : 0, 3u);
-        const int sum = (int)(h & 255u) + (int)((h >> 8) & 255u) + (int)((h >> 16) & 255u) + (int)(h >> 24);
-        v = clip255(v + (((sum - 510) * noise_k + 32768) >> 16));
-      }
-      if (drop_t && (aug_hash(seed, pix, (flags & 4u) ? c : 0, 4u) >> 8) < drop_t) v = 0;
-      if (c < 4) px[c] = v;
-      if (C != 3) img_out[i * C + c] = (uint8_t)((flags & 1u) ? 255 - v : v);
-    }
-    if (C == 3) {
-      const int gq = (int)s.gray_q;
-      if (gq) {
-        const int gray = (px[0] * 4899 + px[1] * 9617 + px[2] * 1868 + 8192) >> 14;
-#pragma unroll
-        for (int c = 0; c < 3; ++c) px[c] = (gq * gray + (256 - gq) * px[c] + 128) >> 8;
-      }
-#pragma unroll
-      for (int c = 0; c < 3; ++c) img_out[i * 3 + c] = (uint8_t)((flags & 1u) ? 255 - px[c] : px[c]);
-    }
-    if (mask) {
-      const int64_t mx = (X0 + 512) >> 10, my = (Y0 + 512) >> 10;
-      uint8_t mv = 0;
-      if (mx >= 0 && mx < Win && my >= 0 && my < Hin) mv = mask[((int64_t)n * Hin + my) * Win + mx];
-      mask_out[i] = mv;
     }
   }
 }
@@ -96,10 +193,13 @@
 static int launch_augment(const uint8_t* img, const uint8_t* mask, uint8_t* img_out, uint8_t* mask_out, const float* params,
                           const int32_t* field, int32_t N, int32_t Hin, int32_t Win, int32_t Hout, int32_t Wout, int32_t C, void* stream) {
   if (!img || !img_out || !params || N <= 0 || C <= 0 || (mask && !mask_out)) return STP_E_BADARG;
-  int64_t g = ((int64_t)N * Hout * Wout + 255) / 256;
-  if (g > 8192) g = 8192;
-  hipLaunchKernelGGL(augment_kernel, dim3((int)g), dim3(256), 0, (hipStream_t)stream, img, mask, img_out, mask_out,
-                     (const AugSample*)params, N, Hin, Win, Hout, Wout, C, field);
+  if (Hout <= 0 || Wout <= 0) return STP_OK;
+  const int tiles_x = (Wout + AUG_TW - 1) / AUG_TW;
+  const int64_t tiles = (int64_t)tiles_x * ((Hout + AUG_TH - 1) / AUG_TH);
+  if (tiles > 0x7fffffffLL) return STP_E_BADARG;
+  const int wide = (Wout & 3) == 0 && (((uintptr_t)img | (uintptr_t)img_out | (uintptr_t)mask | (uintptr_t)mask_out) & 3) == 0;
+  hipLaunchKernelGGL(augment_kernel, dim3((unsigned)tiles, (unsigned)(N < 65535 ? N : 65535)), dim3(256), 0, (hipStream_t)stream, img, mask,
+                     img_out, mask_out, (const AugSample*)params, N, Hin, Win, Hout, Wout, C, field, tiles_x, wide);
   STP_LAUNCH_CHECK();
   return STP_OK;
 }
diff --git a/segmentation_training_pipeline_amd/csrc/bn_pool.hip b/segmentation_training_pipeline_amd/csrc/bn_pool.hip
--- a/segmentation_training_pipeline_amd/csrc/bn_pool.hip
+++ b/segmentation_training_pipeline_amd/csrc/bn_pool.hip
@@ -1224,15 +1224,18 @@
       sh[e] = (e < 4 ? b0[e & 3] : b1[e & 3]) - (e < 4 ? m0[e & 3] : m1[e & 3]) * k;
     }
   }
+  u32x4 keep[3] = {};
   for (int rr = 0; rr < POOL_ROWS; ++rr) {
     const int orow = blockIdx.y * POOL_ROWS + rr;
     if (orow >= N * Ho) break;
     const int n = orow / Ho, ho = orow - n * Ho;
+    const bool reuse = rr > 0 && ho > 0;
     u32x4 v[9];
 #pragma unroll
     for (int kh = 0; kh < 3; ++kh)
 #pragma unroll
       for (int kw = 0; kw < 3; ++kw) {
+        if (kh == 0 && reuse) continue;
         const int h = min(max(2 * ho - 1 + kh, 0), H - 1), w = min(max(2 * wo - 1 + kw, 0), W - 1);
         v[kh * 3 + kw] = *reinterpret_cast<const u32x4*>(x + (((size_t)n * H + h) * W + w) * C + c);
       }
@@ -1247,14 +1250,19 @@
         u32x4 o;
 #pragma unroll
         for (int e = 0; e < 4; ++e) {
-          const float lo = bn_act(bn_affine(h16lo_to_f32(v[kh * 3 + kw][e]), sc[2 * e], sh[2 * e]), relu);
-          const float hi = bn_act(bn_affine(h16hi_to_f32(v[kh * 3 + kw][e]), sc[2 * e + 1], sh[2 * e + 1]), relu);
-          o[e] = pack_bf16x2(lo, hi);
+          if (kh == 0 && reuse) {
+            o[e] = keep[kw][e];
+          } else {
+            const float lo = bn_act(bn_affine(h16lo_to_f32(v[kh * 3 + kw][e]), sc[2 * e], sh[2 * e]), relu);
+            const float hi = bn_act(bn_affine(h16hi_to_f32(v[kh * 3 + kw][e]), sc[2 * e + 1], sh[2 * e + 1]), relu);
+            o[e] = pack_bf16x2(lo, hi);
+          }
           const float tl = in ? h16lo_to_f32(o[e]) : 0.f, th = in ? h16hi_to_f32(o[e]) : 0.f;
           if ((kh | kw) == 0 || tl > best[2 * e]) { best[2 * e] = tl; bi[2 * e] = (uint8_t)(kh * 3 + kw); }
           if ((kh | kw) == 0 || th > best[2 * e + 1]) { best[2 * e + 1] = th; bi[2 * e + 1] = (uint8_t)(kh * 3 + kw); }
         }
         if (kh >= 1 && kw >= 1 && in) *reinterpret_cast<u32x4*>(yb + (((size_t)n * H + h) * W + w) * C + c) = o;
+        if (kh == 2) keep[kw] = o;
       }
     const size_t oo = (((size_t)n * Ho + ho) * Wo + wo) * C + c;
     *reinterpret_cast<u32x4*>(y + oo) = u32x4{pack_bf16x2(best[0], best[1]), pack_bf16x2(best[2], best[3]), pack_bf16x2(best[4], best[5]),
@@ -2989,15 +2997,39 @@
   out[c] = accumulate ? out[c] + (float)t.s : (float)t.s;
 }
 
+__global__ __launch_bounds__(256) void colsum1_partial_kernel(const bf16_t* __restrict__ x, int64_t rows, float* partial) {
+  __shared__ float red[256];
+  const int64_t rowsPerBlock = (rows + gridDim.x - 1) / gridDim.x;
+  const int64_t r0 = (int64_t)blockIdx.x * rowsPerBlock;
+  const int64_t r1 = r0 + rowsPerBlock < rows ? r0 + rowsPerBlock : rows;
+  float s = 0.f;
+  int64_t r = r0 + threadIdx.x;
+  for (; r + 3 * 256 < r1; r += 4 * 256) {
+    const float v0 = bf16_to_f32(x[r]), v1 = bf16_to_f32(x[r + 256]), v2 = bf16_to_f32(x[r + 512]), v3 = bf16_to_f32(x[r + 768]);
+    s += (v0 + v1) + (v2 + v3);
+  }
+  for (; r < r1; r += 256) s += bf16_to_f32(x[r]);
+  red[threadIdx.x] = s;
+  __syncthreads();
+  if (threadIdx.x == 0) {
+    float a = 0.f;
+    for (int t = 0; t < 256; ++t) a += red[t];
+    partial[(size_t)blockIdx.x * 2] = a;
+    partial[(size_t)blockIdx.x * 2 + 1] = 0.f;
+  }
+}
+
 extern "C" int stp_channel_sum(const void* x, int32_t dtype, int64_t rows, int32_t C, float* out, int32_t accumulate,
                                void* workspace, size_t workspace_bytes, void* stream) {
   if (!stp_dtype_ok(dtype)) return STP_E_BADARG;
-  if (!x || !out || !workspace || rows <= 0 || C <= 0 || (C & 3)) return STP_E_BADARG;
+  if (!x || !out || !workspace || rows <= 0 || C <= 0 || ((C & 3) && !(C == 1 && dtype == STP_H16))) return STP_E_BADARG;
   if (workspace_bytes < stp_bn_workspace_bytes(C)) return STP_E_WORKSPACE;
   hipStream_t s = (hipStream_t)stream;
   const int blocks = bn_blocks(rows);
   float* partial = (float*)workspace;
-  if (dtype == STP_H16 && (C & 7) == 0)
+  if (dtype == STP_H16 && C == 1)
+    hipLaunchKernelGGL(colsum1_partial_kernel, dim3(blocks), dim3(256), 0, s, (const bf16_t*)x, rows, partial);
+  else if (dtype == STP_H16 && (C & 7) == 0)
     hipLaunchKernelGGL((bn_partial_kernel<bf16_t, 8>), dim3(blocks), dim3(256), 256 * 16 * sizeof(float), s, (const bf16_t*)x, rows, C, partial);
   else if (dtype == STP_H16)
     hipLaunchKernelGGL((bn_partial_kernel<bf16_t, 4>), dim3(blocks), dim3(256), 256 * 8 * sizeof(float), s, (const bf16_t*)x, rows, C, partial);
diff --git a/segmentation_training_pipeline_amd/csrc/conv_sc.h b/segmentation_training_pipeline_amd/csrc/conv_sc.h
--- a/segmentation_training_pipeline_amd/csrc/conv_sc.h
+++ b/segmentation_training_pipeline_amd/csrc/conv_sc.h
@@ -18,6 +18,7 @@
   int sum2;
   uint32_t src_bytes;
   BnBack pbn;
+  int compact;
 };
 
 template <typename T> struct ScStageBn;
@@ -100,6 +101,7 @@
   int ctot, coff;
   uint32_t src_bytes, dy_bytes;
   BnBack pbn;
+  int compact;
 };
 
 constexpr int ST_HH = (SC_TH - 1) * 2 + 7, ST_HW = 70, ST_WROW = 464, ST_HALO = ST_HH * ST_HW * 8, ST_WBYTES = 64 * ST_WROW;
@@ -123,3 +125,4 @@
 
 int sc_lean_launch(const ScArgs& a, int cin, int dtype, hipStream_t s);
 int sc_wg_lean_launch(const ScWgArgs& a, int cin, int cout, int dtype, int blocks, hipStream_t s);
+bool sc_lean_compact_on();
diff --git a/segmentation_training_pipeline_amd/csrc/conv_sc.hip b/segmentation_training_pipeline_amd/csrc/conv_sc.hip
--- a/segmentation_training_pipeline_amd/csrc/conv_sc.hip
+++ b/segmentation_training_pipeline_amd/csrc/conv_sc.hip
@@ -561,8 +561,10 @@
   if (!p || !stp_dtype_ok(p->dtype)) return 0;
   const int vec = p->dtype == STP_H16 ? 8 : 4;
   const int cin = p->C0;
-  const bool cin_ok = p->dtype == STP_F32 ? (cin == 4 || cin == 8 || cin == 16) : (cin == 8 || cin == 16 || cin == 32);
-  return p->KH == 3 && p->KW == 3 && p->stride == 1 && p->pad == 1 && p->C1 == 0 && cin_ok && (cin % vec) == 0 && p->Cout <= 32 &&
+  const bool compact = p->dtype == STP_H16 && cin == 1 && p->Cout == 16 && p->src0_mode == STP_SRC_DIRECT && !p->bias && !p->relu &&
+                       !p->accumulate0 && !p->stats_slots && !p->dst_sum2x2 && !p->src_bn_mean && sc_lean_compact_on();
+  const bool cin_ok = p->dtype == STP_F32 ? (cin == 4 || cin == 8 || cin == 16) : (cin == 8 || cin == 16 || cin == 32 || compact);
+  return p->KH == 3 && p->KW == 3 && p->stride == 1 && p->pad == 1 && p->C1 == 0 && cin_ok && ((cin % vec) == 0 || compact) && p->Cout <= 32 &&
          p->Cd0 == p->Cout && !p->residual && p->Ho == p->Hv && p->Wo == p->Wv &&
          (p->src0_mode == STP_SRC_DIRECT || (p->src0_mode == STP_SRC_NEAREST2X && p->Hv == 2 * p->Hs0 && p->Wv == 2 * p->Ws0));
 }
@@ -594,10 +596,12 @@
   if (a.sum2 && ((p->Cout & 3) || (a.H & 1) || (a.W & 1) || p->bias || p->relu || (a.stats && !a.bnb.x))) return STP_E_BADARG;
   const_cast<stp_conv_params*>(p)->stats_tiles = stp_conv2d_sc_stats_tiles(p);
   hipStream_t s = (hipStream_t)stream;
+  a.compact = p->C0 == 1;
   {
-    const int r = sc_lean_launch(a, p->C0, p->dtype, s);
+    const int r = sc_lean_launch(a, a.compact ? 8 : p->C0, p->dtype, s);
     if (r != 1) return r;
   }
+  if (a.compact) return STP_E_BADARG;
   return p->dtype == STP_H16 ? dispatch_sc<bf16_t>(a, p->C0, s) : dispatch_sc<float>(a, p->C0, s);
 }
 
@@ -1917,8 +1921,9 @@
   const int vec = p->dtype == STP_H16 ? 8 : 4;
   const bool c0ok = p->C0 == 16 || p->C0 == 32 || (p->C0 == 64 && vec == 8);
   const bool c1ok = p->C1 == 0 || p->C1 == 16 || p->C1 == 32 || (p->C1 == 64 && vec == 8);
+  const bool compact = p->dtype == STP_H16 && p->Cout == 1 && p->C0 == 16 && p->C1 == 0 && p->src0_mode == STP_SRC_DIRECT && sc_lean_compact_on();
   return p->KH == 3 && p->KW == 3 && p->stride == 1 && p->pad == 1 && c0ok && c1ok &&
-         (p->Cout == 8 || p->Cout == 16 || p->Cout == 32 || (p->Cout == 4 && vec == 4)) && (p->Cout % vec) == 0 &&
+         (((p->Cout == 8 || p->Cout == 16 || p->Cout == 32 || (p->Cout == 4 && vec == 4)) && (p->Cout % vec) == 0) || compact) &&
          p->Ho == p->Hv && p->Wo == p->Wv &&
          (p->src0_mode == STP_SRC_DIRECT || (p->src0_mode == STP_SRC_NEAREST2X && p->Hv == 2 * p->Hs0 && p->Wv == 2 * p->Ws0));
 }
@@ -2013,6 +2018,11 @@
   a.dy_bytes = dyb < lim ? (uint32_t)dyb : 0u;
   a.src_bytes = b0 < lim ? (uint32_t)b0 : 0u;
   a.src = (const char*)p->src0; a.Hs = p->Hs0; a.Ws = p->Ws0; a.up = p->src0_mode == STP_SRC_NEAREST2X; a.coff = 0;
+  a.compact = p->Cout == 1;
+  if (a.compact) {
+    const int r = a.dy_bytes && a.src_bytes ? sc_wg_lean_launch(a, p->C0, 8, p->dtype, blocks, s) : 1;
+    return r == 1 ? STP_E_BADARG : r;
+  }
   int rc = p->dtype == STP_H16 ? sc_wg_dispatch<bf16_t>(a, p->C0, p->Cout, blocks, s) : sc_wg_dispatch<float>(a, p->C0, p->Cout, blocks, s);
   if (rc != STP_OK || p->C1 == 0) return rc;
   a.pbn.mean = nullptr;
diff --git a/segmentation_training_pipeline_amd/csrc/conv_sc_lean.hip b/segmentation_training_pipeline_amd/csrc/conv_sc_lean.hip
--- a/segmentation_training_pipeline_amd/csrc/conv_sc_lean.hip
+++ b/segmentation_training_pipeline_amd/csrc/conv_sc_lean.hip
@@ -12,10 +12,12 @@
   else *reinterpret_cast<u32x2*>(p) = o[0];
 }
 
-template <int CIN, int TM, int EPI, bool PBN, bool UP>
+template <int CIN, int TM, int EPI, bool PBN, bool UP, bool CD = false>
 __global__ __launch_bounds__(256, (TM == 1 ? (CIN <= 16 ? SC_WPE_SMALL : 3) : 2)) void conv_sc_lean_kernel(const ScArgs a) {
   typedef bf16_t T;
   constexpr int SZ = 2, VEC = 8, KC = 32, K = 9 * CIN, NCH = (K + KC - 1) / KC, VPP = CIN / VEC, PIXB = CIN * SZ;
+  constexpr int SPB = CD ? SZ : PIXB;
+  static_assert(!CD || (CIN == 8 && !PBN && !UP), "compact source: one real channel of 8, direct source");
   constexpr int HH = UP ? SC_TH / 2 + 2 : SC_HH, HW = UP ? SC_TW / 2 + 2 : SC_HW;
   constexpr int NV = HH * HW * VPP, NPASS = (NV + 255) / 256, BUF = NPASS * 4096;
   constexpr bool PART = (K % KC) != 0;
@@ -52,8 +54,9 @@
     const int v = p * 256 + tid, pix = v / VPP;
     const int hy = pix / HW, hx = pix - hy * HW;
     hyx[p] = v < NV ? (hy << 16 | hx) : -1;
-    lo[p] = v < NV ? (uint32_t)(((hy - 1) * a.Ws + (hx - 1)) * PIXB + cvb) : 0x80000000u;
-  }
+    lo[p] = v < NV ? (uint32_t)(((hy - 1) * a.Ws + (hx - 1)) * SPB + cvb) : 0x80000000u;
+  }
+  uint32_t stg[NPASS];
 
   auto decode = [&](int tile) -> TileC {
     const int bq = (int)fdiv((uint32_t)tile, a.divTx);
@@ -68,19 +71,22 @@
   auto issue_tile = [&](const TileC& t, int b, bool live) -> uint32_t {
     uint32_t inside = 0;
     if (live && t.interior) {
-      const uint32_t tb = (uint32_t)((t.n * a.Hs + (t.y0 >> sh)) * a.Ws + (t.x0 >> sh)) * (uint32_t)PIXB;
-#pragma unroll
-      for (int p = 0; p < NPASS; ++p)
-        __builtin_amdgcn_raw_ptr_buffer_load_lds(rs, (__attribute__((address_space(3))) void*)(smem + b * BUF + p * 4096 + wave * 1024), 16, (int)(tb + lo[p]), 0, 0, 0);
+      const uint32_t tb = (uint32_t)((t.n * a.Hs + (t.y0 >> sh)) * a.Ws + (t.x0 >> sh)) * (uint32_t)SPB;
+#pragma unroll
+      for (int p = 0; p < NPASS; ++p) {
+        if constexpr (CD) stg[p] = __builtin_amdgcn_raw_buffer_load_b16(rs, (int)(tb + lo[p]), 0, 0);
+        else __builtin_amdgcn_raw_ptr_buffer_load_lds(rs, (__attribute__((address_space(3))) void*)(smem + b * BUF + p * 4096 + wave * 1024), 16, (int)(tb + lo[p]), 0, 0, 0);
+      }
       inside = (1u << NPASS) - 1u;
     } else {
 #pragma unroll
       for (int p = 0; p < NPASS; ++p) {
         const int gy = (t.y0 >> sh) - 1 + (hyx[p] >> 16), gx = (t.x0 >> sh) - 1 + (hyx[p] & 0xffff);
         const bool ok = live && hyx[p] >= 0 && (unsigned)gy < (unsigned)a.Hs && (unsigned)gx < (unsigned)a.Ws;
-        const uint32_t off = ok ? (uint32_t)((t.n * a.Hs + gy) * a.Ws + gx) * (uint32_t)PIXB + (uint32_t)cvb : 0x80000000u;
+        const uint32_t off = ok ? (uint32_t)((t.n * a.Hs + gy) * a.Ws + gx) * (uint32_t)SPB + (uint32_t)cvb : 0x80000000u;
         inside |= ok ? (1u << p) : 0u;
-        __builtin_amdgcn_raw_ptr_buffer_load_lds(rs, (__attribute__((address_space(3))) void*)(smem + b * BUF + p * 4096 + wave * 1024), 16, (int)off, 0, 0, 0);
+        if constexpr (CD) stg[p] = __builtin_amdgcn_raw_buffer_load_b16(rs, (int)off, 0, 0);
+        else __builtin_amdgcn_raw_ptr_buffer_load_lds(rs, (__attribute__((address_space(3))) void*)(smem + b * BUF + p * 4096 + wave * 1024), 16, (int)off, 0, 0, 0);
       }
     }
     return inside;
@@ -183,6 +189,10 @@
     if (PBN) sbn.load_tab(ptab, ptab + 32, (tid % VPP) * VEC);
     __builtin_amdgcn_s_waitcnt(0x0f70);
     asm volatile("" ::: "memory");
+    if constexpr (CD) {
+#pragma unroll
+      for (int p = 0; p < NPASS; ++p) *reinterpret_cast<u32x4*>(smem + cur * BUF + (p * 256 + tid) * 16) = u32x4{stg[p] & 0xffffu, 0u, 0u, 0u};
+    }
     if (PBN) {
 #pragma unroll
       for (int p0 = 0; p0 < NPASS; p0 += 3) {
@@ -376,7 +386,7 @@
   }
 }
 
-template <int CIN, int TM, int EPI, bool PBN, bool UP>
+template <int CIN, int TM, int EPI, bool PBN, bool UP, bool CD = false>
 static int launch_scl(const ScArgs& a, hipStream_t s) {
   const int ntiles = a.N * a.tiles_x * a.tiles_y;
   constexpr int NV = (UP ? (SC_TH / 2 + 2) * (SC_TW / 2 + 2) : SC_HH * SC_HW) * (CIN / 8), NPASS = (NV + 255) / 256;
@@ -384,11 +394,11 @@
   const int blocks = sc_stream_blocks(STP_H16, CIN, TM * 16, ntiles);
   static bool attr_set = false;
   if (lds > 64 * 1024 && !attr_set) {
-    if (hipFuncSetAttribute(reinterpret_cast<const void*>(conv_sc_lean_kernel<CIN, TM, EPI, PBN, UP>), hipFuncAttributeMaxDynamicSharedMemorySize, (int)lds) != hipSuccess)
+    if (hipFuncSetAttribute(reinterpret_cast<const void*>(conv_sc_lean_kernel<CIN, TM, EPI, PBN, UP, CD>), hipFuncAttributeMaxDynamicSharedMemorySize, (int)lds) != hipSuccess)
       return STP_E_LAUNCH;
     attr_set = true;
   }
-  hipLaunchKernelGGL((conv_sc_lean_kernel<CIN, TM, EPI, PBN, UP>), dim3(blocks), dim3(256), lds, s, a);
+  hipLaunchKernelGGL((conv_sc_lean_kernel<CIN, TM, EPI, PBN, UP, CD>), dim3(blocks), dim3(256), lds, s, a);
   STP_LAUNCH_CHECK();
   return STP_OK;
 }
@@ -417,11 +427,17 @@
   static const bool on = !(getenv("STP_SC_LEAN") && atoi(getenv("STP_SC_LEAN")) == 0);
   return on;
 }
+bool sc_lean_compact_on() { return sc_lean_on() && sc_stream_on(); }
 
 int sc_lean_launch(const ScArgs& a, int cin, int dtype, hipStream_t s) {
   if (!sc_lean_on() || !sc_stream_on() || dtype != STP_H16 || a.stat_slots || a.accumulate || a.relu) return 1;
   const bool pbn = a.pbn.mean != nullptr;
   const int tm = a.Cout <= 16 ? 1 : 2;
+  if (a.compact) {
+    if (cin != 8 || a.Cout != 16 || a.up || pbn || a.bias || a.sum2) return 1;
+    if (a.bnb.x) return a.stats ? launch_scl<8, 1, SCL_BNB, false, false, true>(a, s) : 1;
+    return launch_scl<8, 1, SCL_STATS, false, false, true>(a, s);
+  }
   if (a.bnb.x) {
     if (pbn || a.bias || !a.stats || a.Cout != tm * 16) return 1;
     return a.sum2 ? dispatch_scl<SCL_BNB_SUM2, false>(a, cin, tm, s) : dispatch_scl<SCL_BNB, false>(a, cin, tm, s);
@@ -435,10 +451,12 @@
   return pbn ? dispatch_scl<SCL_STATS, true>(a, cin, tm, s) : dispatch_scl<SCL_STATS, false>(a, cin, tm, s);
 }
 
-template <int CIN, int COUT, bool PBN, bool UP>
+template <int CIN, int COUT, bool PBN, bool UP, bool CD = false>
 __global__ __launch_bounds__(256) void conv_sc_wgrad_lean_kernel(const ScWgArgs a) {
   typedef bf16_t T;
   constexpr int SZ = 2, VEC = 8, TMo = (COUT + 15) / 16, TNi = CIN / 16, PIXB = CIN * SZ, DYB = COUT * SZ;
+  constexpr int DSB = CD ? SZ : DYB;
+  static_assert(!CD || COUT == 8, "compact dY: one real channel of 8");
   constexpr int VPPX = CIN / VEC, VPPD = COUT / VEC;
   constexpr int HH = UP ? SC_TH / 2 + 2 : SC_HH, HW = UP ? SC_TW / 2 + 2 : SC_HW;
   constexpr int NVX = HH * HW * VPPX, NPX = (NVX + 255) / 256;
@@ -488,8 +506,9 @@
       const int v = p * 256 + tid, pix = v / VPPD;
       const int py = pix / SC_TW, px = pix % SC_TW;
       pyx[p] = v < NVD ? (py << 16 | px) : -1;
-      lod[p] = v < NVD ? (uint32_t)((py * a.W + px) * DYB) + cvd : 0x80000000u;
-    }
+      lod[p] = v < NVD ? (uint32_t)((py * a.W + px) * DSB) + cvd : 0x80000000u;
+    }
+    uint32_t dstg[NPD];
     auto decode = [&](int tile) -> TileC {
       int b = tile;
       const int tx = b % a.tiles_x; b /= a.tiles_x;
@@ -504,13 +523,15 @@
       char* xb = smem + bsel * BUF;
       if (live && t.interior) {
         const uint32_t tbx = (uint32_t)((t.n * a.Hs + (t.y0 >> sh)) * a.Ws + (t.x0 >> sh)) * (uint32_t)PIXB;
-        const uint32_t tbd = (uint32_t)((t.n * a.H + t.y0) * a.W + t.x0) * (uint32_t)DYB;
+        const uint32_t tbd = (uint32_t)((t.n * a.H + t.y0) * a.W + t.x0) * (uint32_t)DSB;
 #pragma unroll
         for (int p = 0; p < NPX; ++p)
           __builtin_amdgcn_raw_ptr_buffer_load_lds(rsx, (__attribute__((address_space(3))) void*)(xb + p * 4096 + wave * 1024), 16, (int)(tbx + lox[p]), 0, 0, 0);
 #pragma unroll
-        for (int p = 0; p < NPD; ++p)
-          __builtin_amdgcn_raw_ptr_buffer_load_lds(rsd, (__attribute__((address_space(3))) void*)(xb + XBUF + p * 4096 + wave * 1024), 16, (int)(tbd + lod[p]), 0, 0, 0);
+        for (int p = 0; p < NPD; ++p) {
+          if constexpr (CD) dstg[p] = __builtin_amdgcn_raw_buffer_load_b16(rsd, (int)(tbd + lod[p]), 0, 0);
+          else __builtin_amdgcn_raw_ptr_buffer_load_lds(rsd, (__attribute__((address_space(3))) void*)(xb + XBUF + p * 4096 + wave * 1024), 16, (int)(tbd + lod[p]), 0, 0, 0);
+        }
         inside = (1u << NPX) - 1u;
       } else {
 #pragma unroll
@@ -525,8 +546,9 @@
         for (int p = 0; p < NPD; ++p) {
           const int gy = t.y0 + (pyx[p] >> 16), gx = t.x0 + (pyx[p] & 0xffff);
           const bool ok = live && pyx[p] >= 0 && gy < a.H && gx < a.W;
-          const uint32_t off = ok ? (uint32_t)((t.n * a.H + gy) * a.W + gx) * (uint32_t)DYB + cvd : 0x80000000u;
-          __builtin_amdgcn_raw_ptr_buffer_load_lds(rsd, (__attribute__((address_space(3))) void*)(xb + XBUF + p * 4096 + wave * 1024), 16, (int)off, 0, 0, 0);
+          const uint32_t off = ok ? (uint32_t)((t.n * a.H + gy) * a.W + gx) * (uint32_t)DSB + cvd : 0x80000000u;
+          if constexpr (CD) dstg[p] = __builtin_amdgcn_raw_buffer_load_b16(rsd, (int)off, 0, 0);
+          else __builtin_amdgcn_raw_ptr_buffer_load_lds(rsd, (__attribute__((address_space(3))) void*)(xb + XBUF + p * 4096 + wave * 1024), 16, (int)off, 0, 0, 0);
         }
       }
       return inside;
@@ -547,6 +569,11 @@
     for (int tile = t_first; tile < t_end; tile += t_step, cur ^= 1) {
       __builtin_amdgcn_s_waitcnt(0x0f70);
       asm volatile("" ::: "memory");
+      if constexpr (CD) {
+#pragma unroll
+        for (int p = 0; p < NPD; ++p)
+          *reinterpret_cast<u32x4*>(smem + cur * BUF + XBUF + (p * 256 + tid) * 16) = u32x4{dstg[p] & 0xffffu, 0u, 0u, 0u};
+      }
       if (PBN) {
 #pragma unroll
         for (int p0 = 0; p0 < NPX; p0 += 3) {
@@ -646,17 +673,17 @@
   }
 }
 
-template <int CIN, int COUT, bool PBN, bool UP>
+template <int CIN, int COUT, bool PBN, bool UP, bool CD = false>
 static int launch_scwl(const ScWgArgs& a, int blocks, hipStream_t s) {
   constexpr int NPX = ((UP ? (SC_TH / 2 + 2) * (SC_TW / 2 + 2) : SC_HH * SC_HW) * (CIN / 8) + 255) / 256, NPD = (SC_TH * SC_TW * (COUT / 8) + 255) / 256;
   const size_t lds = (size_t)2 * (NPX + NPD) * 4096;
   static bool attr_set = false;
   if (lds > 64 * 1024 && !attr_set) {
-    if (hipFuncSetAttribute(reinterpret_cast<const void*>(conv_sc_wgrad_lean_kernel<CIN, COUT, PBN, UP>), hipFuncAttributeMaxDynamicSharedMemorySize, (int)lds) != hipSuccess)
+    if (hipFuncSetAttribute(reinterpret_cast<const void*>(conv_sc_wgrad_lean_kernel<CIN, COUT, PBN, UP, CD>), hipFuncAttributeMaxDynamicSharedMemorySize, (int)lds) != hipSuccess)
       return STP_E_LAUNCH;
     attr_set = true;
   }
-  hipLaunchKernelGGL((conv_sc_wgrad_lean_kernel<CIN, COUT, PBN, UP>), dim3(blocks), dim3(256), lds, s, a);
+  hipLaunchKernelGGL((conv_sc_wgrad_lean_kernel<CIN, COUT, PBN, UP, CD>), dim3(blocks), dim3(256), lds, s, a);
   STP_LAUNCH_CHECK();
   return STP_OK;
 }
@@ -681,6 +708,10 @@
 
 int sc_wg_lean_launch(const ScWgArgs& a, int cin, int cout, int dtype, int blocks, hipStream_t s) {
   if (!sc_lean_on() || !sc_stream_on() || dtype != STP_H16 || !a.src_bytes || !a.dy_bytes) return 1;
+  if (a.compact) {
+    if (cin != 16 || cout != 8 || a.up) return 1;
+    return a.pbn.mean ? launch_scwl<16, 8, true, false, true>(a, blocks, s) : launch_scwl<16, 8, false, false, true>(a, blocks, s);
+  }
   if (a.up) return a.pbn.mean ? dispatch_scwl<true, true>(a, cin, cout, blocks, s) : dispatch_scwl<false, true>(a, cin, cout, blocks, s);
   return a.pbn.mean ? dispatch_scwl<true, false>(a, cin, cout, blocks, s) : dispatch_scwl<false, false>(a, cin, cout, blocks, s);
 }
diff --git a/segmentation_training_pipeline_amd/graph.py b/segmentation_training_pipeline_amd/graph.py
--- a/segmentation_training_pipeline_amd/graph.py
+++ b/segmentation_training_pipeline_amd/graph.py
@@ -363,7 +363,7 @@
     def _emit_conv(self, lst, p, meta=None):
         self._keep.append(p)
         if meta is not None and meta.get("tile") == 512:
-            meta = dict(meta, sc=(int(p.C0), 1 if p.Cout <= 16 else 2))
+            meta = dict(meta, sc=(max(int(p.C0), 8) if self.dtype != "fp32" else int(p.C0), 1 if p.Cout <= 16 else 2))
         if meta is not None and meta.get("tile") == 800:
             meta = dict(meta, pw=(int(p.C0), int(p.Cout)))
         lst.append((self.lib.stp_conv2d, (C.byref(p),), "stp_conv2d", meta))
@@ -1151,6 +1151,8 @@
         self.loss_scalars = self._alloc((16,), torch.float32)
         self.loss_scalars.zero_()
         count = logits.rows
+        if not w_lovasz and logits.meta.get("conv_layer") is not None:
+            logits.meta["conv_layer"].compact_head_grad()
         if w_iou or w_jaccard or w_focal:
             dl = self._emit_loss("stp_sigmoid_loss_ex", logits, target, (count,), (w_bce, w_dice, w_iou, w_jaccard, w_focal))
         else:
@@ -1357,7 +1359,8 @@
         CoutB = self.CoutB = _rup(Cout, cout_pad or pl.vec)
         self.x_ng, self.s_ng = x.needs_grad, (src1.needs_grad if src1 is not None else False)
         self.out = pl._new(name, self.Ho, self.Wo, Cout, self.x_ng or self.s_ng or w.trainable or (residual is not None and residual.needs_grad))
-        self.out.gradC = CoutB
+        self.out.gradC = self.dyC = CoutB
+        self.out.meta["conv_layer"] = self
         if bias:
             pl._bn_ws_c = max(pl._bn_ws_c, CoutB)
         pl._use(x, src1, residual)
@@ -1367,6 +1370,25 @@
         wp.accumulate, wp.dtype, wp.splits = 0, pl.cdt, 0
         if pl.training and w.trainable:
             pl._wg_ws_bytes = max(pl._wg_ws_bytes, int(pl.lib.stp_conv2d_wgrad_workspace_bytes(C.byref(wp))))
+
+    def compact_head_grad(self):
+        pl, x, out = self.plan, self.x, self.out
+        if (self.Cout != 1 or pl.dtype not in ("bf16", "fp16") or not pl.training or os.environ.get("STP_HEAD_GRAD_COMPACT", "1") == "0"
+                or self.k != 3 or self.stride != 1 or self.pad != 1 or self.transpose or self.upsample or self.stem or self.src1 is not None
+                or self.residual is not None or self.fs is not None or self.relu or self.param_cols is not None or not self.w.trainable
+                or out.grad is not None or x.meta.get("uses", 0) != 1 or pl.slot_arena is not None):
+            return
+        wq = _lib.WgradParams.from_buffer_copy(self.wp)
+        wq.Cout = 1
+        if not pl.lib.stp_wgrad_sc_eligible(C.byref(wq)):
+            return
+        if self.need_dgrad:
+            q = _lib.ConvParams()
+            q.N, q.Hs0, q.Ws0, q.Hv, q.Wv, q.C0, q.C1, q.src0_mode = pl.N, self.Ho, self.Wo, self.Ho, self.Wo, 1, 0, ops.SRC_DIRECT
+            q.KH, q.KW, q.stride, q.pad, q.Ho, q.Wo, q.Cout, q.Cd0, q.dtype = 3, 3, 1, 1, self.Hv, self.Wv, self.C0, self.C0, pl.cdt
+            if not pl.lib.stp_conv2d_sc_eligible(C.byref(q)):
+                return
+        self.wp.Cout = out.gradC = self.dyC = 1
 
     def forward(self, bn_stats, flops_as):
         pl, x, src1, residual, out, k, Cout = self.plan, self.x, self.src1, self.residual, self.out, self.k, self.Cout
@@ -1456,7 +1478,7 @@
         elif b is not None and b.trainable and out.meta.get("loss_bias_grad") == "multilabel":
             pl._emit(pl.bwd, "stp_sigmoid_multilabel_bias_grad", pl.ws_loss.data_ptr(), out.rows, self.Cout, pl._gptr(b), 0)
         elif b is not None and b.trainable:
-            pl._emit_bias_grad(dy, out.rows, self.CoutB, self.Cout, b)
+            pl._emit_bias_grad(dy, out.rows, out.gradC, self.Cout, b)
         if self.need_dgrad and not out.meta.get("dgrad_folded"):
             self._data_grad()
 
@@ -1550,7 +1572,7 @@
                                    stride=2, pad=k - 1 - self.pad, Ho=x.H, Wo=x.W, Cout=C0, dtype=pl.cdt, accumulate0=self.acc0)
         return ops.conv_params(self.dy, self.wb, self.d0, N=pl.N, Hs0=Ho, Ws0=Wo,
                                Hv=(2 * Ho - 1 if stride == 2 else Ho), Wv=(2 * Wo - 1 if stride == 2 else Wo),
-                               C0=self.CoutB, mode=(ops.SRC_ZEROINS2X if stride == 2 else ops.SRC_DIRECT), KH=k, KW=k, stride=1,
+                               C0=self.dyC, mode=(ops.SRC_ZEROINS2X if stride == 2 else ops.SRC_DIRECT), KH=k, KW=k, stride=1,
                                pad=k - 1 - self.pad, Ho=self.Hv, Wo=self.Wv, Cout=C0 + self.C1, dtype=pl.cdt, dst1=self.d1, Cd0=C0,
                                accumulate0=self.acc0, accumulate1=self.acc1)
 
```
